# MKimiSH/video-filler

Measured on AMD Instinct MI355X. Metric: netG+netD fwd+bwd images/sec, 128x128 center-mask, higher is better.
Workload: dtype f32

## Files before the change

### include/vf_hip.h

```cpp
#ifndef VF_HIP_H
#define VF_HIP_H
#include <stddef.h>
#include <stdint.h>
#ifdef __cplusplus
extern "C" {
#endif

typedef struct vf_ctx vf_ctx;

enum { VF_ACT_NONE = 0, VF_ACT_LRELU = 1, VF_ACT_RELU = 2, VF_ACT_TANH = 3, VF_ACT_SIGMOID = 4 };

const char* vf_last_error(void);
int vf_version(void);
int vf_ctx_create(vf_ctx** out, int device, void* stream);
int vf_ctx_destroy(vf_ctx* ctx);
int vf_ctx_set_mfma_mode(vf_ctx* ctx, int mode);
int vf_ctx_set_stream(vf_ctx* ctx, void* stream);
int vf_ctx_set_workspace(vf_ctx* ctx, void* ptr, size_t bytes);
size_t vf_workspace_bytes_hint(void);
int vf_stream_synchronize(vf_ctx* ctx);
int vf_malloc(void** out, size_t bytes);
int vf_free(void* ptr);
int vf_memcpy_h2d(vf_ctx* ctx, void* dst, const void* src, size_t bytes);
int vf_memcpy_d2h(vf_ctx* ctx, void* dst, const void* src, size_t bytes);
// ... 6 lines not shown
int vf_conv2d_fwd(vf_ctx* ctx, const float* x, const float* w, const float* bias, float* y, int B, int H,
                  int W, int Cin, int Cout, int k, int stride, int pad, int act, float slope);
int vf_conv2d_bwd_data(vf_ctx* ctx, const float* gy, const float* w, float* gx, int B, int H, int W,
                       int Cin, int Cout, int k, int stride, int pad);
int vf_conv2d_bwd_data_act(vf_ctx* ctx, const float* gy, const float* w, float* gx, const float* x_act, int act,
                           float slope, int B, int H, int W, int Cin, int Cout, int k, int stride, int pad);
int vf_conv2d_bwd_weight(vf_ctx* ctx, const float* x, const float* gy, float* gw, float* gb, int B, int H,
                         int W, int Cin, int Cout, int k, int stride, int pad, float beta);

int vf_deconv2d_fwd(vf_ctx* ctx, const float* x, const float* w, const float* bias, float* y, int B, int H,
                    int W, int Cin, int Cout, int k, int stride, int pad, int act, float slope);
int vf_deconv2d_bwd_data(vf_ctx* ctx, const float* gy, const float* w, float* gx, int B, int H, int W,
                         int Cin, int Cout, int k, int stride, int pad);
int vf_deconv2d_bwd_weight(vf_ctx* ctx, const float* x, const float* gy, float* gw, float* gb, int B, int H,
                           int W, int Cin, int Cout, int k, int stride, int pad, float beta);

int vf_planes_split(vf_ctx* ctx, const float* x, void* planes, int64_t n);
int vf_conv2d_fwd_planes(vf_ctx* ctx, const float* x, const float* w, const float* bias, float* y, void* y_planes, int B,
                         int H, int W, int Cin, int Cout, int k, int stride, int pad, int act, float slope);
int vf_weight_planes(vf_ctx* ctx, const float* w, void* planes_native, void* planes_transposed, int d0, int d1);
int vf_weight_planes_multi(vf_ctx* ctx, const void* desc_dev, int n, int blocks);
int vf_pconv_supported(int B, int H, int W, int Cin, int Cout, int k, int stride, int pad, int transposed);
int vf_pconv_supported_in_mode(int mfma_mode, int B, int H, int W, int Cin, int Cout, int k, int stride, int pad, int transposed);
int vf_pconv_set_routing(int gather_patch, int scatter_patch);
int vf_pconv_gather(vf_ctx* ctx, const void* ap, const void* wp, const float* bias, float* y, int B, int H, int W, int Cin,
                    int Cout, int act, float slope);
int vf_pconv_scatter(vf_ctx* ctx, const void* ap, const void* wp, const float* bias, float* y, int B, int H, int W, int Cin,
                     int Cout, int act, float slope, const float* dmask, int dact, float dslope);
int vf_conv2d_bwd_weight_planes(vf_ctx* ctx, const float* x, const float* gy, const void* x_planes, const void* gy_planes, float* gw,
                                float* gb, int B, int H, int W, int Cin, int Cout, int k, int stride, int pad, float beta);
int vf_deconv2d_bwd_weight_planes(vf_ctx* ctx, const float* x, const float* gy, const void* x_planes, const void* gy_planes,
                                  float* gw, float* gb, int B, int H, int W, int Cin, int Cout, int k, int stride, int pad,
                                  float beta);

int vf_bn_stats(vf_ctx* ctx, const float* x, const float* shift, double* sums, int64_t npix, int C);
int vf_bn_finalize(vf_ctx* ctx, const double* sums, float* running_mean, float* running_var, float* save_mean,
                   float* save_invstd, int64_t n_total, int C, float momentum, float eps);
int vf_bn_apply(vf_ctx* ctx, const float* x, float* y, const float* gamma, const float* beta, const float* mean,
                const float* invstd, int64_t npix, int C, int act, float slope);
int vf_bn_train_fwd(vf_ctx* ctx, const float* x, float* y, const float* gamma, const float* beta,
                    float* running_mean, float* running_var, float* save_mean, float* save_invstd, double* sums,
                    int64_t npix, int C, float momentum, float eps, int act, float slope);
int vf_bn_eval_fwd(vf_ctx* ctx, const float* x, float* y, const float* gamma, const float* beta,
                   const float* running_mean, const float* running_var, int64_t npix, int C, float eps, int act,
                   float slope);
int vf_bn_bwd_stats(vf_ctx* ctx, const float* x, const float* y_act, const float* gy, const float* save_mean,
                    double* sums, int64_t npix, int C, int act, float slope);
int vf_bn_bwd_apply(vf_ctx* ctx, const float* x, const float* y_act, const float* gy, float* gx, float* ggamma,
                    float* gbeta, const float* gamma, const float* save_mean, const float* save_invstd,
                    const double* sums, int64_t npix, int64_t n_total, int C, int act, float slope, float pbeta);
int vf_bn_bwd(vf_ctx* ctx, const float* x, const float* y_act, const float* gy, float* gx, float* ggamma,
              float* gbeta, const float* gamma, const float* save_mean, const float* save_invstd, double* sums,
              int64_t npix, int C, int act, float slope, float pbeta);
int vf_bn_train_fwd_groups(vf_ctx* ctx, const float* x, float* y, const float* gamma, const float* beta,
                           float* running_mean, float* running_var, float* save_mean, float* save_invstd,
                           double* sums, int64_t npix_per_group, int C, int groups, float momentum, float eps,
                           int act, float slope);
int vf_bn_bwd_groups(vf_ctx* ctx, const float* x, const float* y_act, const float* gy, float* gx, float* ggamma,
                     float* gbeta, const float* gamma, const float* save_mean, const float* save_invstd,
                     double* sums, int64_t npix_per_group, int C, int groups, int act, float slope, float pbeta);

int vf_bn_train_fwd_planes(vf_ctx* ctx, const float* x, float* y, const float* gamma, const float* beta,
                           float* running_mean, float* running_var, float* save_mean, float* save_invstd, double* sums,
                           int64_t npix_per_group, int C, int groups, float momentum, float eps, int act, float slope,
                           void* y_planes);
int vf_bn_bwd_planes(vf_ctx* ctx, const float* x, const float* y_act, const float* gy, float* gx, float* ggamma,
// ... 158 lines not shown
                   int reason_cap);
int vf_gif_decode_workspace_bytes(const unsigned char* data, const int64_t* offs, int n, int alpha, size_t* ws_bytes,
                                  size_t* stage_bytes);
int vf_gif_decode(vf_ctx* ctx, const unsigned char* data, const int64_t* offs, int n, int alpha, const int64_t* out_offs,
                  unsigned char* out, void* stage, size_t stage_bytes, void* ws, size_t ws_bytes, int32_t* status);

int vf_display_workspace_bytes(int N, int C, int h, int w, int padding, int nrow, int scaleeach, int has_min, int has_max,
                               size_t* ws_bytes);
int vf_display_tensor(vf_ctx* ctx, const float* packed, int src_layout, float* grid, int N, int C, int h, int w, int padding,
                      int nrow, int scaleeach, int has_min, double min, int has_max, double max, int symmetric, int saturate);
int vf_center_finish(vf_ctx* ctx, const float* ctx_nhwc, const float* pred_nhwc, float* pretty, float* pasted,
                     float* pred_mapped, int B, int C, int fs, int overlapPred);

enum {
  VF_METRICS_N = 0, VF_METRICS_SSE = 1, VF_METRICS_SAE = 2, VF_METRICS_SSIM_Q = 3, VF_METRICS_SSIM_N = 4,
  VF_METRICS_FLICKER = 5, VF_METRICS_COLS = 6
};
int vf_frame_metrics(vf_ctx* ctx, const void* a, const void* b, int kind, int N, int C, int H, int W, int vh, int vw,
                     const unsigned char* mask, int clip, int64_t* table);

int vf_channel_copy(vf_ctx* ctx, const float* src, int Csrc, int c_src, float* dst, int Cdst, int c_dst, int Ccopy,
                    int64_t npix);
int vf_noise_fill(vf_ctx* ctx, float* out, int64_t n, uint64_t seed, const int32_t* counter_dev, uint64_t counter,
                  int normal);

int vf_wgrad_group_begin(vf_ctx* ctx);
int vf_wgrad_group_end(vf_ctx* ctx);
int vf_wgrad_group_abort(vf_ctx* ctx);
int vf_wgrad_group_count(vf_ctx* ctx, int* count);
int vf_wgrad_group_end_partial(vf_ctx* ctx, int count);

int vf_bias_grad_plan(int64_t P, int C, int* cq, int* rows_per_block, int* gx, int* gy);
int vf_bias_grad_multi(vf_ctx* ctx, const void* desc_dev, int n, int blocks1, int blocks2);

typedef struct vf_comm vf_comm;
#define VF_COMM_ID_BYTES 128
int vf_comm_available(void);
int vf_comm_unique_id(void* id128);
int vf_comm_init(vf_comm** out, const void* id128, int world, int rank);
int vf_comm_world(const vf_comm* c);
int vf_comm_rank(const vf_comm* c);
int vf_comm_allreduce_async(vf_comm* c, vf_ctx* ctx, void* buf, int64_t count, int dtype, int op, int* ticket);
int vf_comm_allreduce_avg_async(vf_comm* c, vf_ctx* ctx, float* buf, int64_t n, int* ticket);
int vf_comm_reduce_scatter_avg_async(vf_comm* c, vf_ctx* ctx, float* buf, int64_t shard_count, int* ticket);
int vf_comm_allgather_async(vf_comm* c, vf_ctx* ctx, float* buf, int64_t shard_count, int* ticket);
int vf_comm_broadcast_async(vf_comm* c, vf_ctx* ctx, float* buf, int64_t count, int root, int* ticket);
int vf_comm_wait(vf_comm* c, vf_ctx* ctx, int ticket);
int vf_comm_allreduce_inline(vf_comm* c, vf_ctx* ctx, void* buf, int64_t count, int dtype, int op);
int vf_comm_broadcast(vf_comm* c, vf_ctx* ctx, void* buf, int64_t count, int dtype, int root);
int vf_comm_barrier(vf_comm* c, vf_ctx* ctx);
int vf_comm_destroy(vf_comm* c);

int vf_prof_begin(vf_ctx* ctx);
int vf_prof_end(vf_ctx* ctx);
int vf_prof_count(void);
int vf_prof_get(int i, char* name, int name_cap, int64_t* launches, double* ms, double* flops, double* bytes);

enum { VF_L_CONV = 1, VF_L_FULLCONV = 2, VF_L_BN = 3, VF_L_ACT = 4, VF_L_VIEW = 5 };
typedef struct vf_layer_desc {
  int kind;
  int nin, nout;
  int k, stride, pad;
  int act;
  float slope;
  float eps, momentum;
} vf_layer_desc;
// ... 60 lines not shown
```

### video-filler_amd/_lib.py

```python
import ctypes as C
import os
import re

_HERE = os.path.dirname(os.path.abspath(__file__))
_HEADER = os.path.join(_HERE, "..", "include", "vf_hip.h")

vp, f32, i32, i64, f64, sz, u64 = C.c_void_p, C.c_float, C.c_int, C.c_int64, C.c_double, C.c_size_t, C.c_uint64

SIGNATURES = {
    "vf_last_error": (C.c_char_p, []),
    "vf_version": (i32, []),
    "vf_ctx_create": (i32, [C.POINTER(vp), i32, vp]),
    "vf_ctx_destroy": (i32, [vp]),
    "vf_ctx_set_mfma_mode": (i32, [vp, i32]),
    "vf_ctx_set_stream": (i32, [vp, vp]),
    "vf_ctx_set_workspace": (i32, [vp, vp, sz]),
    "vf_workspace_bytes_hint": (sz, []),
    "vf_stream_synchronize": (i32, [vp]),
    "vf_malloc": (i32, [C.POINTER(vp), sz]),
    "vf_free": (i32, [vp]),
    "vf_memcpy_h2d": (i32, [vp, vp, vp, sz]),
    "vf_memcpy_d2h": (i32, [vp, vp, vp, sz]),
    "vf_zero": (i32, [vp, vp, sz]),
    "vf_zero_segments": (i32, [vp, vp, vp, vp, i32]),
# ... 13 lines not shown
    "vf_pconv_supported_in_mode": (i32, [i32] * 10),
    "vf_pconv_set_routing": (i32, [i32, i32]),
    "vf_pconv_gather": (i32, [vp, vp, vp, vp, vp] + [i32] * 5 + [i32, f32]),
    "vf_pconv_scatter": (i32, [vp, vp, vp, vp, vp] + [i32] * 5 + [i32, f32, vp, i32, f32]),
    "vf_bn_stats": (i32, [vp, vp, vp, vp, i64, i32]),
    "vf_bn_finalize": (i32, [vp, vp, vp, vp, vp, vp, i64, i32, f32, f32]),
    "vf_bn_apply": (i32, [vp, vp, vp, vp, vp, vp, vp, i64, i32, i32, f32]),
    "vf_bn_train_fwd": (i32, [vp] * 10 + [i64, i32, f32, f32, i32, f32]),
    "vf_bn_eval_fwd": (i32, [vp] * 7 + [i64, i32, f32, i32, f32]),
    "vf_bn_bwd_stats": (i32, [vp] * 6 + [i64, i32, i32, f32]),
    "vf_bn_bwd_apply": (i32, [vp] * 11 + [i64, i64, i32, i32, f32, f32]),
    "vf_bn_bwd": (i32, [vp] * 11 + [i64, i32, i32, f32, f32]),
    "vf_bn_train_fwd_groups": (i32, [vp] * 10 + [i64, i32, i32, f32, f32, i32, f32]),
    "vf_bn_bwd_groups": (i32, [vp] * 11 + [i64, i32, i32, i32, f32, f32]),
    "vf_bn_train_fwd_planes": (i32, [vp] * 10 + [i64, i32, i32, f32, f32, i32, f32, vp]),
    "vf_bn_bwd_planes": (i32, [vp] * 11 + [i64, i32, i32, i32, f32, f32, vp]),
    "vf_bn_fuse_next_fwd": (i32, [vp, vp, vp, i32, i32]),
    "vf_bn_fuse_next_bwd": (i32, [vp, vp, vp, i32, f32, vp, vp, i32, i32]),
    "vf_bn_fuse_result": (i32, [vp, C.POINTER(i32)]),
    "vf_bn_train_fwd_pre": (i32, [vp, vp, i32] + [vp] * 9 + [i64, i32, i32, f32, f32, i32, f32, vp]),
    "vf_bn_bwd_pre": (i32, [vp, vp, i32] + [vp] * 9 + [i64, i32, i32, f32, vp]),
    "vf_act_fwd": (i32, [vp, vp, vp, i64, i32, f32]),
    "vf_act_bwd": (i32, [vp, vp, vp, vp, i64, i32, f32]),
    "vf_axpby": (i32, [vp, f32, vp, f32, vp, i64]),
    "vf_cmul": (i32, [vp, vp, vp, i64]),
    "vf_scale_shift": (i32, [vp, vp, f32, f32, i64]),
    "vf_masked_compose": (i32, [vp, vp, vp, vp, vp, i64]),
    "vf_conv2d_bwd_data_act": (i32, [vp, vp, vp, vp, vp, i32, f32, i32, i32, i32, i32, i32, i32, i32, i32]),
    "vf_wgrad_group_begin": (i32, [vp]),
    "vf_wgrad_group_end": (i32, [vp]),
    "vf_wgrad_group_abort": (i32, [vp]),
    "vf_bias_grad_plan": (i32, [i64, i32, vp, vp, vp, vp]),
    "vf_bias_grad_multi": (i32, [vp, vp, i32, i32, i32]),
    "vf_center_prepare": (i32, [vp, vp, vp, vp, vp, i32, i32, i32, i32]),
    "vf_clip_prepare": (i32, [vp, vp, vp, vp, vp, vp, i32, i32, i32, i32, i32, i32, i32, f32, i32, i32, vp, vp]),
    "vf_tiles_gather": (i32, [vp, vp, vp, i32, i32, i32, i32, i32, vp]),
    "vf_tiles_scatter": (i32, [vp, vp, vp, i32, i32, i32, i32, i32, vp]),
    "vf_image_scale": (i32, [vp, vp, i32, vp] + [i32] * 6),
    "vf_image_scale_u8": (i32, [vp, vp, vp] + [i32] * 6),
    "vf_image_hook2d": (i32, [vp, vp, i32, vp] + [i32] * 9),
    "vf_image_whole_frames": (i32, [vp, vp, i32, vp] + [i32] * 8 + [vp, f32]),
    "vf_crop_stats": (i32, [vp, vp, vp] + [i32] * 6 + [vp]),
    "vf_patch_array_prepare": (i32, [vp, vp, i32] + [vp] * 5 + [i32] * 10 + [f32]),
    "vf_jpeg_inspect": (i32, [vp, sz, i32, vp, C.c_char_p, i32]),
    "vf_jpeg_workspace_bytes": (i32, [vp, vp, i32, i32, C.POINTER(sz), C.POINTER(sz)]),
    "vf_jpeg_decode": (i32, [vp, vp, vp, i32, i32, i32, vp, vp, vp, sz, vp, sz, vp, vp]),
    "vf_jpeg_scans_inspect": (i32, [vp, sz, vp, vp, i32, C.c_char_p, i32]),
    "vf_jpeg_prog_workspace_bytes": (i32, [vp, vp, i32, i32, C.POINTER(sz), C.POINTER(sz)]),
    "vf_jpeg_prog_decode": (i32, [vp, vp, vp, i32, i32, i32, vp, vp, vp, sz, vp, sz, vp, vp, vp]),
    "vf_jpeg_prog_coefficients_host": (i32, [vp, sz, i32, vp, sz, vp]),
    "vf_jpeg_inspect_layouts": (i32, [vp, sz, vp, C.c_char_p, i32]),
    "vf_jpeg_layouts_workspace_bytes": (i32, [vp, vp, i32, i32, C.POINTER(sz), C.POINTER(sz)]),
    "vf_jpeg_decode_layouts": (i32, [vp, vp, vp, i32, i32, i32, vp, vp, vp, sz, vp, sz, vp, vp, vp]),
    "vf_jpeg_layouts_coefficients_host": (i32, [vp, sz, i32, vp, sz, vp]),
    "vf_png_inspect": (i32, [vp, sz, vp, C.c_char_p, i32]),
    "vf_png_decode_workspace_bytes": (i32, [vp, vp, i32, i32, C.POINTER(sz), C.POINTER(sz)]),
    "vf_png_decode": (i32, [vp, vp, vp, i32, i32, vp, vp, vp, sz, vp, sz, vp]),
    "vf_png_bytes_to_float": (i32, [vp, vp, vp, i64]),
    "vf_png_inspect_full": (i32, [vp, sz, vp, vp, C.c_char_p, i32]),
    "vf_png_decode_full_workspace_bytes": (i32, [vp, vp, i32, i32, i32, C.POINTER(sz), C.POINTER(sz)]),
    "vf_png_decode_full": (i32, [vp, vp, vp, i32, i32, i32, vp, vp, vp, sz, vp, sz, vp]),
    "vf_png_workspace_bytes": (i32, [i32, i32, i32, i32, C.POINTER(sz), C.POINTER(sz)]),
    "vf_png_encode": (i32, [vp, vp, i32, i32, i32, i32, i32, vp, sz, vp, sz, vp]),
    "vf_jpeg_encode_workspace_bytes": (i32, [i32, i32, i32, i32, i32, C.POINTER(sz), C.POINTER(sz)]),
    "vf_jpeg_encode": (i32, [vp, vp, i32, i32, i32, i32, i32, i32, i32, vp, sz, vp, sz, vp]),
    "vf_jpeg_encode_opts_workspace_bytes": (i32, [i32] * 8 + [C.POINTER(sz), C.POINTER(sz)]),
# ... 6 lines not shown
    "vf_apng_encode": (i32, [vp, vp, i32, i32, i32, i32, i32, i32, i32, i32, vp, sz, vp, sz, vp]),
    "vf_apng_inspect": (i32, [vp, sz, vp, vp, i32, C.c_char_p, i32]),
    "vf_apng_decode_workspace_bytes": (i32, [vp, vp, i32, i32, C.POINTER(sz), C.POINTER(sz)]),
    "vf_apng_decode": (i32, [vp, vp, vp, i32, i32, vp, vp, vp, sz, vp, sz, vp]),
    "vf_gif_inspect": (i32, [vp, sz, vp, vp, i32, C.c_char_p, i32]),
    "vf_gif_decode_workspace_bytes": (i32, [vp, vp, i32, i32, C.POINTER(sz), C.POINTER(sz)]),
    "vf_gif_decode": (i32, [vp, vp, vp, i32, i32, vp, vp, vp, sz, vp, sz, vp]),
    "vf_display_workspace_bytes": (i32, [i32] * 9 + [C.POINTER(sz)]),
    "vf_display_tensor": (i32, [vp, vp, i32, vp] + [i32] * 8 + [f64, i32, f64, i32, i32]),
    "vf_center_finish": (i32, [vp] * 6 + [i32] * 4),
    "vf_frame_metrics": (i32, [vp, vp, vp] + [i32] * 7 + [vp, i32, vp]),
    "vf_channel_copy": (i32, [vp, vp, i32, i32, vp, i32, i32, i32, i64]),
    "vf_noise_fill": (i32, [vp, vp, i64, u64, vp, u64, i32]),
    "vf_bce_fwd": (i32, [vp, vp, f32, i32, vp]),
    "vf_bce_bwd": (i32, [vp, vp, f32, vp, i32]),
    "vf_bce_fwd_bwd": (i32, [vp, vp, f32, f32, i32, i32, vp, vp, vp]),
    "vf_mse_fwd": (i32, [vp, vp, vp, i64, vp]),
    "vf_mse_bwd": (i32, [vp, vp, vp, vp, i64]),
    "vf_recon_grad_mix": (i32, [vp, vp, vp, vp, vp, f32, f32, f32, i32, i32, i32, i64, vp]),
    "vf_gdl_fwd": (i32, [vp, vp, vp, i32, i32, i32, i32, vp]),
    "vf_gdl_bwd": (i32, [vp, vp, vp, vp, i32, i32, i32, i32]),
    "vf_masked_mse_fwd": (i32, [vp, vp, vp, vp, f32, i64, vp]),
    "vf_masked_mse_bwd": (i32, [vp, vp, vp, vp, f32, vp, i64]),
    "vf_adam_step": (i32, [vp, vp, vp, vp, vp, i64, f64, f64, f64, f64, vp]),
    "vf_adam_prep": (i32, [vp, f64, f64, f64, vp]),
    "vf_adam_apply": (i32, [vp, vp, vp, vp, vp, i64, f64, f64, f64, vp]),
    "vf_adam_apply_ranges": (i32, [vp, vp, vp, vp, vp, C.POINTER(i64), C.POINTER(i64), i32, f64, f64, f64, vp]),
    "vf_wgrad_adam_outer_supported": (i32, [i32, i32, i32]),
    "vf_wgrad_adam_outer": (i32, [vp, vp, vp, i32, i32, i32, vp, vp, vp, vp, f64, f64, f64, vp]),
    "vf_wgrad_adam_outer_gathered": (i32, [vp, vp, vp, i32, i32, i64, i32, i32, vp, vp, vp, vp, C.c_float, f64, f64, f64, vp]),
    "vf_wgrad_adam_outer_rows": (i32, [vp, vp, vp, i32, i32, i64, i32, i32, i32, i32, vp, vp, vp, vp, C.c_float, f64, f64, f64, vp]),
    "vf_conv_is_fast": (i32, [i32, i32, i32, i32, i32]),
    "vf_conv2d_bwd_weight_planes": (i32, [vp, vp, vp, vp, vp, vp, vp, i32, i32, i32, i32, i32, i32, i32, i32, f32]),
    "vf_deconv2d_bwd_weight_planes": (i32, [vp, vp, vp, vp, vp, vp, vp, i32, i32, i32, i32, i32, i32, i32, i32, f32]),
    "vf_comm_available": (i32, []),
    "vf_comm_unique_id": (i32, [vp]),
    "vf_comm_init": (i32, [C.POINTER(vp), vp, i32, i32]),
    "vf_comm_world": (i32, [vp]),
    "vf_comm_rank": (i32, [vp]),
    "vf_comm_allreduce_async": (i32, [vp, vp, vp, i64, i32, i32, C.POINTER(i32)]),
    "vf_comm_allreduce_avg_async": (i32, [vp, vp, vp, i64, C.POINTER(i32)]),
    "vf_comm_reduce_scatter_avg_async": (i32, [vp, vp, vp, i64, C.POINTER(i32)]),
    "vf_comm_allgather_async": (i32, [vp, vp, vp, i64, C.POINTER(i32)]),
    "vf_comm_broadcast_async": (i32, [vp, vp, vp, i64, i32, C.POINTER(i32)]),
    "vf_comm_wait": (i32, [vp, vp, i32]),
    "vf_comm_allreduce_inline": (i32, [vp, vp, vp, i64, i32, i32]),
    "vf_comm_broadcast": (i32, [vp, vp, vp, i64, i32, i32]),
    "vf_comm_barrier": (i32, [vp, vp]),
    "vf_comm_destroy": (i32, [vp]),
    "vf_net_create": (i32, [vp, C.POINTER(vp), vp, i32, i32, i32, i32, i32]),
    "vf_net_destroy": (i32, [vp]),
    "vf_net_parameters": (i32, [vp, C.POINTER(vp), C.POINTER(vp), C.POINTER(i64)]),
    "vf_net_param_offset": (i64, [vp, i32, i32, C.POINTER(i64)]),
    "vf_net_bn_running": (i32, [vp, i32, C.POINTER(vp), C.POINTER(vp)]),
    "vf_net_training": (i32, [vp, i32]),
    "vf_net_zero_grad": (i32, [vp]),
    "vf_net_forward": (i32, [vp, vp, C.POINTER(vp)]),
    "vf_net_backward": (i32, [vp, vp, vp, C.POINTER(vp)]),
    "vf_net_update_grad_input": (i32, [vp, vp, vp, C.POINTER(vp)]),
    "vf_net_layer_output": (i32, [vp, i32, C.POINTER(vp)]),
    "vf_net_layer_grad_input": (i32, [vp, i32, C.POINTER(vp)]),
    "vf_net_layer_shape": (i32, [vp, i32] + [C.POINTER(i32)] * 7),
    "vf_net_reshape": (i32, [vp, i32, i32, i32, i32]),
    "vf_net_bind_parameters": (i32, [vp, vp, vp, i64]),
    "vf_net_bind_bn_running": (i32, [vp, i32, vp, vp]),
    "vf_net_bn_saved": (i32, [vp, i32, C.POINTER(vp), C.POINTER(vp)]),
# ... 79 lines not shown
```

### video-filler_amd/backend.py

```python
import ctypes as C
import os

import numpy as np
import torch

from . import _lib

ACT = {"none": 0, "lrelu": 1, "relu": 2, "tanh": 3, "sigmoid": 4}
COLSUM_DESC = [("g", "<u8"), ("gb", "<u8"), ("part", "<u8"), ("P", "<i8"), ("C", "<i4"), ("cq", "<i4"), ("rows_per_block", "<i4"),
               ("gx", "<i4"), ("gy", "<i4"), ("blk1_off", "<i4"), ("blk2_off", "<i4"), ("beta", "<f4")]
WPLANES_DESC = [("w", "<u8"), ("nat", "<u8"), ("tr", "<u8"), ("d0", "<i4"), ("d1", "<i4"), ("gx", "<i4"), ("gz", "<i4"),
                ("blk_off", "<i4"), ("pad", "<i4")]
MFMA_MODES = {"f32": 0, "bf16": 1, "f32_3xbf16": 3}
DEFAULT_MFMA_MODE = "f32_3xbf16"


_COMM_DTYPE = {torch.float32: 0, torch.float64: 1}
_COMM_OP = {"sum": 0, "avg": 1, "max": 2, "min": 3}


class _Range:
    def __init__(self, lib, name):
        self.lib, self.name = lib, name.encode()

    def __enter__(self):
        self.lib.vf_range_push(self.name)
        return self

    def __exit__(self, *exc):
        self.lib.vf_range_pop()
        return False


class _CommHandle:

    def __init__(self, backend, ticket):
        self.backend, self.ticket = backend, ticket

    def wait(self):
        b = self.backend
        _lib.check(b.lib.vf_comm_wait(b.comm, b.ctx, self.ticket))


def exchange_comm_id(backend, world, rank, addr=None, port=None, timeout_s=300):
    import datetime
# ... 640 lines not shown
        self._c("vf_conv2d_fwd_planes", _ptr(x), _ptr(w), _ptr(bias), _ptr(y), _ptr(y_planes), B, H, W, Cin, w.shape[0], k, stride,
                pad, ACT[act], slope)

    def conv2d_bwd_data(self, gy, w, gx, k, stride, pad):
        B, Cin, H, W = gx.shape
        self._c("vf_conv2d_bwd_data", _ptr(gy), _ptr(w), _ptr(gx), B, H, W, Cin, w.shape[0], k, stride, pad)

    def conv2d_bwd_data_act(self, gy, w, gx, x_act, act, slope, k, stride, pad):
        B, Cin, H, W = gx.shape
        self._c("vf_conv2d_bwd_data_act", _ptr(gy), _ptr(w), _ptr(gx), _ptr(x_act), ACT[act], slope, B, H, W, Cin,
                w.shape[0], k, stride, pad)

    def wgrad_group_begin(self):
        self._c("vf_wgrad_group_begin")

    def wgrad_group_end(self):
        self._c("vf_wgrad_group_end")

    def wgrad_group_abort(self):
        self._c("vf_wgrad_group_abort")

    def wgrad_group_count(self):
        n = C.c_int(0)
        self._c("vf_wgrad_group_count", C.byref(n))
        return n.value

    def wgrad_group_end_partial(self, count):
        self._c("vf_wgrad_group_end_partial", int(count))

    def bias_grad_multi(self, items):
        import numpy as np
        if not items:
            return
        key = (self.workspace.data_ptr(), self.workspace.numel()) + tuple(
            (g.data_ptr(), gb.data_ptr(), g.numel(), gb.numel(), float(beta)) for g, gb, beta in items)
        cache = self.__dict__.setdefault("_colsum_plans", {})
        plan = cache.get(key)
        if plan is None:
            desc = np.zeros(len(items), dtype=COLSUM_DESC)
            ws = self.workspace.data_ptr()
            off, b1, b2 = 0, 0, 0
            for i, (g, gb, beta) in enumerate(items):
                Cc = gb.numel()
                P = g.numel() // Cc
                assert Cc % 4 == 0 and g.data_ptr() % 16 == 0 and is_nhwc(g)
                geo = [C.c_int() for _ in range(4)]
                _lib.check(self.lib.vf_bias_grad_plan(P, Cc, *[C.byref(v) for v in geo]))
                cq, rpb, gx, gy = [v.value for v in geo]
                desc[i] = (g.data_ptr(), gb.data_ptr(), ws + off, P, Cc, cq, rpb, gx, gy, b1, b2, beta)
                off += (gx * Cc * 8 + 255) // 256 * 256
                b1 += gx * gy
                b2 += (Cc + 3) // 4
            assert off <= self.workspace.numel(), "workspace too small for the bias-gradient partials"
            dev = torch.from_numpy(desc.view(np.uint8).copy()).to(self.device)
            plan = (dev, len(items), b1, b2)
            cache[key] = plan
        dev, n, b1, b2 = plan
        self._c("vf_bias_grad_multi", _ptr(dev), n, b1, b2)

    def conv2d_bwd_weight(self, x, gy, gw, gb, k, stride, pad, beta, x_planes=None, gy_planes=None):
        B, Cin, H, W = x.shape
        if x_planes is not None and gy_planes is not None:
            self._c("vf_conv2d_bwd_weight_planes", _ptr(x), _ptr(gy), _ptr(x_planes), _ptr(gy_planes), _ptr(gw), _ptr(gb), B, H, W,
                    Cin, gw.shape[0], k, stride, pad, beta)
            return
        self._c("vf_conv2d_bwd_weight", _ptr(x), _ptr(gy), _ptr(gw), _ptr(gb), B, H, W, Cin, gw.shape[0], k, stride,
                pad, beta)

    def deconv2d_fwd(self, x, w, bias, y, k, stride, pad, act="none", slope=0.0):
        B, Cin, H, W = x.shape
        self._c("vf_deconv2d_fwd", _ptr(x), _ptr(w), _ptr(bias), _ptr(y), B, H, W, Cin, w.shape[1], k, stride, pad,
                ACT[act], slope)

    def deconv2d_bwd_data(self, gy, w, gx, k, stride, pad):
        B, Cin, H, W = gx.shape
        self._c("vf_deconv2d_bwd_data", _ptr(gy), _ptr(w), _ptr(gx), B, H, W, Cin, w.shape[1], k, stride, pad)

    def deconv2d_bwd_weight(self, x, gy, gw, gb, k, stride, pad, beta, x_planes=None, gy_planes=None):
        B, Cin, H, W = x.shape
        if x_planes is not None and gy_planes is not None:
            self._c("vf_deconv2d_bwd_weight_planes", _ptr(x), _ptr(gy), _ptr(x_planes), _ptr(gy_planes), _ptr(gw), _ptr(gb), B, H,
                    W, Cin, gw.shape[1], k, stride, pad, beta)
            return
        self._c("vf_deconv2d_bwd_weight", _ptr(x), _ptr(gy), _ptr(gw), _ptr(gb), B, H, W, Cin, gw.shape[1], k, stride,
                pad, beta)

    def planes_split(self, x, planes=None):
        n = x.numel()
        if planes is None:
            planes = torch.empty((3, n), dtype=torch.bfloat16, device=self.device)
        self._c("vf_planes_split", _ptr(x), _ptr(planes), n)
        return planes

    def weight_planes(self, w, native=None, transposed=None, want_transposed=True):
        d0, d1 = w.shape[0], w.shape[1]
        n = w.numel()
        if native is None:
            native = torch.empty((3, n), dtype=torch.bfloat16, device=self.device)
        if transposed is None and want_transposed:
            transposed = torch.empty((3, n), dtype=torch.bfloat16, device=self.device)
# ... 29 lines not shown
        self._c("vf_pconv_scatter", _ptr(ap), _ptr(wp), _ptr(bias), _ptr(y), B, H, W, Cin, Cout, ACT[act], slope, _ptr(dmask),
                ACT[dact], dslope)

    def bn_stats(self, x, shift, sums):
        B, Cc, H, W = x.shape
        self._c("vf_bn_stats", _ptr(x), _ptr(shift), _ptr(sums), B * H * W, Cc)

    def bn_finalize(self, sums, rm, rv, save_mean, save_invstd, n_total, momentum, eps):
        self._c("vf_bn_finalize", _ptr(sums), _ptr(rm), _ptr(rv), _ptr(save_mean), _ptr(save_invstd), n_total,
                rm.numel(), momentum, eps)

    def bn_apply(self, x, y, gamma, beta, mean, invstd, act="none", slope=0.0):
        B, Cc, H, W = x.shape
        self._c("vf_bn_apply", _ptr(x), _ptr(y), _ptr(gamma), _ptr(beta), _ptr(mean), _ptr(invstd), B * H * W, Cc,
                ACT[act], slope)

    def bn_train_fwd(self, x, y, gamma, beta, rm, rv, save_mean, save_invstd, sums, momentum, eps, act="none", slope=0.0):
        B, Cc, H, W = x.shape
        self._c("vf_bn_train_fwd", _ptr(x), _ptr(y), _ptr(gamma), _ptr(beta), _ptr(rm), _ptr(rv), _ptr(save_mean),
                _ptr(save_invstd), _ptr(sums), B * H * W, Cc, momentum, eps, ACT[act], slope)

    def bn_train_fwd_groups(self, x, y, gamma, beta, rm, rv, save_mean, save_invstd, sums, groups, momentum, eps,
                            act="none", slope=0.0, y_planes=None):
        B, Cc, H, W = x.shape
        assert B % groups == 0 and save_mean.numel() == groups * Cc and sums.numel() == groups * 2 * Cc
        if y_planes is not None:
            self._c("vf_bn_train_fwd_planes", _ptr(x), _ptr(y), _ptr(gamma), _ptr(beta), _ptr(rm), _ptr(rv), _ptr(save_mean),
                    _ptr(save_invstd), _ptr(sums), (B // groups) * H * W, Cc, groups, momentum, eps, ACT[act], slope, _ptr(y_planes))
            return
        self._c("vf_bn_train_fwd_groups", _ptr(x), _ptr(y), _ptr(gamma), _ptr(beta), _ptr(rm), _ptr(rv), _ptr(save_mean),
                _ptr(save_invstd), _ptr(sums), (B // groups) * H * W, Cc, groups, momentum, eps, ACT[act], slope)

    def bn_bwd_groups(self, x, y_act, gy, gx, ggamma, gbeta, gamma, save_mean, save_invstd, sums, groups, act="none",
                      slope=0.0, pbeta=1.0, gx_planes=None):
        B, Cc, H, W = x.shape
        assert B % groups == 0 and save_mean.numel() == groups * Cc and sums.numel() == groups * 2 * Cc
        if gx_planes is not None:
            self._c("vf_bn_bwd_planes", _ptr(x), _ptr(y_act), _ptr(gy), _ptr(gx), _ptr(ggamma), _ptr(gbeta), _ptr(gamma),
                    _ptr(save_mean), _ptr(save_invstd), _ptr(sums), (B // groups) * H * W, Cc, groups, ACT[act], slope, pbeta,
                    _ptr(gx_planes))
            return
        self._c("vf_bn_bwd_groups", _ptr(x), _ptr(y_act), _ptr(gy), _ptr(gx), _ptr(ggamma), _ptr(gbeta), _ptr(gamma),
                _ptr(save_mean), _ptr(save_invstd), _ptr(sums), (B // groups) * H * W, Cc, groups, ACT[act], slope, pbeta)

    def bn_fuse_next_fwd(self, shift, part, groups=1):
        self._c("vf_bn_fuse_next_fwd", _ptr(shift), _ptr(part), part.numel() // (2 * shift.numel()), groups)

    def bn_fuse_next_bwd(self, x, y_act, act, slope, save_mean, part, groups=1):
        Cc = x.shape[1]
        self._c("vf_bn_fuse_next_bwd", _ptr(x), _ptr(y_act), ACT[act], slope, _ptr(save_mean), _ptr(part),
                part.numel() // (2 * Cc), groups)

    def bn_fuse_result(self):
        rows = C.c_int(0)
        self._c("vf_bn_fuse_result", C.byref(rows))
        return rows.value

    def bn_train_fwd_pre(self, part, rows, x, y, gamma, beta, rm, rv, save_mean, save_invstd, sums, groups, momentum, eps,
                         act="none", slope=0.0, y_planes=None):
        B, Cc, H, W = x.shape
        self._c("vf_bn_train_fwd_pre", _ptr(part), rows, _ptr(x), _ptr(y), _ptr(gamma), _ptr(beta), _ptr(rm), _ptr(rv),
                _ptr(save_mean), _ptr(save_invstd), _ptr(sums), (B // groups) * H * W, Cc, groups, momentum, eps, ACT[act], slope,
                _ptr(y_planes))

    def bn_bwd_pre(self, part, rows, x, g_masked, gx, ggamma, gbeta, gamma, save_mean, save_invstd, sums, groups, pbeta=1.0,
                   gx_planes=None):
        B, Cc, H, W = x.shape
        self._c("vf_bn_bwd_pre", _ptr(part), rows, _ptr(x), _ptr(g_masked), _ptr(gx), _ptr(ggamma), _ptr(gbeta), _ptr(gamma),
                _ptr(save_mean), _ptr(save_invstd), _ptr(sums), (B // groups) * H * W, Cc, groups, pbeta, _ptr(gx_planes))

    def bn_eval_fwd(self, x, y, gamma, beta, rm, rv, eps, act="none", slope=0.0):
        B, Cc, H, W = x.shape
        self._c("vf_bn_eval_fwd", _ptr(x), _ptr(y), _ptr(gamma), _ptr(beta), _ptr(rm), _ptr(rv), B * H * W, Cc, eps,
                ACT[act], slope)

    def bn_bwd_stats(self, x, y_act, gy, save_mean, sums, act="none", slope=0.0):
        B, Cc, H, W = x.shape
        self._c("vf_bn_bwd_stats", _ptr(x), _ptr(y_act), _ptr(gy), _ptr(save_mean), _ptr(sums), B * H * W, Cc,
                ACT[act], slope)

    def bn_bwd_apply(self, x, y_act, gy, gx, ggamma, gbeta, gamma, save_mean, save_invstd, sums, n_total, act="none",
                     slope=0.0, pbeta=1.0):
        B, Cc, H, W = x.shape
        self._c("vf_bn_bwd_apply", _ptr(x), _ptr(y_act), _ptr(gy), _ptr(gx), _ptr(ggamma), _ptr(gbeta), _ptr(gamma),
                _ptr(save_mean), _ptr(save_invstd), _ptr(sums), B * H * W, n_total, Cc, ACT[act], slope, pbeta)

    def bn_bwd(self, x, y_act, gy, gx, ggamma, gbeta, gamma, save_mean, save_invstd, sums, act="none", slope=0.0, pbeta=1.0):
        B, Cc, H, W = x.shape
        self._c("vf_bn_bwd", _ptr(x), _ptr(y_act), _ptr(gy), _ptr(gx), _ptr(ggamma), _ptr(gbeta), _ptr(gamma),
                _ptr(save_mean), _ptr(save_invstd), _ptr(sums), B * H * W, Cc, ACT[act], slope, pbeta)

    def act_fwd(self, x, y, act, slope=0.0):
        self._c("vf_act_fwd", _ptr(x), _ptr(y), x.numel(), ACT[act], slope)

    def act_bwd(self, y, gy, gx, act, slope=0.0):
        self._c("vf_act_bwd", _ptr(y), _ptr(gy), _ptr(gx), y.numel(), ACT[act], slope)

    def axpby(self, a, x, b, y):
        self._c("vf_axpby", a, _ptr(x), b, _ptr(y), y.numel())

# ... 404 lines not shown
```

### video-filler_amd/csrc/vf_bn.hip

```cpp
#include <algorithm>

#include "vf_device.h"

__device__ __forceinline__ void bn_store_planes(unsigned short* __restrict__ planes, int64_t pstride, int64_t i, f32x4 v, int npl) {
  if (npl == 1) {
    *(u32x2*)(planes + i) = vf_round4(v);
    return;
  }
  u32x2 o[3];
  vf_split3(v, o);
#pragma unroll
  for (int q = 0; q < 3; ++q) *(u32x2*)(planes + q * pstride + i) = o[q];
}

struct BnGeom {
  int cq;
  int rp;
  int gy;
  int gx;
  int rows_per_block;
};

static BnGeom bn_geom(int64_t npix, int C, int target_blocks = 2048) {
  BnGeom g;
// ... 271 lines not shown
      const int64_t o = r * C + 4 * c4;
      f32x4 g = *(const f32x4*)(gy + o);
      if (act != VF_ACT_NONE) {
        const f32x4 ya = *(const f32x4*)(yact + o);
#pragma unroll
        for (int e = 0; e < 4; ++e) g[e] = vf_act_grad(ya[e], g[e], act, slope);
      }
      const f32x4 xv = *(const f32x4*)(x + o);
      s += g;
      dp += g * (xv - mu);
    }
  }
  __shared__ f32x4 red[2][256];
  red[0][threadIdx.x] = s;
  red[1][threadIdx.x] = dp;
  __syncthreads();
  if (ty == 0 && c4 < C4) {
    double a[4] = {0, 0, 0, 0}, b[4] = {0, 0, 0, 0};
    for (int j = 0; j < rp; ++j) {
      const f32x4 u = red[0][j * cq + tx], w = red[1][j * cq + tx];
      for (int e = 0; e < 4; ++e) {
        a[e] += (double)u[e];
        b[e] += (double)w[e];
      }
    }
    double* o = part + (int64_t)blockIdx.x * 2 * C;
    for (int e = 0; e < 4; ++e) {
      o[4 * c4 + e] = a[e];
      o[C + 4 * c4 + e] = b[e];
    }
  }
}

__global__ __launch_bounds__(256) void k_bn_bwd_apply(const float* __restrict__ x, const float* __restrict__ yact,
                                                      const float* __restrict__ gy, float* __restrict__ gx,
                                                      float* __restrict__ ggamma, float* __restrict__ gbeta,
                                                      const float* __restrict__ gamma, const float* __restrict__ mean,
                                                      const float* __restrict__ invstd, const double* __restrict__ sums,
                                                      int64_t npix, double n, int C, int cq, int rows_per_block, int act,
                                                      float slope, float pbeta, unsigned short* __restrict__ planes, int64_t pstride, int npl) {
  const int rp = 256 / cq;
  const int tx = threadIdx.x % cq, ty = threadIdx.x / cq;
  const int c4 = blockIdx.y * cq + tx;
  if (c4 >= (C >> 2)) return;
  if (blockIdx.x == 0 && blockIdx.z == 0 && ty == 0) {
#pragma unroll
    for (int e = 0; e < 4; ++e) {
      float gg = (ggamma && pbeta != 0.f) ? pbeta * ggamma[4 * c4 + e] : 0.f;
      float gb = (gbeta && pbeta != 0.f) ? pbeta * gbeta[4 * c4 + e] : 0.f;
      for (int g = 0; g < (int)gridDim.z; ++g) {
        const double sm = sums[(int64_t)g * 2 * C + 4 * c4 + e], dp = sums[(int64_t)g * 2 * C + C + 4 * c4 + e];
        gg = gg + (float)(dp * invstd[(int64_t)g * C + 4 * c4 + e]);
        gb = gb + (float)sm;
      }
      if (ggamma) ggamma[4 * c4 + e] = gg;
      if (gbeta) gbeta[4 * c4 + e] = gb;
    }
  }
  if (!gx) return;
  {
    const int64_t go = (int64_t)blockIdx.z * npix * C;
    x += go;
    gy += go;
    gx += go;
    if (yact) yact += go;
    if (planes) planes += go;
    mean += (int64_t)blockIdx.z * C;
    invstd += (int64_t)blockIdx.z * C;
    sums += (int64_t)blockIdx.z * 2 * C;
  }
  const int64_t r0 = (int64_t)blockIdx.x * rows_per_block, r1 = min(npix, r0 + rows_per_block);
  const f32x4 mu = *(const f32x4*)(mean + 4 * c4), is = *(const f32x4*)(invstd + 4 * c4);
  const f32x4 ga = gamma ? *(const f32x4*)(gamma + 4 * c4) : f32x4{1, 1, 1, 1};
  f32x4 kk, gm;
#pragma unroll
  for (int e = 0; e < 4; ++e) {
    const double sum = sums[4 * c4 + e], dotp = sums[C + 4 * c4 + e];
    kk[e] = (float)(dotp * is[e] * is[e] / n);
    gm[e] = (float)(sum / n);
  }
  for (int64_t r = r0 + ty; r < r1; r += rp) {
    const int64_t o = r * C + 4 * c4;
    f32x4 g = *(const f32x4*)(gy + o);
    if (act != VF_ACT_NONE) {
      const f32x4 ya = *(const f32x4*)(yact + o);
#pragma unroll
      for (int e = 0; e < 4; ++e) g[e] = vf_act_grad(ya[e], g[e], act, slope);
    }
    const f32x4 xv = *(const f32x4*)(x + o);
    const f32x4 out = (g - gm - (xv - mu) * kk) * is * ga;
    *(f32x4*)(gx + o) = out;
    if (planes) bn_store_planes(planes, pstride, o, out, npl);
  }
}

__device__ __forceinline__ int vf_find_layer(const VfColsumDesc* __restrict__ d, int n, int blk, bool stage2) {
  int l = 0;
  while (l + 1 < n && blk >= (stage2 ? d[l + 1].blk2_off : d[l + 1].blk1_off)) ++l;
  return l;
}
__global__ __launch_bounds__(256) void k_colsum4_multi(const VfColsumDesc* __restrict__ d, int n) {
  const int l = vf_find_layer(d, n, blockIdx.x, false);
  const VfColsumDesc L = d[l];
  const int local = blockIdx.x - L.blk1_off;
  const int bx = local % L.gx, by = local / L.gx;
  const int rp = 256 / L.cq;
  const int tx = threadIdx.x % L.cq, ty = threadIdx.x / L.cq;
  const int c4 = by * L.cq + tx;
  const int C4 = L.C >> 2;
  const int64_t r0 = (int64_t)bx * L.rows_per_block, r1 = min(L.P, r0 + L.rows_per_block);
  f32x4 s = {0, 0, 0, 0};
  if (c4 < C4)
    for (int64_t r = r0 + ty; r < r1; r += rp) s += *(const f32x4*)(L.g + r * L.C + 4 * c4);
  __shared__ f32x4 red[256];
  red[threadIdx.x] = s;
  __syncthreads();
  if (ty == 0 && c4 < C4) {
    double a[4] = {0, 0, 0, 0};
    for (int j = 0; j < rp; ++j) {
      const f32x4 u = red[j * L.cq + tx];
      for (int e = 0; e < 4; ++e) a[e] += (double)u[e];
    }
    double* o = L.part + (int64_t)bx * L.C;
    for (int e = 0; e < 4; ++e) o[4 * c4 + e] = a[e];
  }
}
__global__ __launch_bounds__(256) void k_reduce_bias_multi(const VfColsumDesc* __restrict__ d, int n) {
  const int l = vf_find_layer(d, n, blockIdx.x, true);
  const VfColsumDesc L = d[l];
  const int lane = threadIdx.x & 63, slot = threadIdx.x >> 6;
  const int col = (blockIdx.x - L.blk2_off) * 4 + slot;
  double s0 = 0, s1 = 0;
  if (col < L.C) {
    const double* p = L.part + col;
    int k = lane;
    for (; k + 64 < L.gx; k += 128) {
      s0 += p[(int64_t)k * L.C];
      s1 += p[(int64_t)(k + 64) * L.C];
    }
    for (; k < L.gx; k += 64) s0 += p[(int64_t)k * L.C];
  }
  double t = s0 + s1;
#pragma unroll
  for (int off = 32; off > 0; off >>= 1) t += __shfl_down(t, off, 64);
  if (lane == 0 && col < L.C) L.gb[col] = (L.beta != 0.f ? L.beta * L.gb[col] : 0.f) + (float)t;
}

static int run_stats(vf_ctx* ctx, const BnGeom& g, double* sums, int C, int groups = 1) {
  hipLaunchKernelGGL((k_reduce_partials<0>), dim3((int)vf_cdiv(2 * C, 16), groups), dim3(256), 0, ctx->stream,
                     (const double*)vf_ws_ptr(ctx), g.gx, 2 * C, sums, (float*)nullptr, (float*)nullptr, (float*)nullptr,
                     (float*)nullptr, 0.0, 0.f, 0.f, (float*)nullptr, 0.f, 1);
  VF_LAUNCH_CHECK();
  return 0;
}

int vf_internal_colsum(vf_ctx* ctx, const float* g, float* gb, int64_t P, int C, float beta) {
  VfProf prof(ctx, "bias_grad", 0.0, 4.0 * (double)P * C);
  double* part = (double*)vf_ws_ptr(ctx);
  int nslab;
  if (C % 4 == 0 && (((uintptr_t)g) & 15) == 0) {
    const BnGeom ge = bn_geom(P, C, bn_stat_blocks(P, C, 32768));
    nslab = ge.gx;
    VF_REQUIRE((size_t)(nslab + 1) * C * sizeof(double) <= vf_ws_avail(ctx), "workspace too small for bias-grad partials");
    hipLaunchKernelGGL(k_colsum4, dim3(ge.gx, ge.gy), dim3(256), 0, ctx->stream, g, part, P, C, ge.cq, ge.rows_per_block);
  } else {
    const int64_t rpb = std::max<int64_t>(256, vf_cdiv(P, std::max(1, 1024 / C)));
    nslab = (int)vf_cdiv(P, rpb);
    VF_REQUIRE((size_t)(nslab + 1) * C * sizeof(double) <= vf_ws_avail(ctx), "workspace too small for bias-grad partials");
    hipLaunchKernelGGL(k_colsum1, dim3(nslab, C), dim3(256), 0, ctx->stream, g, part, P, C, (int)rpb);
  }
  VF_LAUNCH_CHECK();
  hipLaunchKernelGGL((k_reduce_partials<2>), dim3((int)vf_cdiv(C, 16)), dim3(256), 0, ctx->stream, (const double*)part, nslab,
                     C, (double*)nullptr, (float*)nullptr, (float*)nullptr, (float*)nullptr, (float*)nullptr, 0.0, 0.f, 0.f,
                     gb, beta, 1);
  VF_LAUNCH_CHECK();
  return 0;
}

VF_API int vf_bn_stats(vf_ctx* ctx, const float* x, const float* shift, double* sums, int64_t npix, int C) {
// ... 71 lines not shown
  return bn_train_fwd_groups(ctx, x, y, gamma, beta, running_mean, running_var, save_mean, save_invstd, sums, npix_per_group, C,
                             groups, momentum, eps, act, slope);
}

VF_API int vf_bn_eval_fwd(vf_ctx* ctx, const float* x, float* y, const float* gamma, const float* beta,
                          const float* running_mean, const float* running_var, int64_t npix, int C, float eps, int act,
                          float slope) {
  VF_REQUIRE((size_t)2 * C * sizeof(float) <= vf_ws_avail(ctx), "workspace too small");
  float* mean = (float*)vf_ws_ptr(ctx);
  float* invstd = mean + C;
  hipLaunchKernelGGL(k_bn_eval_coeff, dim3((int)vf_cdiv(C, 256)), dim3(256), 0, ctx->stream, running_mean, running_var, mean,
                     invstd, C, eps);
  VF_LAUNCH_CHECK();
  return vf_bn_apply(ctx, x, y, gamma, beta, mean, invstd, npix, C, act, slope);
}

static int bn_bwd_stats_groups(vf_ctx* ctx, const float* x, const float* y_act, const float* gy, const float* save_mean,
                               double* sums, int64_t npix, int C, int groups, int act, float slope) {
  VF_REQUIRE(C % 4 == 0, "BatchNorm channel count must be a multiple of 4 (got %d)", C);
  VF_REQUIRE(act == VF_ACT_NONE || y_act != nullptr, "fused activation backward needs the activated output");
  VF_REQUIRE(groups >= 1 && groups <= 64, "BatchNorm batch groups: %d", groups);
  const BnGeom g = bn_geom(npix, C, bn_stat_blocks(npix, C, 16384));
  VF_REQUIRE((size_t)groups * g.gx * 2 * C * sizeof(double) <= vf_ws_avail(ctx), "workspace too small for BN partials");
  VfProf prof(ctx, "bn_bwd_stats", 0.0, 4.0 * (double)npix * C * groups * (act != VF_ACT_NONE ? 3 : 2));
  hipLaunchKernelGGL(k_bn_bwd_stats, dim3(g.gx, g.gy, groups), dim3(256), 0, ctx->stream, x, y_act, gy, save_mean,
                     (double*)vf_ws_ptr(ctx), npix, C, g.cq, g.rows_per_block, act, slope);
  VF_LAUNCH_CHECK();
  return run_stats(ctx, g, sums, C, groups);
}

static int bn_bwd_apply_groups(vf_ctx* ctx, const float* x, const float* y_act, const float* gy, float* gx, float* ggamma,
                               float* gbeta, const float* gamma, const float* save_mean, const float* save_invstd,
                               const double* sums, int64_t npix, int64_t n_total, int C, int groups, int act, float slope,
                               float pbeta, void* planes = nullptr) {
  VF_REQUIRE(C % 4 == 0, "BatchNorm channel count must be a multiple of 4 (got %d)", C);
  VF_REQUIRE(!planes || gx, "gradient planes go with the gradient itself");
  const BnGeom g = bn_geom(npix, C);
  VfProf prof(ctx, planes ? "bn_bwd_apply_planes" : "bn_bwd_apply", 0.0,
              gx ? (double)npix * C * groups * (4.0 * (act != VF_ACT_NONE ? 4 : 3) + (planes ? 6.0 : 0.0)) : 0.0);
  hipLaunchKernelGGL(k_bn_bwd_apply, dim3(g.gx, g.gy, groups), dim3(256), 0, ctx->stream, x, y_act, gy, gx, ggamma, gbeta, gamma,
                     save_mean, save_invstd, sums, npix, (double)n_total, C, g.cq, g.rows_per_block, act, slope, pbeta,
                     (unsigned short*)planes, npix * C * groups, ctx->mfma_bf16 == 1 ? 1 : 3);
  VF_LAUNCH_CHECK();
  return 0;
}

VF_API int vf_bn_bwd_stats(vf_ctx* ctx, const float* x, const float* y_act, const float* gy, const float* save_mean,
                           double* sums, int64_t npix, int C, int act, float slope) {
  return bn_bwd_stats_groups(ctx, x, y_act, gy, save_mean, sums, npix, C, 1, act, slope);
}

VF_API int vf_bn_bwd_apply(vf_ctx* ctx, const float* x, const float* y_act, const float* gy, float* gx, float* ggamma,
                           float* gbeta, const float* gamma, const float* save_mean, const float* save_invstd,
                           const double* sums, int64_t npix, int64_t n_total, int C, int act, float slope, float pbeta) {
  return bn_bwd_apply_groups(ctx, x, y_act, gy, gx, ggamma, gbeta, gamma, save_mean, save_invstd, sums, npix, n_total, C, 1, act,
                             slope, pbeta);
}

VF_API int vf_bn_bwd(vf_ctx* ctx, const float* x, const float* y_act, const float* gy, float* gx, float* ggamma,
                     float* gbeta, const float* gamma, const float* save_mean, const float* save_invstd, double* sums,
                     int64_t npix, int C, int act, float slope, float pbeta) {
  if (int rc = bn_bwd_stats_groups(ctx, x, y_act, gy, save_mean, sums, npix, C, 1, act, slope)) return rc;
  return bn_bwd_apply_groups(ctx, x, y_act, gy, gx, ggamma, gbeta, gamma, save_mean, save_invstd, sums, npix, npix, C, 1, act,
                             slope, pbeta);
}

VF_API int vf_bn_bwd_groups(vf_ctx* ctx, const float* x, const float* y_act, const float* gy, float* gx, float* ggamma,
                            float* gbeta, const float* gamma, const float* save_mean, const float* save_invstd, double* sums,
                            int64_t npix_per_group, int C, int groups, int act, float slope, float pbeta) {
  if (int rc = bn_bwd_stats_groups(ctx, x, y_act, gy, save_mean, sums, npix_per_group, C, groups, act, slope)) return rc;
  return bn_bwd_apply_groups(ctx, x, y_act, gy, gx, ggamma, gbeta, gamma, save_mean, save_invstd, sums, npix_per_group,
                             npix_per_group, C, groups, act, slope, pbeta);
}

VF_API int vf_bn_train_fwd_planes(vf_ctx* ctx, const float* x, float* y, const float* gamma, const float* beta,
                                  float* running_mean, float* running_var, float* save_mean, float* save_invstd, double* sums,
                                  int64_t npix_per_group, int C, int groups, float momentum, float eps, int act, float slope,
                                  void* y_planes) {
  return bn_train_fwd_groups(ctx, x, y, gamma, beta, running_mean, running_var, save_mean, save_invstd, sums, npix_per_group, C,
                             groups, momentum, eps, act, slope, y_planes);
}
VF_API int vf_bn_bwd_planes(vf_ctx* ctx, const float* x, const float* y_act, const float* gy, float* gx, float* ggamma,
                            float* gbeta, const float* gamma, const float* save_mean, const float* save_invstd, double* sums,
                            int64_t npix_per_group, int C, int groups, int act, float slope, float pbeta, void* gx_planes) {
  if (int rc = bn_bwd_stats_groups(ctx, x, y_act, gy, save_mean, sums, npix_per_group, C, groups, act, slope)) return rc;
  return bn_bwd_apply_groups(ctx, x, y_act, gy, gx, ggamma, gbeta, gamma, save_mean, save_invstd, sums, npix_per_group,
                             npix_per_group, C, groups, act, slope, pbeta, gx_planes);
}

VF_API int vf_bn_train_fwd_pre(vf_ctx* ctx, const double* part, int rows_per_group, const float* x, float* y, const float* gamma,
                               const float* beta, float* running_mean, float* running_var, float* save_mean, float* save_invstd,
                               double* sums, int64_t npix_per_group, int C, int groups, float momentum, float eps, int act,
                               float slope, void* y_planes) {
  VF_REQUIRE(C % 4 == 0, "BatchNorm channel count must be a multiple of 4 (got %d)", C);
  VF_REQUIRE(part && rows_per_group > 0 && groups >= 1 && groups <= 64, "vf_bn_train_fwd_pre: bad partials");
  {
    VfProf prof(ctx, "bn_finalize", 0.0, 8.0 * (double)rows_per_group * 2 * C * groups);
    hipLaunchKernelGGL((k_reduce_partials<1>), dim3((int)vf_cdiv(C, 8)), dim3(256), 0, ctx->stream, part, rows_per_group, 2 * C, sums,
                       running_mean, running_var, save_mean, save_invstd, (double)npix_per_group, momentum, eps, (float*)nullptr, 0.f,
                       groups);
    VF_LAUNCH_CHECK();
  }
  return bn_apply_groups(ctx, x, y, gamma, beta, save_mean, save_invstd, npix_per_group, C, groups, act, slope, y_planes);
}
VF_API int vf_bn_bwd_pre(vf_ctx* ctx, const double* part, int rows_per_group, const float* x, const float* g_masked, float* gx,
                         float* ggamma, float* gbeta, const float* gamma, const float* save_mean, const float* save_invstd,
                         double* sums, int64_t npix_per_group, int C, int groups, float pbeta, void* gx_planes) {
  VF_REQUIRE(C % 4 == 0, "BatchNorm channel count must be a multiple of 4 (got %d)", C);
  VF_REQUIRE(part && rows_per_group > 0 && groups >= 1 && groups <= 64, "vf_bn_bwd_pre: bad partials");
  {
    VfProf prof(ctx, "bn_bwd_finalize", 0.0, 8.0 * (double)rows_per_group * 2 * C * groups);
    hipLaunchKernelGGL((k_reduce_partials<0>), dim3((int)vf_cdiv(2 * C, 16), groups), dim3(256), 0, ctx->stream, part, rows_per_group,
                       2 * C, sums, (float*)nullptr, (float*)nullptr, (float*)nullptr, (float*)nullptr, 0.0, 0.f, 0.f, (float*)nullptr,
                       0.f, 1);
    VF_LAUNCH_CHECK();
  }
  return bn_bwd_apply_groups(ctx, x, nullptr, g_masked, gx, ggamma, gbeta, gamma, save_mean, save_invstd, sums, npix_per_group,
                             npix_per_group, C, groups, VF_ACT_NONE, 0.f, pbeta, gx_planes);
}

VF_API int vf_bias_grad_plan(int64_t P, int C, int* cq, int* rows_per_block, int* gx, int* gy) {
  VF_REQUIRE(P > 0 && C > 0 && C % 4 == 0, "vf_bias_grad_plan: C must be a positive multiple of 4 (got %d)", C);
  const BnGeom g = bn_geom(P, C, bn_stat_blocks(P, C, 32768));
  *cq = g.cq; *rows_per_block = g.rows_per_block; *gx = g.gx; *gy = g.gy;
  return 0;
}
VF_API int vf_bias_grad_multi(vf_ctx* ctx, const void* desc_dev, int n, int blocks1, int blocks2) {
  VF_REQUIRE(desc_dev != nullptr && n > 0 && blocks1 > 0 && blocks2 > 0, "vf_bias_grad_multi: empty plan");
  VfProf prof(ctx, "bias_grad_multi", 0.0, 0.0);
  hipLaunchKernelGGL(k_colsum4_multi, dim3(blocks1), dim3(256), 0, ctx->stream, (const VfColsumDesc*)desc_dev, n);
  VF_LAUNCH_CHECK();
  hipLaunchKernelGGL(k_reduce_bias_multi, dim3(blocks2), dim3(256), 0, ctx->stream, (const VfColsumDesc*)desc_dev, n);
  VF_LAUNCH_CHECK();
  return 0;
}
```

### video-filler_amd/csrc/vf_conv.hip

```cpp
#include <algorithm>
#include <vector>
#include <cstdlib>

#include "vf_device.h"

template <int LD>
__device__ __forceinline__ bf16x8 vf_tr_frag(const __bf16* tile, int col0, int k0, int lane) {
  const int grp = lane >> 4, i = lane & 15;
  const __bf16* a = tile + (k0 + 8 * (grp >> 1) + (i >> 2)) * LD + col0 + 16 * (grp & 1) + 4 * (i & 3);
  typedef __attribute__((address_space(3))) bf16x4 lds_bf16x4;
  const bf16x4 lo = __builtin_amdgcn_ds_read_tr16_b64_v4bf16((lds_bf16x4*)a);
  const bf16x4 hi = __builtin_amdgcn_ds_read_tr16_b64_v4bf16((lds_bf16x4*)(a + 4 * LD));
  return __builtin_shufflevector(lo, hi, 0, 1, 2, 3, 4, 5, 6, 7);
}

struct IGemm {
  const float* A;
  const float* Wt;
  const float* bias;
  float* Y;
  float* slab;
  int64_t out_elems;
  unsigned a_bytes, w_bytes;
  int M, lgMh, lgMw;
// ... 678 lines not shown
static int launch_slab_reduce(vf_ctx* ctx, const float* slab, float* dst, const float* bias, int64_t total, int N, int ksplit,
                              int act, float slope, float beta, const float* dmask = nullptr, int dact = 0,
                              float dslope = 0.f) {
  if (total % 4 == 0 && ((((uintptr_t)slab) | ((uintptr_t)dst) | ((uintptr_t)dmask)) & 15) == 0 && ksplit > 0) {
    const int64_t total4 = total / 4;
    if (total4 <= 8192 && ksplit >= 64)
      hipLaunchKernelGGL(k_slab_reduce4<16>, dim3((int)vf_cdiv(total4, 16)), dim3(256), 0, ctx->stream, slab, dst, bias, total4, N,
                         ksplit, act, slope, beta, dmask, dact, dslope);
    else
      hipLaunchKernelGGL(k_slab_reduce4<64>, dim3((int)vf_cdiv(total4, 64)), dim3(256), 0, ctx->stream, slab, dst, bias, total4, N,
                         ksplit, act, slope, beta, dmask, dact, dslope);
  } else {
    const int nb = (int)std::min<int64_t>(vf_cdiv(total, 256), 4096);
    hipLaunchKernelGGL(k_slab_reduce, dim3(nb), dim3(256), 0, ctx->stream, slab, dst, bias, total, N, ksplit, act, slope, beta,
                       dmask, dact, dslope);
  }
  VF_LAUNCH_CHECK();
  return 0;
}

struct WGrad {
  const float* U;
  const float* V;
  float* dW;
  float* slab;
  unsigned u_bytes, v_bytes;
  int P, lgMh, lgMw;
  int Nu, Cv, Hv, Wv;
  int stride, pad;
  int ntaps;
  int gx, gy, gz;
  int ksplit, nk;
  float beta;
};

enum WgV {
  WGV_SCALAR,
  WGV_VEC16,
  WGV_PIX3
};
template <int BM, bool VU, WgV VV, int BF = 0, int BN = 128>
__device__ __forceinline__ void wgrad_body(const WGrad& p, const int block_id) {
  static_assert(VV == WGV_PIX3 ? (BN == 64 && BF != 0) : BN == 128, "the whole-pixel form is a 64-column tile of the bf16 modes");
  constexpr int BK = BF ? 32 : 16;
  constexpr int LDU = BM + 4, LDV = BN + 4;
  constexpr int WN = (BM == 128 && BN == 128) ? 64 : 32;
  constexpr int NT = WN / 32;
  constexpr int WAVES_N = BN / WN;
  constexpr int WM = BM / (4 / WAVES_N);
  constexpr int MT = WM / 32;
  constexpr int CQ = BN / 4;
  constexpr int U_CH = (BK * BM / 4) / 256;
  constexpr int V_CH = (BK * BN / 4) / 256;
  constexpr int U_SZ = BK * LDU, V_SZ = BK * LDV;
  constexpr int LDMU = BM + 32, LDMV = BN + 32;
  constexpr int UH_SZ = BK * LDMU, VH_SZ = BK * LDMV;
  constexpr int NP = BF > 0 ? BF : 1;
  constexpr int NBUF = BF == 3 ? 1 : 2;
  constexpr int PL_SZ = UH_SZ + VH_SZ;
  constexpr int SMEM_F = BF ? (NBUF * NP * PL_SZ + 1) / 2 : 2 * (U_SZ + V_SZ);
  __shared__ __attribute__((aligned(16))) float smem[SMEM_F];

  const int tid = threadIdx.x, lane = tid & 63, wave = tid >> 6;
  const int wm = (wave / WAVES_N) * WM, wn = (wave % WAVES_N) * WN;
  const int lid = vf_xcd_remap(block_id, p.gx * p.gy * p.gz);
  const int n0 = ((lid / p.gx) % p.gy) * BM, j0 = (lid % p.gx) * BN;
  const int ks = lid / (p.gx * p.gy);
  const int steps = (p.nk + p.ksplit - 1) / p.ksplit;
  const int kt0 = ks * steps, kt1 = min(p.nk, kt0 + steps);
  const int Ncols = p.ntaps * p.Cv;
  const int Mw = 1 << p.lgMw, Mh = 1 << p.lgMh;

  const int cq = tid % CQ, vrow = tid / CQ;
  int v_dy[4], v_dx[4], v_c[4];
  bool v_okc[4];
#pragma unroll
  for (int j = 0; j < 4; ++j) {
    const int col = j0 + 4 * cq + j;
    v_okc[j] = col < Ncols;
    const int tap = v_okc[j] ? col / p.Cv : 0;
    v_c[j] = v_okc[j] ? col - tap * p.Cv : 0;
    v_dy[j] = (tap >> 2) - p.pad;
    v_dx[j] = (tap & 3) - p.pad;
  }
  const int uq = tid % (BM / 4), ukk = tid / (BM / 4);
  const int un = n0 + 4 * uq;

  f32x4 ru[U_CH], rv[V_CH];
  const __amdgpu_buffer_rsrc_t rsU = vf_rsrc(p.U, p.u_bytes), rsV = vf_rsrc(p.V, p.v_bytes);

  auto load_piece = [&](int kt, int pc, bool live) {
    if (pc < U_CH) {
      const int i = pc;
      const int pp = kt * BK + ukk + i * (1024 / BM);
      const bool okp = live && pp < p.P;
      if constexpr (VU) {
        ru[i] = vf_bload4(rsU, (okp && un < p.Nu) ? 4u * (unsigned)(pp * p.Nu + un) : VF_OOB);
      } else {
        f32x4 v;
#pragma unroll
        for (int j = 0; j < 4; ++j) {
          v[j] = vf_bload1(rsU, (okp && un + j < p.Nu) ? 4u * (unsigned)(pp * p.Nu + un + j) : VF_OOB);
        }
        ru[i] = v;
      }
    } else {
      const int i = pc - U_CH;
      const int pp = kt * BK + vrow + (256 / CQ) * i;
      const bool okp = live && pp < p.P;
      const int mx = pp & (Mw - 1), my = (pp >> p.lgMw) & (Mh - 1), b = pp >> (p.lgMw + p.lgMh);
      const int boff = b * p.Hv * p.Wv * p.Cv;
      if constexpr (VV == WGV_PIX3) {
        const int iy = my * p.stride + (cq >> 2) - p.pad, ix = mx * p.stride + (cq & 3) - p.pad;
        const bool ok = okp && (unsigned)iy < (unsigned)p.Hv && (unsigned)ix < (unsigned)p.Wv;
        rv[i] = vf_bload3(rsV, ok ? 4u * (unsigned)(boff + (iy * p.Wv + ix) * 3) : VF_OOB);
      } else if constexpr (VV == WGV_VEC16) {
        const int iy = my * p.stride + v_dy[0], ix = mx * p.stride + v_dx[0];
        const bool ok = okp && v_okc[0] && (unsigned)iy < (unsigned)p.Hv && (unsigned)ix < (unsigned)p.Wv;
        rv[i] = vf_bload4(rsV, ok ? 4u * (unsigned)(boff + (iy * p.Wv + ix) * p.Cv + v_c[0]) : VF_OOB);
      } else {
        f32x4 v;
#pragma unroll
        for (int j = 0; j < 4; ++j) {
          const int iy = my * p.stride + v_dy[j], ix = mx * p.stride + v_dx[j];
          const bool ok = okp && v_okc[j] && (unsigned)iy < (unsigned)p.Hv && (unsigned)ix < (unsigned)p.Wv;
          v[j] = vf_bload1(rsV, ok ? 4u * (unsigned)(boff + (iy * p.Wv + ix) * p.Cv + v_c[j]) : VF_OOB);
        }
        rv[i] = v;
      }
    }
  };
  auto store_piece = [&](int buf, int pc) {
    if constexpr (BF) {
      __bf16* base = (__bf16*)smem + buf * (NP * PL_SZ);
      f32x4 v;
      int off;
      if (pc < U_CH) {
        v = ru[pc];
        off = (ukk + pc * (1024 / BM)) * LDMU + 4 * uq;
      } else {
        const int i = pc - U_CH;
        v = rv[i];
        off = UH_SZ + (vrow + (256 / CQ) * i) * LDMV + 4 * cq;
      }
      if constexpr (NP == 3) {
        u32x2 s3[3];
        vf_split3(v, s3);
#pragma unroll
        for (int q = 0; q < 3; ++q) *(u32x2*)(base + q * PL_SZ + off) = s3[q];
      } else {
        *(bf16x4*)(base + off) = __builtin_convertvector(v, bf16x4);
      }
      return;
    }
    float* Us = smem + buf * (U_SZ + V_SZ);
    float* Vs = Us + U_SZ;
    if (pc < U_CH) {
      *(f32x4*)(Us + (ukk + pc * (1024 / BM)) * LDU + 4 * uq) = ru[pc];
    } else {
      const int i = pc - U_CH;
      *(f32x4*)(Vs + (vrow + (256 / CQ) * i) * LDV + 4 * cq) = rv[i];
    }
  };
  constexpr int NPC = U_CH + V_CH;
  auto load_tile = [&](int kt) {
#pragma unroll
    for (int pc = 0; pc < NPC; ++pc) load_piece(kt, pc, true);
  };
  auto store_tile = [&](int buf) {
#pragma unroll
    for (int pc = 0; pc < NPC; ++pc) store_piece(buf, pc);
// ... 62 lines not shown
    const float* Vs = Us + U_SZ;
    auto read_frag = [&](int ss, float (&a)[2][4], float (&b)[NT][4]) {
#pragma unroll
      for (int j = 0; j < 4; ++j) {
        const int k = 8 * ss + 4 * lh + j;
#pragma unroll
        for (int mt = 0; mt < 2; ++mt) a[mt][j] = Us[k * LDU + wm + mt * 32 + lr];
#pragma unroll
        for (int nt = 0; nt < NT; ++nt) b[nt][j] = Vs[k * LDV + wn + nt * 32 + lr];
      }
    };
    float fa[2][2][4], fb[2][NT][4];
    read_frag(0, fa[0], fb[0]);
#pragma unroll
    for (int ss = 0; ss < 2; ++ss) {
      if (ss == 0) read_frag(1, fa[1], fb[1]);
      __builtin_amdgcn_sched_barrier(0);
#pragma unroll
      for (int j = 0; j < 4; ++j)
#pragma unroll
        for (int mt = 0; mt < 2; ++mt)
#pragma unroll
          for (int nt = 0; nt < NT; ++nt) {
            acc[mt][nt] = __builtin_amdgcn_mfma_f32_32x32x2f32(fa[ss][mt][j], fb[ss][nt][j], acc[mt][nt], 0, 0, 0);
            const int slot = ss * NMF + (j * 2 + mt) * NT + nt;
            if (slot < NPC) load_piece(kt + 1, slot, more);
            if (slot >= SLOTS - NPC) store_piece(buf ^ 1, slot - (SLOTS - NPC));
            __builtin_amdgcn_sched_barrier(0);
          }
    }
    __syncthreads();
  }

  }
  const int64_t total = (int64_t)p.Nu * Ncols;
  float* out = p.ksplit > 1 ? p.slab + (int64_t)ks * total : p.dW;
#pragma unroll
  for (int mt = 0; mt < MT; ++mt)
#pragma unroll
    for (int r = 0; r < 16; ++r) {
      const int n = n0 + wm + mt * 32 + (r & 3) + 8 * (r >> 2) + 4 * lh;
      if (n >= p.Nu) continue;
#pragma unroll
      for (int nt = 0; nt < NT; ++nt) {
        int col = j0 + wn + nt * 32 + lr;
        bool okc = col < Ncols;
        if constexpr (VV == WGV_PIX3) {
          okc = (col & 3) != 3;
          col = 3 * (col >> 2) + (col & 3);
        }
        if (okc) {
          const int64_t idx = (int64_t)n * Ncols + col;
          float v = acc[mt][nt][r];
          if (p.ksplit == 1 && p.beta != 0.f) v += p.beta * out[idx];
          out[idx] = v;
        }
      }
    }
}

template <int BM, bool VU, WgV VV, int BF = 0>
__global__ __launch_bounds__(256) void k_wgrad(const WGrad p) {
  wgrad_body<BM, VU, VV, BF, VV == WGV_PIX3 ? 64 : 128>(p, blockIdx.x);
}

#define VF_WG_GROUP_MAX 16
struct WGradGroup {
  int n;
  int blk_off[VF_WG_GROUP_MAX + 1];
  WGrad d[VF_WG_GROUP_MAX];
};
static_assert(sizeof(WGradGroup) <= 3584, "kernel arguments are limited to 4 KB");
template <int BM, bool VU, WgV VV, int BF>
__global__ __launch_bounds__(256) void k_wgrad_group(const WGradGroup G) {
  int l = 0;
  while (l + 1 < G.n && (int)blockIdx.x >= G.blk_off[l + 1]) ++l;
  const int local = (int)blockIdx.x - G.blk_off[l];
  if (local >= G.d[l].gx * G.d[l].gy * G.d[l].gz) return;
  wgrad_body<BM, VU, VV, BF>(G.d[l], local);
}
struct SlabGroup {
  int n;
  int blk_off[VF_WG_GROUP_MAX + 1];
  struct { const float* slab; float* dst; int64_t total4; int ksplit; float beta; } d[VF_WG_GROUP_MAX];
};
__global__ __launch_bounds__(256) void k_slab_reduce4_group(const SlabGroup G) {
  int l = 0;
  while (l + 1 < G.n && (int)blockIdx.x >= G.blk_off[l + 1]) ++l;
  const int tx = threadIdx.x & 63, sl = threadIdx.x >> 6;
  const int64_t i4 = (int64_t)((int)blockIdx.x - G.blk_off[l]) * 64 + tx;
  const int64_t total4 = G.d[l].total4;
  const int ksplit = G.d[l].ksplit;
  const float* slab = G.d[l].slab;
  f32x4 s = {0.f, 0.f, 0.f, 0.f};
  if (i4 < total4) {
#pragma unroll 4
// ... 661 lines not shown
  R.clear();
  R.open = false;
  return 0;
}
VF_API int vf_wgrad_group_end(vf_ctx* ctx) {
  WgRecorder& R = wg_recorder(ctx);
  VF_REQUIRE(R.open, "vf_wgrad_group_end: no group is open");
  R.open = false;
  return wg_flush(ctx);
}

VF_API int vf_wgrad_group_count(vf_ctx* ctx, int* count) {
  VF_REQUIRE(count != nullptr, "vf_wgrad_group_count: NULL");
  WgRecorder& R = wg_recorder(ctx);
  *count = R.open ? (int)R.recs.size() : 0;
  return 0;
}
VF_API int vf_wgrad_group_end_partial(vf_ctx* ctx, int count) {
  WgRecorder& R = wg_recorder(ctx);
  VF_REQUIRE(R.open, "vf_wgrad_group_end_partial: no group is open");
  if (R.recs.empty() || count <= 0) return 0;
  std::vector<WgRec> rest;
  if (count < (int)R.recs.size()) {
    rest.assign(R.recs.begin() + count, R.recs.end());
    R.recs.resize((size_t)count);
  }
  const size_t used = R.ws_used;
  const int rc = wg_flush(ctx);
  R.recs = rest;
  R.ws_used = used;
  return rc;
}

static int wgrad(vf_ctx* ctx, const float* U, const float* V, float* dW, const VfConvShape& s, bool full, float beta, const void* Up,
                 const void* Vp) {
  WgPlan p = wg_plan(ctx, s, full, U, V, Up, Vp);
  if (p.route == WG_SMALLK) {
    const int rc = vf_internal_wgrad_smallk(ctx, U, V, dW, p.B, p.Nu, 16 * p.Cv, beta);
    if (rc >= 0) return rc;
    p.route = p.fp32_route();
  }
  VF_REQUIRE(p.in_range(4), "operand exceeds the 2 GiB buffer-descriptor range");
  WgRecorder& R = wg_recorder(ctx);
  auto slab_at = [&](size_t off) { return p.ksplit > 1 ? (float*)(vf_ws_ptr(ctx) + off) : nullptr; };
  size_t off = 0;
  if (p.planes() || (R.open && p.route == WG_FP32_GROUP)) {
    if (!R.reserve(p.slab_bytes(), vf_ws_avail(ctx), &off)) {
      if (int rc = wg_flush(ctx)) return rc;
      R.clear();
      VF_REQUIRE(R.reserve(p.slab_bytes(), vf_ws_avail(ctx), &off), "workspace too small for this layer's split-K slabs");
    }
    WgRec r;
    r.p = p;
    r.g = wg_desc(p, U, V, dW, slab_at(off), beta);
    r.bf = p.planes() ? 4 : ctx->mfma_bf16;
    if (p.planes()) r.pw = wg_desc_planes(p, Up, Vp, dW, r.g.slab, beta);
    else if (p.rider) r.pw = wg_desc_rider(p, U, V, dW, beta);
    R.recs.push_back(r);
    return R.open ? 0 : wg_flush(ctx);
  }
  float* slab = slab_at(0);
  if (R.open) {
    if (R.reserve(p.slab_bytes(), vf_ws_avail(ctx), &off)) slab = slab_at(off);
    else if (int rc = wg_flush(ctx)) return rc;
  }
  const WGrad g = wg_desc(p, U, V, dW, slab, beta);
  const int bf = ctx->mfma_bf16;
  const char* wname = p.pix3 ? (p.bm == 128 ? (bf == 3 ? "wgrad_128x64_pix3_bf16x3" : "wgrad_128x64_pix3_bf16")
                                            : (bf == 3 ? "wgrad_64x64_pix3_bf16x3" : "wgrad_64x64_pix3_bf16"))
                      : p.bm == 128 ? (bf == 3 ? "wgrad_128x128_bf16x3" : bf ? "wgrad_128x128_bf16" : "wgrad_128x128")
                                    : (bf == 3 ? "wgrad_64x128_bf16x3" : bf ? "wgrad_64x128_bf16" : "wgrad_64x128");
  const double wfl = p.flops();
  const dim3 grid((unsigned)p.blocks()), block(256);
  wg_dispatch(p.bm, bf, [&](auto BM, auto BF) {
    constexpr int bm_ = decltype(BM)::value, bf_ = decltype(BF)::value;
    if constexpr (bf_ != 0) {
      if (p.pix3) {
        VF_LAUNCH_TIMED(ctx, wname, wfl, 0.0, (k_wgrad<bm_, true, WGV_PIX3, bf_>), grid, block, g);
        return;
      }
    }
    if (p.vecU && p.vecV) VF_LAUNCH_TIMED(ctx, wname, wfl, 0.0, (k_wgrad<bm_, true, WGV_VEC16, bf_>), grid, block, g);
    else if (p.vecU) VF_LAUNCH_TIMED(ctx, wname, wfl, 0.0, (k_wgrad<bm_, true, WGV_SCALAR, bf_>), grid, block, g);
    else if (p.vecV) VF_LAUNCH_TIMED(ctx, wname, wfl, 0.0, (k_wgrad<bm_, false, WGV_VEC16, bf_>), grid, block, g);
    else VF_LAUNCH_TIMED(ctx, wname, wfl, 0.0, (k_wgrad<bm_, false, WGV_SCALAR, bf_>), grid, block, g);
  });
  VF_LAUNCH_CHECK();
  if (p.ksplit > 1) {
    VfProf prof(ctx, "slab_reduce_wgrad", 0.0, 4.0 * (double)p.total * (p.ksplit + 1));
    return launch_slab_reduce(ctx, g.slab, dW, nullptr, p.total, 1, p.ksplit, VF_ACT_NONE, 0.f, beta);
  }
  return 0;
}

VF_API int vf_conv_is_fast(int H, int W, int k, int stride, int pad) { return VfConvShape{0, H, W, 0, 0, k, stride, pad}.matrix_core_conv(); }

int vf_internal_conv2d_fwd(vf_ctx* ctx, const float* x, const float* w, const float* bias, float* y, const VfConvShape& s, int act,
                           float slope, VfConvExtras* ex) {
  if (!s.matrix_core_conv()) return vf_internal_gconv_fwd(ctx, x, w, bias, y, s, act, slope);
  if (int rc = check_conv_args(s)) return rc;
  if (s.stride == 2 && s.Cin == 3 && !ex->bn.st.mode) {
    const int rc = vf_internal_conv_thin_fwd(ctx, x, w, bias, y, nullptr, s, act, slope, ex);
    if (rc >= 0) return rc;
  }
  return conv_like_fwd(ctx, x, w, bias, y, s, act, slope, ex);
}
VF_API int vf_conv2d_fwd(vf_ctx* ctx, const float* x, const float* w, const float* bias, float* y, int B, int H, int W,
                         int Cin, int Cout, int k, int stride, int pad, int act, float slope) {
  const VfConvShape s{B, H, W, Cin, Cout, k, stride, pad};
  return vf_take_pending(ctx, [&](VfConvExtras* ex) { return vf_internal_conv2d_fwd(ctx, x, w, bias, y, s, act, slope, ex); });
}
// ... 19 lines not shown
  return vf_take_pending(ctx, [&](VfConvExtras* ex) { return vf_internal_conv2d_bwd_data(ctx, gy, w, gx, s, ex); });
}

int vf_internal_conv2d_bwd_data_act(vf_ctx* ctx, const float* gy, const float* w, float* gx, const float* x_act, int act, float slope,
                                    const VfConvShape& s, VfConvExtras* ex) {
  if (int rc = check_conv_args(s)) return rc;
  VF_REQUIRE(x_act != nullptr && (act == VF_ACT_LRELU || act == VF_ACT_RELU),
             "vf_conv2d_bwd_data_act: needs the activated input and a (leaky) ReLU");
  VF_REQUIRE(s.stride == 2, "vf_conv2d_bwd_data_act: only the stride-2 layers follow a bare conv + activation pair");
  return conv_like_bwd(ctx, gy, w, nullptr, gx, s.gradient_of_conv(), VF_ACT_NONE, 0.f, ex, x_act, act, slope);
}
VF_API int vf_conv2d_bwd_data_act(vf_ctx* ctx, const float* gy, const float* w, float* gx, const float* x_act, int act,
                                  float slope, int B, int H, int W, int Cin, int Cout, int k, int stride, int pad) {
  const VfConvShape s{B, H, W, Cin, Cout, k, stride, pad};
  return vf_take_pending(ctx, [&](VfConvExtras* ex) { return vf_internal_conv2d_bwd_data_act(ctx, gy, w, gx, x_act, act, slope, s, ex); });
}

int vf_internal_conv2d_bwd_weight(vf_ctx* ctx, const float* x, const float* gy, const void* x_planes, const void* gy_planes, float* gw,
                                  float* gb, const VfConvShape& s, float beta, const VfConvExtras* ex) {
  if (!s.matrix_core_conv()) return vf_internal_gconv_bwd_weight(ctx, x, gy, gw, gb, s, beta);
  if (int rc = check_conv_args(s)) return rc;
  if (s.Cout == 1 && s.stride == 1 && s.H == 4 && s.W == 4) {
    const VfConvExtras plain;
    if (!ex) ex = &plain;
    hipLaunchKernelGGL(k_dot_bwd_weight, dim3((int)vf_cdiv(16 * s.Cin, 64)), dim3(512), 0, ctx->stream, x, gy, gw, gb, s.B,
                       16 * s.Cin, beta, ex->dot_act_y, ex->dot_act, ex->dot_act_slope);
    VF_LAUNCH_CHECK();
    return 0;
  }
  if (int rc = wgrad(ctx, gy, x, gw, s, false, beta, gy_planes, x_planes)) return rc;
  if (gb) return vf_internal_colsum(ctx, gy, gb, (int64_t)s.B * s.out_h() * s.out_w(), s.Cout, beta);
  return 0;
}
VF_API int vf_conv2d_bwd_weight(vf_ctx* ctx, const float* x, const float* gy, float* gw, float* gb, int B, int H, int W,
                                int Cin, int Cout, int k, int stride, int pad, float beta) {
  return vf_conv2d_bwd_weight_planes(ctx, x, gy, nullptr, nullptr, gw, gb, B, H, W, Cin, Cout, k, stride, pad, beta);
}
VF_API int vf_conv2d_bwd_weight_planes(vf_ctx* ctx, const float* x, const float* gy, const void* x_planes, const void* gy_planes,
                                       float* gw, float* gb, int B, int H, int W, int Cin, int Cout, int k, int stride, int pad,
                                       float beta) {
  return vf_internal_conv2d_bwd_weight(ctx, x, gy, x_planes, gy_planes, gw, gb, VfConvShape{B, H, W, Cin, Cout, k, stride, pad}, beta, nullptr);
}

int vf_internal_deconv2d_fwd(vf_ctx* ctx, const float* x, const float* w, const float* bias, float* y, const VfConvShape& s, int act,
                             float slope, VfConvExtras* ex) {
  if (int rc = check_full_conv_args(s)) return rc;
  return conv_like_bwd(ctx, x, w, bias, y, s, act, slope, ex);
}
VF_API int vf_deconv2d_fwd(vf_ctx* ctx, const float* x, const float* w, const float* bias, float* y, int B, int H, int W,
                           int Cin, int Cout, int k, int stride, int pad, int act, float slope) {
  const VfConvShape s{B, H, W, Cin, Cout, k, stride, pad};
  return vf_take_pending(ctx, [&](VfConvExtras* ex) { return vf_internal_deconv2d_fwd(ctx, x, w, bias, y, s, act, slope, ex); });
}

int vf_internal_deconv2d_bwd_data(vf_ctx* ctx, const float* gy, const float* w, float* gx, const VfConvShape& s, VfConvExtras* ex) {
  if (int rc = check_full_conv_args(s)) return rc;
  return conv_like_fwd(ctx, gy, w, nullptr, gx, s.gradient_of_full(), VF_ACT_NONE, 0.f, ex);
}
VF_API int vf_deconv2d_bwd_data(vf_ctx* ctx, const float* gy, const float* w, float* gx, int B, int H, int W, int Cin,
                                int Cout, int k, int stride, int pad) {
  const VfConvShape s{B, H, W, Cin, Cout, k, stride, pad};
  return vf_take_pending(ctx, [&](VfConvExtras* ex) { return vf_internal_deconv2d_bwd_data(ctx, gy, w, gx, s, ex); });
}

int vf_internal_deconv2d_bwd_weight(vf_ctx* ctx, const float* x, const float* gy, const void* x_planes, const void* gy_planes, float* gw,
                                    float* gb, const VfConvShape& s, float beta) {
// ... 15 lines not shown
```

### video-filler_amd/csrc/vf_internal.h

```cpp
#pragma once
struct vf_ctx; struct VfBnSt; struct VfBnRequest; struct VfConvExtras; struct VfPWGradGroup; struct VfFusedLayer; struct WgRecorder;

struct VfConvShape {
  int B, H, W, Cin, Cout, k, stride, pad;
  int out_h() const { return (H + 2 * pad - k) / stride + 1; }
  int out_w() const { return (W + 2 * pad - k) / stride + 1; }
  int full_out_h() const { return (H - 1) * stride - 2 * pad + k; }
  int full_out_w() const { return (W - 1) * stride - 2 * pad + k; }
  bool pow2_map() const { return H > 0 && (H & (H - 1)) == 0 && W > 0 && (W & (W - 1)) == 0; }
  bool main_net_taps() const { return k == 4 && ((stride == 2 && pad == 1) || (stride == 1 && pad == 0)); }
  bool matrix_core_conv() const { return main_net_taps() && (stride == 2 || (H == 4 && W == 4)) && pow2_map(); }
  VfConvShape gradient_of_conv() const { return {B, out_h(), out_w(), Cout, Cin, k, stride, pad}; }
  VfConvShape gradient_of_full() const { return {B, full_out_h(), full_out_w(), Cout, Cin, k, stride, pad}; }
};

void vf_internal_wg_free(vf_ctx* ctx);
int vf_internal_slab_reduce(vf_ctx* ctx, const float* slab, float* dst, const float* bias, int64_t total, int N, int ksplit, int act,
                            float slope, const float* dmask, int dact, float dslope, const VfBnSt* st, int st_groups);
bool vf_internal_slab_st_ok(int64_t total, int N, int groups, int rows_cap, int* blocks_per_group);
int vf_internal_conv2d_fwd(vf_ctx* ctx, const float* x, const float* w, const float* bias, float* y, const VfConvShape& s, int act,
                           float slope, VfConvExtras* ex);
int vf_internal_conv2d_bwd_data(vf_ctx* ctx, const float* gy, const float* w, float* gx, const VfConvShape& s, VfConvExtras* ex);
int vf_internal_conv2d_bwd_data_act(vf_ctx* ctx, const float* gy, const float* w, float* gx, const float* x_act, int act, float slope,
                                    const VfConvShape& s, VfConvExtras* ex);
int vf_internal_conv2d_bwd_weight(vf_ctx* ctx, const float* x, const float* gy, const void* x_planes, const void* gy_planes, float* gw,
                                  float* gb, const VfConvShape& s, float beta, const VfConvExtras* ex);
int vf_internal_deconv2d_fwd(vf_ctx* ctx, const float* x, const float* w, const float* bias, float* y, const VfConvShape& s, int act,
                             float slope, VfConvExtras* ex);
int vf_internal_deconv2d_bwd_data(vf_ctx* ctx, const float* gy, const float* w, float* gx, const VfConvShape& s, VfConvExtras* ex);
int vf_internal_deconv2d_bwd_weight(vf_ctx* ctx, const float* x, const float* gy, const void* x_planes, const void* gy_planes, float* gw,
                                    float* gb, const VfConvShape& s, float beta);
int vf_internal_bn_request_fwd(VfBnRequest* r, const float* shift, double* part, int part_rows_cap, int groups);
int vf_internal_bn_request_bwd(VfBnRequest* r, const float* x, const float* y_act, int act, float slope, const float* save_mean,
                               double* part, int part_rows_cap, int groups);

int vf_internal_conv2d_fwd_planes(vf_ctx* ctx, const float* x, const float* w, const float* bias, float* y, void* y_planes,
                                  const VfConvShape& s, int act, float slope, VfConvExtras* ex);
int vf_internal_conv_thin_fwd(vf_ctx* ctx, const float* x, const float* w, const float* bias, float* y, void* y_planes,
                              const VfConvShape& s, int act, float slope, VfConvExtras* ex);
int vf_internal_deconv_thin_out(vf_ctx* ctx, const float* x, const float* w, const float* bias, float* y, const VfConvShape& s, int act,
                                float slope);

int vf_internal_gconv_fwd(vf_ctx* ctx, const float* x, const float* w, const float* bias, float* y, const VfConvShape& s, int act,
                          float slope);
int vf_internal_gconv_bwd_data(vf_ctx* ctx, const float* gy, const float* w, float* gx, const VfConvShape& s);
int vf_internal_gconv_bwd_weight(vf_ctx* ctx, const float* x, const float* gy, float* gw, float* gb, const VfConvShape& s, float beta);

bool vf_internal_pconv_supported(int mfma_mode, const VfConvShape& s, bool transposed);
int vf_internal_pconv_gather(vf_ctx* ctx, const void* ap, const void* wp, const float* bias, float* y, const VfConvShape& s, int act,
                             float slope, VfConvExtras* ex);
int vf_internal_pconv_scatter(vf_ctx* ctx, const void* ap, const void* wp, const float* bias, float* y, const VfConvShape& s, int act,
                              float slope, const float* dmask, int dact, float dslope, VfConvExtras* ex);
int vf_internal_pwgrad_group(vf_ctx* ctx, const VfPWGradGroup& G, int blocks, const char* name, double flops);

int vf_internal_smallm_plan(int form, int M, int N, int K, size_t ws_bytes);
int vf_internal_smallm_launch(vf_ctx* ctx, int form, const float* A, const float* W, float* slab, int M, int N, int K, int ksplit);

int vf_internal_wgrad_smallk(vf_ctx* ctx, const float* U, const float* V, float* dW, int K, int Nu, int Ncols, float beta);
int vf_internal_adam_fused_multi(vf_ctx* ctx, const VfFusedLayer* layers, int nl, double beta1, double beta2, double eps,
// ... 4 lines not shown
```

### video-filler_amd/csrc/vf_net.hip

```cpp
#include <algorithm>
#include <cstdlib>
#include <cstring>
#include <map>
#include <string>
#include <vector>

#include "vf_common.h"

namespace {

double g_gate_gflop = getenv("VF_PCONV_MIN_GFLOP") ? atof(getenv("VF_PCONV_MIN_GFLOP")) : 3.0;
int g_gate_rows = getenv("VF_PCONV_MIN_ROWS") ? atoi(getenv("VF_PCONV_MIN_ROWS")) : 1024;
const bool g_no_pconv = getenv("VF_NO_PCONV") != nullptr;
const bool g_no_bn_fuse = getenv("VF_NO_BN_FUSE") != nullptr;
const bool g_pwgrad = !(getenv("VF_PWGRAD") && strcmp(getenv("VF_PWGRAD"), "1") != 0);

struct Layer {
  vf_layer_desc d;
  int C = 0, H = 0, W = 0;
  int Co = 0, Ho = 0, Wo = 0;
  int64_t w_off = -1, b_off = -1, w_n = 0, b_n = 0;
  float* y = nullptr;
  float* y_own = nullptr;
  float* gx = nullptr;
  float* gtmp = nullptr;
  float *rm = nullptr, *rv = nullptr, *sm = nullptr, *si = nullptr;
  double* sums = nullptr;
  double* part = nullptr;
  int part_rows_cap = 0;
  void* xp = nullptr;
  void* gp = nullptr;
  void* yp = nullptr;
  void* bgp = nullptr;
  unsigned* ybits = nullptr;
  bool bits_live = false;
  const void* out_planes = nullptr;
  const void* grad_planes = nullptr;
  void *wp_nat = nullptr, *wp_tr = nullptr;
  bool wp_live = false;
  int wp_mode = 0;
  const float* x_seen = nullptr;
  const void* xp_seen = nullptr;
  const float* g_seen = nullptr;
  const void* gp_seen = nullptr;
  int fused_act = VF_ACT_NONE;
  float fused_slope = 0.f;
  bool absorbed = false;
  bool fresh = true;
  bool fa = false;
  const float *fa_u = nullptr, *fa_v = nullptr;
  int fa_k = 0;
  VfConvShape shape(int Bn) const { return {Bn, H, W, C, Co, d.k, d.stride, d.pad}; }
  VfConvShape grad_shape(int Bn) const { return d.kind == VF_L_FULLCONV ? shape(Bn).gradient_of_full() : shape(Bn).gradient_of_conv(); }
};

struct Entry {
  int main;
  int act;
};

inline bool is_conv(const Layer& l) { return l.d.kind == VF_L_CONV || l.d.kind == VF_L_FULLCONV; }
inline bool is_full(const Layer& l) { return l.d.kind == VF_L_FULLCONV; }
// ... 224 lines not shown
int conv_bwd_data(vf_net* n, Layer& l, const float* x, const float* go, int Bn, int in_act, float in_slope, const void* g_planes,
                  VfConvExtras* ex) {
  vf_ctx* ctx = n->ctx;
  const float* w = n->params + l.w_off;
  const bool full = is_full(l);
  const VfConvShape s = l.shape(Bn), gs = l.grad_shape(Bn);
  if (pconv_ok(n, l, gs, !full) && (in_act == VF_ACT_NONE || !full)) {
    const void* gp = g_planes;
    if (!gp) {
      if (int rc = ensure_planes(n, &l.gp, (int64_t)n->B * l.Ho * l.Wo * l.Co)) return rc;
      if (int rc = vf_planes_split(ctx, go, l.gp, (int64_t)Bn * l.Ho * l.Wo * l.Co)) return rc;
      gp = l.gp;
    }
    l.g_seen = go;
    l.gp_seen = gp;
    const void* wp = nullptr;
    if (int rc = weight_planes(n, l, !full, &wp)) return rc;
    if (full) return vf_internal_pconv_gather(ctx, gp, wp, nullptr, l.gx, gs, VF_ACT_NONE, 0.f, ex);
    return vf_internal_pconv_scatter(ctx, gp, wp, nullptr, l.gx, gs, VF_ACT_NONE, 0.f, in_act != VF_ACT_NONE ? x : nullptr, in_act, in_slope,
                                     ex);
  }
  l.g_seen = nullptr;
  if (in_act != VF_ACT_NONE)
    return vf_internal_conv2d_bwd_data_act(ctx, go, w, l.gx, x, in_act, in_slope, s, ex);
  return full ? vf_internal_deconv2d_bwd_data(ctx, go, w, l.gx, s, ex) : vf_internal_conv2d_bwd_data(ctx, go, w, l.gx, s, ex);
}

struct Deferred {
  const float* g;
  float* gb;
  int64_t P;
  int C;
  float beta;
};

int conv_acc(vf_net* n, Layer& l, const float* x, const float* go, int Bn, std::vector<Deferred>* deferred, const VfConvExtras* ex) {
  vf_ctx* ctx = n->ctx;
  const bool full = is_full(l);
  float* gw = n->grads + l.w_off;
  float* gb = n->grads + l.b_off;
  const float beta = l.fresh ? 0.f : 1.f;
  l.fresh = false;
  if (deferred && l.Co % 4 == 0 && ((uintptr_t)go & 15) == 0) {
    deferred->push_back(Deferred{go, gb, (int64_t)Bn * l.Ho * l.Wo, l.Co, beta});
    gb = nullptr;
  }
  VF_REQUIRE(!(n->fused_adam && l.fa && l.fa_k > 0 && beta != 0.f),
             "fused Adam: a second backward pass accumulates onto a weight gradient that was never written (one backward per zeroGradParameters)");
  if (n->fused_adam && l.fa && beta == 0.f) {
    l.fa_u = full ? x : go;
    l.fa_v = full ? go : x;
    l.fa_k = Bn;
    l.g_seen = nullptr;
    l.gp_seen = nullptr;
    if (!gb) return 0;
    return vf_internal_colsum(ctx, go, gb, (int64_t)Bn * l.Ho * l.Wo, l.Co, beta);
  }
  l.fa_k = 0;
  const bool planes = g_pwgrad && !g_no_pconv && l.x_seen == x && l.xp_seen && l.g_seen == go && l.gp_seen;
  const void *xp = l.xp_seen, *gp = l.gp_seen;
  l.g_seen = nullptr;
  l.gp_seen = nullptr;
  if (!planes) xp = gp = nullptr;
  return full ? vf_internal_deconv2d_bwd_weight(ctx, x, go, xp, gp, gw, gb, l.shape(Bn), beta)
              : vf_internal_conv2d_bwd_weight(ctx, x, go, xp, gp, gw, gb, l.shape(Bn), beta, ex);
}

int bn_backward(vf_net* n, Layer& l, const float* x, const float* gy, int Bn, bool want_gx, bool want_gp, int act, float slope,
                const float* y_act, int gsel, int pre_rows, bool want_planes) {
  vf_ctx* ctx = n->ctx;
  VF_REQUIRE(n->train, "vf_net_backward: BatchNorm backward in evaluate mode is not part of the path");
  const float* gamma = n->params + l.w_off;
  float* gg = want_gp ? n->grads + l.w_off : nullptr;
  float* gbt = want_gp ? n->grads + l.b_off : nullptr;
  float* gx = want_gx ? l.gx : nullptr;
  float pbeta = 1.f;
  if (want_gp) {
    pbeta = l.fresh ? 0.f : 1.f;
    l.fresh = false;
  }
  l.grad_planes = nullptr;
  const int G = gsel >= 0 ? 1 : n->groups;
  const int row = gsel >= 0 ? gsel : 0;
  float *sm = l.sm + (int64_t)row * l.C, *si = l.si + (int64_t)row * l.C;
  double* su = l.sums + (int64_t)row * 2 * l.C;
  const int64_t npix_g = (int64_t)Bn * l.H * l.W / G;
  void* gp = nullptr;
  if (want_planes && gx && !sync_on(n)) {
    if (int rc = ensure_planes(n, &l.bgp, (int64_t)n->B * l.H * l.W * l.C)) return rc;
    gp = l.bgp;
  }
  if (pre_rows > 0) {
    int rc = vf_bn_bwd_pre(ctx, l.part, pre_rows, x, gy, gx, gg, gbt, gamma, sm, si, su, npix_g, l.C, G, pbeta, gp);
    l.grad_planes = gp;
    return rc;
  }
  if (!sync_on(n)) {
    int rc = gp ? vf_bn_bwd_planes(ctx, x, y_act, gy, gx, gg, gbt, gamma, sm, si, su, npix_g, l.C, G, act, slope, pbeta, gp)
                : vf_bn_bwd_groups(ctx, x, y_act, gy, gx, gg, gbt, gamma, sm, si, su, npix_g, l.C, G, act, slope, pbeta);
    l.grad_planes = gp;
    return rc;
  }
  VF_REQUIRE(G == 1 && gsel < 0, "SyncBN with batch groups is not part of the path");
  const int64_t npix = (int64_t)Bn * l.H * l.W, n_total = npix * n->sync_world;
  if (int rc = vf_bn_bwd_stats(ctx, x, y_act, gy, sm, su, npix, l.C, act, slope)) return rc;
  if (want_gp)
    if (int rc = vf_bn_bwd_apply(ctx, x, y_act, gy, nullptr, gg, gbt, gamma, sm, si, su, npix, n_total, l.C, act, slope, pbeta)) return rc;
  if (n->comm)
    if (int rc = vf_comm_allreduce_inline(n->comm, ctx, su, 2 * l.C, 1, 0)) return rc;
  if (want_gx) return vf_bn_bwd_apply(ctx, x, y_act, gy, gx, nullptr, nullptr, gamma, sm, si, su, npix, n_total, l.C, act, slope, 1.f);
  return 0;
}

int bias_grad_flush(vf_net* n, const std::vector<Deferred>& items) {
  if (items.empty()) return 0;
  std::string key((const char*)items.data(), items.size() * sizeof(Deferred));
  char* ws = vf_ws_ptr(n->ctx);
  const size_t ws_avail = vf_ws_avail(n->ctx);
  auto it = n->colsum_plans.find(key);
  if (it == n->colsum_plans.end() || it->second.ws != ws || it->second.ws_avail != ws_avail) {
    std::vector<VfColsumDesc> desc(items.size());
    size_t off = 0;
    int b1 = 0, b2 = 0;
    for (size_t i = 0; i < items.size(); ++i) {
      const Deferred& d = items[i];
      int cq, rpb, gx, gy;
      if (int rc = vf_bias_grad_plan(d.P, d.C, &cq, &rpb, &gx, &gy)) return rc;
      desc[i] = VfColsumDesc{d.g, d.gb, (double*)(ws + off), d.P, d.C, cq, rpb, gx, gy, b1, b2, d.beta};
      off += ((size_t)gx * d.C * 8 + 255) / 256 * 256;
      b1 += gx * gy;
      b2 += (d.C + 3) / 4;
    }
    VF_REQUIRE(off <= ws_avail, "vf_net: workspace too small for the bias-gradient partials");
    void* dev = nullptr;
    if (int rc = net_alloc(n->owned, &dev, desc.size() * sizeof(VfColsumDesc))) return rc;
    VF_CHECK_HIP(hipMemcpy(dev, desc.data(), desc.size() * sizeof(VfColsumDesc), hipMemcpyHostToDevice));
    vf_net::ColsumPlan plan;
    plan.dev = dev;
    plan.n = (int)items.size(); plan.b1 = b1; plan.b2 = b2;
    plan.ws = ws; plan.ws_avail = ws_avail;
    n->colsum_plans[key] = plan;
    it = n->colsum_plans.find(key);
  }
  const vf_net::ColsumPlan& p = it->second;
  return vf_bias_grad_multi(n->ctx, p.dev, p.n, p.b1, p.b2);
}

int net_walk_back(vf_net* n, const float* x_in, const float* gy, const float** gx_out, bool want_gp, bool need_input_grad, int hi,
                  int lo, int gi, int G, int defer_cut = -1) {
  vf_ctx* ctx = n->ctx;
  const int np = (int)n->plan.size();
  if (hi < 0 || hi > np) hi = np;
  VF_REQUIRE(lo >= 0 && lo <= hi, "vf_net backward: bad plan range [%d, %d)", lo, hi);
  VF_REQUIRE(gi < 0 || (!want_gp && G >= 1 && gi < G && n->B % G == 0), "vf_net: bad batch group %d of %d", gi, G);
  VF_REQUIRE(!(want_gp && n->split_pending), "vf_net: a split backward is pending — call vf_net_backward_finish first");
  const int Bn = gi >= 0 ? n->B / G : n->B;
  int cut_wg = -1;
  size_t cut_bias = 0;
  const float* g = gy;
  const void* g_pl = nullptr;
  std::vector<Deferred> deferred;
  bool act_done = hi < np ? (n->act_done_at == hi) : false;
  int bn_pre = 0, pre = 0;
  if (!n->wp_managed)
    if (int rc = refresh_weight_planes(n)) return rc;
  if (hi < np && n->bn_pre_at == hi) bn_pre = n->bn_pre_rows;
  n->bn_pre_at = -1;
  int rc = 0;
  if (want_gp && (rc = vf_wgrad_group_begin(ctx))) return rc;
  auto slice = [&](const float* p, int64_t per_sample) { return (gi >= 0 && p) ? p + (int64_t)gi * Bn * per_sample : p; };
  for (int idx = hi - 1; idx >= lo && !rc; --idx) {
    if (want_gp && defer_cut >= 0 && idx == defer_cut - 1) {
      if ((rc = vf_wgrad_group_count(ctx, &cut_wg))) break;
      cut_bias = deferred.size();
    }
    const Entry& e = n->plan[idx];
    Layer& l = n->L[e.main];
    const float* x = idx == 0 ? x_in : slice(entry_out(n, idx - 1, nullptr), (int64_t)l.H * l.W * l.C);
    const float* mout = slice(entry_out(n, idx, nullptr), (int64_t)l.Ho * l.Wo * l.Co);
    const bool want_gx = need_input_grad || idx > 0;
    const int64_t out_e = (int64_t)Bn * l.Ho * l.Wo * l.Co;
    if (l.d.kind == VF_L_BN) {
      const int rows = bn_pre;
      bn_pre = 0;
      bool want_pl = false;
      if (want_gx && idx > 0) {
        const Layer& below = n->L[n->plan[idx - 1].main];
        want_pl = is_conv(below) && pconv_layer(below) && (idx - 1 > 0 || need_input_grad) &&
                  pconv_ok(n, below, below.grad_shape(Bn), !is_full(below));
      }
      rc = bn_backward(n, l, x, g, Bn, want_gx, want_gp, l.fused_act, l.fused_slope, l.fused_act != VF_ACT_NONE ? mout : nullptr,
                       gi, rows, want_pl);
      g = l.gx;
      g_pl = l.grad_planes;
      act_done = false;
      continue;
    }
    if (is_conv(l)) {
      const float* go = g;
      VfConvExtras ex;
      const bool dot_head = l.d.kind == VF_L_CONV && l.Co == 1 && l.d.k == 4 && l.d.stride == 1 && l.d.pad == 0 && l.H == 4 && l.W == 4 &&
                            l.fused_act != VF_ACT_NONE && !relu_like(l.fused_act) && !act_done;
      if (l.fused_act != VF_ACT_NONE && !act_done && !dot_head) {
        const bool ours = g != gy;
        if (relu_like(l.fused_act) && ours) {
          rc = vf_act_bwd(ctx, mout, g, const_cast<float*>(g), out_e, l.fused_act, l.fused_slope);
          g_pl = nullptr;
        } else {
          if (!l.gtmp && (rc = net_alloc(n->act_owned, (void**)&l.gtmp, sizeof(float) * (size_t)n->B * l.Ho * l.Wo * l.Co))) break;
          rc = vf_act_bwd(ctx, mout, g, l.gtmp, out_e, l.fused_act, l.fused_slope);
          go = l.gtmp;
          g_pl = nullptr;
        }
        if (rc) break;
      }
      int in_act = VF_ACT_NONE;
      float in_slope = 0.f;
      const unsigned* in_bits = nullptr;
      if (want_gx && idx > 0 && l.d.kind == VF_L_CONV && is_s2(l)) {
        const Layer& pm = n->L[n->plan[idx - 1].main];
        if (is_conv(pm) && relu_like(pm.fused_act)) {
          in_act = pm.fused_act;
          in_slope = pm.fused_slope;
          if (pm.bits_live && pm.ybits && !n->observer)
            in_bits = pm.ybits + (gi >= 0 ? (int64_t)gi * Bn * pm.Ho * pm.Wo * (pm.Co / 32) : 0);
        }
      }
      bool fuse_below = false;
      if (want_gx && idx > 1) {
        Layer& pm = n->L[n->plan[idx - 1].main];
        if (pm.d.kind == VF_L_BN && bn_fusable(n, pm) && (pm.fused_act == VF_ACT_NONE || relu_like(pm.fused_act)) && pm.C == l.C &&
            (gi < 0 || n->groups == G)) {
          const float* xbn = slice(entry_out(n, idx - 2, nullptr), (int64_t)pm.H * pm.W * pm.C);
          const float* yact = pm.fused_act != VF_ACT_NONE ? x : nullptr;
          const float* smv = gi >= 0 ? pm.sm + (int64_t)gi * pm.C : pm.sm;
          if ((rc = vf_internal_bn_request_bwd(&ex.bn, xbn, yact, pm.fused_act, pm.fused_slope, smv, pm.part, pm.part_rows_cap,
                                               gi >= 0 ? 1 : n->groups)))
            break;
          fuse_below = true;
        }
      }
      ex.dot_act_y = dot_head ? mout : nullptr;
      ex.dot_act = l.fused_act;
      ex.dot_act_slope = l.fused_slope;
      if (want_gx) {
        if (!fuse_below && in_act != VF_ACT_NONE) ex.dmask_bits = in_bits;
        rc = conv_bwd_data(n, l, x, go, Bn, fuse_below ? VF_ACT_NONE : in_act, in_slope, g_pl, &ex);
        pre = ex.bn_result_rows;
        if (rc) break;
      }
      if (want_gp) {
        rc = conv_acc(n, l, x, go, Bn, &deferred, &ex);
        if (rc) break;
      }
      g = want_gx ? l.gx : nullptr;
      g_pl = nullptr;
      act_done = !fuse_below && in_act != VF_ACT_NONE && want_gx;
      bn_pre = pre;
      pre = 0;
      continue;
    }
    if (l.d.kind == VF_L_ACT && !l.absorbed) {
      rc = vf_act_bwd(ctx, mout, g, l.gx, out_e, l.d.act, l.d.slope);
      g = l.gx;
      g_pl = nullptr;
    }
    act_done = false;
  }
  if (want_gp) {
    if (rc) {
      (void)vf_wgrad_group_abort(ctx);
      return rc;
    }
    if (defer_cut >= 0 && cut_wg >= 0) {
      if ((rc = vf_wgrad_group_end_partial(ctx, cut_wg))) return rc;
      std::vector<Deferred> first(deferred.begin(), deferred.begin() + cut_bias);
      if ((rc = bias_grad_flush(n, first))) return rc;
      n->pending_bias.assign((const char*)(deferred.data() + cut_bias), (deferred.size() - cut_bias) * sizeof(Deferred));
      n->split_pending = true;
    } else {
      if ((rc = vf_wgrad_group_end(ctx))) return rc;
      if ((rc = bias_grad_flush(n, deferred))) return rc;
    }
  }
  if (rc) return rc;
// ... 15 lines not shown
  free_pool(n->act_owned);
  n->colsum_plans.clear();
  n->B = B; n->C0 = C; n->H0 = H; n->W0 = W;
  n->act_done_at = n->bn_pre_at = -1;
  int c = C, h = H, w = W;
  for (size_t i = 0; i < n->L.size(); ++i) {
    Layer& l = n->L[i];
    l.C = c; l.H = h; l.W = w;
    l.Co = c; l.Ho = h; l.Wo = w;
    switch (l.d.kind) {
      case VF_L_CONV:
      case VF_L_FULLCONV:
        VF_REQUIRE(l.d.nin == c, "vf_net: layer %d expects %d input planes, gets %d", (int)i, l.d.nin, c);
        l.Co = l.d.nout;
        l.Ho = is_full(l) ? l.shape(B).full_out_h() : l.shape(B).out_h();
        l.Wo = is_full(l) ? l.shape(B).full_out_w() : l.shape(B).out_w();
        break;
      case VF_L_BN:
        VF_REQUIRE(l.d.nout == c, "vf_net: BatchNorm layer %d has %d channels, gets %d", (int)i, l.d.nout, c);
        break;
      default:
        break;
    }
    VF_REQUIRE(l.Ho > 0 && l.Wo > 0, "vf_net: layer %d has an empty output", (int)i);
    c = l.Co; h = l.Ho; w = l.Wo;
    l.y = l.y_own = l.gx = l.gtmp = nullptr;
    l.xp = l.gp = l.yp = l.bgp = nullptr;
    l.ybits = nullptr;
    l.bits_live = false;
    l.out_planes = l.grad_planes = nullptr;
    l.x_seen = l.g_seen = nullptr;
    l.xp_seen = l.gp_seen = nullptr;
    l.part = nullptr;
    l.sm = l.si = nullptr;
    l.sums = nullptr;
  }
  n->gcap = std::max(n->groups, 2);
  for (size_t i = 0; i < n->L.size(); ++i) {
    Layer& l = n->L[i];
    const size_t in_e = (size_t)B * l.H * l.W * l.C, out_e = (size_t)B * l.Ho * l.Wo * l.Co;
    const bool own_out = is_conv(l) || l.d.kind == VF_L_BN || (l.d.kind == VF_L_ACT && !l.absorbed);
    if (own_out) {
      if (int rc = net_alloc(n->act_owned, (void**)&l.y_own, sizeof(float) * out_e)) return rc;
      l.y = l.y_own;
    }
    if (is_conv(l) || l.d.kind == VF_L_BN || (l.d.kind == VF_L_ACT && !l.absorbed))
      if (int rc = net_alloc(n->act_owned, (void**)&l.gx, sizeof(float) * in_e)) return rc;
    if (l.d.kind == VF_L_BN) {
      const size_t gc = (size_t)n->gcap * l.C;
      if (int rc = net_alloc(n->act_owned, (void**)&l.sm, 4 * gc)) return rc;
      if (int rc = net_alloc(n->act_owned, (void**)&l.si, 4 * gc)) return rc;
      if (int rc = net_alloc(n->act_owned, (void**)&l.sums, 16 * gc)) return rc;
      const int64_t npix = (int64_t)B * l.H * l.W;
      l.part_rows_cap = (int)std::max<int64_t>(npix / 64, 512) + 8 * n->gcap;
      if (int rc = net_alloc(n->act_owned, (void**)&l.part, sizeof(double) * (size_t)l.part_rows_cap * 2 * l.C)) return rc;
      (void)hipMemsetAsync(l.sm, 0, 4 * gc, n->ctx->stream);
      (void)hipMemsetAsync(l.si, 0, 4 * gc, n->ctx->stream);
      (void)hipMemsetAsync(l.sums, 0, 16 * gc, n->ctx->stream);
    }
  }
  return 0;
}

}

VF_API int vf_net_destroy(vf_net* n) {
  if (!n) return 0;
  if (n->ctx) (void)hipStreamSynchronize(n->ctx->stream);
  free_pool(n->act_owned);
  free_pool(n->owned);
  delete n;
  return 0;
}

VF_API int vf_net_create(vf_ctx* ctx, vf_net** out, const vf_layer_desc* layers, int nlayers, int B, int C, int H, int W) {
  VF_REQUIRE(ctx && out && layers && nlayers > 0 && B > 0 && C > 0 && H > 0 && W > 0, "vf_net_create: bad arguments");
  *out = nullptr;
  vf_net* n = new vf_net();
  n->ctx = ctx;
  int64_t off = 0;
// ... 553 lines not shown
```

### video-filler_amd/nn.py

```python
import torch

from .backend import bump_param_version, get_backend, is_nhwc, param_version, to_nhwc


class DeviceScalar:

    def __init__(self, fn):
        self._fn = fn

    @staticmethod
    def of(t):
        return DeviceScalar(lambda: float(t.item()))

    def __float__(self):
        return float(self._fn())

    def _bin(self, other, op):
        a, b = self, other
        return DeviceScalar(lambda: op(float(a), float(b)))

    def __add__(self, o):
        return self._bin(o, lambda x, y: x + y)

    __radd__ = __add__
# ... 136 lines not shown
            wp = self.weight_planes(self._is_full, refresh=not managed)
            fn = B.pconv_scatter if self._is_full else B.pconv_gather
            fn(xp, wp, self.bias, y, Bn, H, W, Cin, self.nOutputPlane, act, slope)
            return y
        self._x_planes = None
        fn = B.deconv2d_fwd if self._is_full else B.conv2d_fwd
        fn(input, self.weight, self.bias, y, self.kH, self.dH, self.padH, act, slope)
        return y

    def updateGradInput(self, input, gradOutput, in_act=None, buf="gradInput", g_planes=None, managed=False):
        gx = self._buf(buf, *input.shape)
        B = get_backend()
        go = to_nhwc(gradOutput)
        Bn, Co, Ho, Wo = go.shape
        if self._pconv_ok(Bn, Ho, Wo, Co, self.nInputPlane, not self._is_full) and (in_act is None or not self._is_full):
            gp = g_planes if g_planes is not None else B.planes_split(go, self._planes_buf("_gp" + buf, go.numel()))
            self._g_planes = (go.data_ptr(), tuple(go.shape), gp)
            wp = self.weight_planes(not self._is_full, refresh=not managed)
            if self._is_full:
                B.pconv_gather(gp, wp, None, gx, Bn, Ho, Wo, Co, self.nInputPlane)
            elif in_act is not None:
                B.pconv_scatter(gp, wp, None, gx, Bn, Ho, Wo, Co, self.nInputPlane, dmask=input, dact=in_act[0], dslope=in_act[1])
            else:
                B.pconv_scatter(gp, wp, None, gx, Bn, Ho, Wo, Co, self.nInputPlane)
            return gx
        self._g_planes = None
        if in_act is not None:
            B.conv2d_bwd_data_act(to_nhwc(gradOutput), self.weight, gx, input, in_act[0], in_act[1], self.kH, self.dH, self.padH)
            return gx
        fn = B.deconv2d_bwd_data if self._is_full else B.conv2d_bwd_data
        fn(to_nhwc(gradOutput), self.weight, gx, self.kH, self.dH, self.padH)
        return gx

    def accGradParameters(self, input, gradOutput, scale=1, defer_bias=None, use_planes=True):
        assert scale == 1, "the reference always uses scale = 1"
        beta = 0.0 if self._fresh else 1.0
        self._fresh = False
        fn = get_backend().deconv2d_bwd_weight if self._is_full else get_backend().conv2d_bwd_weight
        go = to_nhwc(gradOutput)
        gb = self.gradBias
        if defer_bias is not None and self.nOutputPlane % 4 == 0 and go.data_ptr() % 16 == 0:
            defer_bias.append((go, self.gradBias, beta))
            gb = None
        x = to_nhwc(input)
        xs, gs = getattr(self, "_x_planes", None), getattr(self, "_g_planes", None)
        self._g_planes = None
        if (use_planes and _PWGRAD and not _NO_PCONV and xs is not None and gs is not None and xs[0] == x.data_ptr()
                and xs[1] == tuple(x.shape) and gs[0] == go.data_ptr() and gs[1] == tuple(go.shape)):
            fn(x, go, self.gradWeight, gb, self.kH, self.dH, self.padH, beta, xs[2], gs[2])
        else:
            fn(x, go, self.gradWeight, gb, self.kH, self.dH, self.padH, beta)

    def parameters(self):
        return [self.weight, self.bias], [self.gradWeight, self.gradBias]


class SpatialFullConvolution(SpatialConvolution):
    _type = "nn.SpatialFullConvolution"
    _is_full = True


class SpatialBatchNormalization(Module):
    _type = "nn.SpatialBatchNormalization"

    def __init__(self, nOutput, eps=1e-5, momentum=0.1, affine=True):
        super().__init__()
        assert affine, "the reference builds affine BN only"
        B = get_backend()
        self.nOutputPlane = nOutput
        self.eps, self.momentum = eps, momentum
        self.weight = B.zeros(nOutput) + 1.0
        self.bias = B.zeros(nOutput)
        self.gradWeight = B.zeros(nOutput)
        self.gradBias = B.zeros(nOutput)
        self.running_mean = B.zeros(nOutput)
        self.running_var = B.zeros(nOutput) + 1.0
        self.save_mean = B.zeros(nOutput)
        self.save_std = B.zeros(nOutput)
        self._sums = B.zeros(2 * nOutput, dtype=torch.float64)
        self._fresh = False
        self.sync_world = 1
        self.sync_group = None
        self.sync_force = False
        self.groups = 1
# ... 59 lines not shown
                if hasattr(B, "bn_train_fwd"):
                    B.bn_train_fwd(xg, yg, self.weight, self.bias, self.running_mean, self.running_var, sm, ss, su,
                                   self.momentum, self.eps, act, slope)
                else:
                    B.bn_stats(xg, self.running_mean, su)
                    B.bn_finalize(su, self.running_mean, self.running_var, sm, ss, h * H * W, self.momentum, self.eps)
                    B.bn_apply(xg, yg, self.weight, self.bias, sm, ss, act, slope)
            return y
        if self.train and not self._sync() and hasattr(B, "bn_train_fwd"):
            B.bn_train_fwd(input, y, self.weight, self.bias, self.running_mean, self.running_var, self.save_mean,
                           self.save_std, self._sums, self.momentum, self.eps, act, slope)
        elif self.train:
            B.bn_stats(input, self.running_mean, self._sums)
            if self._sync():
                B.all_reduce(self._sums, self.sync_group)
            B.bn_finalize(self._sums, self.running_mean, self.running_var, self.save_mean, self.save_std,
                          Bn * H * W * self.sync_world, self.momentum, self.eps)
            B.bn_apply(input, y, self.weight, self.bias, self.save_mean, self.save_std, act, slope)
        else:
            B.bn_eval_fwd(input, y, self.weight, self.bias, self.running_mean, self.running_var, self.eps, act, slope)
        return y

    def _group_state(self):
        if self._gsave is None or len(self._gsave) != self.groups:
            B = get_backend()
            n, G = self.nOutputPlane, self.groups
            self._gmean, self._gstd = B.zeros(G * n), B.zeros(G * n)
            self._gsums = B.zeros(G * 2 * n, dtype=torch.float64)
            self._gsave = [(self._gmean[g * n:(g + 1) * n], self._gstd[g * n:(g + 1) * n],
                            self._gsums[g * 2 * n:(g + 1) * 2 * n]) for g in range(G)]
        return self._gsave

    def _bwd(self, input, gradOutput, want_gx, want_gp, act="none", slope=0.0, y_act=None, group=None, buf="gradInput",
             pre_rows=0, want_planes=False):
        assert self.train, "the reference never back-propagates through BN in evaluate mode"
        B = get_backend()
        input, gradOutput = to_nhwc(input), to_nhwc(gradOutput)
        Bn, Cc, H, W = input.shape
        gx = self._buf(buf, Bn, Cc, H, W) if want_gx else None
        pbeta = 1.0
        if want_gp:
            pbeta = 0.0 if self._fresh else 1.0
            self._fresh = False
        self.grad_planes = None
        if pre_rows > 0:
            assert self.fusable()
            if group is not None:
                (sm, ss, su), G = self._group_state()[group], 1
            else:
                (sm, ss, su), G = self._stat_bufs(), self.groups
            gp = None
            if want_planes and gx is not None:
                gp = getattr(self, "_gp_" + buf, None)
                if gp is None or gp.shape[1] != gx.numel():
                    gp = torch.empty((3, gx.numel()), dtype=torch.bfloat16, device=gx.device)
                    setattr(self, "_gp_" + buf, gp)
            B.bn_bwd_pre(self._part, pre_rows, input, gradOutput, gx, self.gradWeight if want_gp else None,
                         self.gradBias if want_gp else None, self.weight, sm, ss, su, G, pbeta, gp)
            self.grad_planes = gp
            return gx
        if want_planes and gx is not None and not self._sync() and hasattr(B, "bn_bwd_groups"):
            if group is not None:
                (sm, ss, su), G = self._group_state()[group], 1
            else:
                (sm, ss, su), G = self._stat_bufs(), self.groups
            gp = getattr(self, "_gp_" + buf, None)
            if gp is None or gp.shape[1] != gx.numel():
                gp = torch.empty((3, gx.numel()), dtype=torch.bfloat16, device=gx.device)
                setattr(self, "_gp_" + buf, gp)
            B.bn_bwd_groups(input, y_act, gradOutput, gx, self.gradWeight if want_gp else None, self.gradBias if want_gp else None,
                            self.weight, sm, ss, su, G, act, slope, pbeta, gx_planes=gp)
            self.grad_planes = gp
            return gx
        if self.groups > 1:
            assert not self._sync()
            state = self._group_state()
            gw, gb = (self.gradWeight, self.gradBias) if want_gp else (None, None)

            def one(x, ya, gy, gxx, st, pb):
                sm, ss, su = st
                if hasattr(B, "bn_bwd"):
                    B.bn_bwd(x, ya, gy, gxx, gw, gb, self.weight, sm, ss, su, act, slope, pb)
                else:
                    B.bn_bwd_stats(x, ya, gy, sm, su, act, slope)
                    B.bn_bwd_apply(x, ya, gy, gxx, gw, gb, self.weight, sm, ss, su, x.shape[0] * H * W, act, slope, pb)

            if group is not None:
                one(input, y_act, gradOutput, gx, state[group], pbeta)
                return gx
            h = Bn // self.groups
            if hasattr(B, "bn_bwd_groups") and not _NO_BN_GROUPS:
# ... 346 lines not shown
                if Sequential.act_hook is not None and isinstance(m, _Act) and m.act in ("lrelu", "relu"):
                    Sequential.act_hook(m, cur)
            else:
                cur = m.updateOutput(cur, a.act, a.slope)
                a.output = cur
                if Sequential.act_hook is not None and a.act in ("lrelu", "relu"):
                    Sequential.act_hook(a, cur)
        self.output = cur
        return cur

    @staticmethod
    def _run_act_hook(a, cur, cur_pl):
        if Sequential.act_hook is None or a.act not in ("lrelu", "relu"):
            return
        edited = Sequential.act_hook(a, cur)
        if cur_pl is not None and edited is not False:
            get_backend().planes_split(cur, cur_pl)

    def _walk(self, input, gradOutput, want_gp, need_input_grad=True, hi=None, lo=0, group=None, defer_cut=None):
        plan = self._plan or self._build_plan()
        B = get_backend()
        g = gradOutput
        used_side = False
        deferred = [] if (want_gp and self.fuse and hasattr(B, "bias_grad_multi") and not _NO_DEFER_BIAS) else None
        grouped = (want_gp and self.fuse and self.side is None and hasattr(B, "wgrad_group_begin") and not _NO_WG_GROUP
                   and not Sequential._group_open)
        if grouped:
            B.wgrad_group_begin()
            Sequential._group_open = True
        hi = len(plan) if hi is None else hi
        act_done = self._act_done_at == hi if hi < len(plan) else False
        bn_pre, pre = 0, [0]
        g_pl = None
        managed = self._wp_managed
        if not managed or self._wp_stale():
            self.refresh_weight_planes()
            managed = True
        if hi < len(plan) and self._bn_pre_at is not None and self._bn_pre_at[0] == hi:
            bn_pre = self._bn_pre_at[1]
        self._bn_pre_at = None
        cut_wg, cut_bias = None, 0
        assert not getattr(self, "_split_pending", None) or not want_gp, "a split backward is pending: call backward_finish() first"
        try:
            for idx in range(hi - 1, lo - 1, -1):
                if defer_cut is not None and want_gp and idx == defer_cut - 1:
                    cut_wg = B.wgrad_group_count() if grouped else 0
                    cut_bias = len(deferred) if deferred is not None else 0
                m, a = plan[idx]
                x = input if idx == 0 else plan[idx - 1][0].output
                mout = m.output
                gbuf = "gradInput"
                if group is not None:
                    gi, G = group
                    gbuf = "gradInput_g"
                    h = mout.shape[0] // G
                    mout = mout[gi * h:(gi + 1) * h]
                    if idx > 0:
                        x = x[gi * h:(gi + 1) * h]
                want_gx = need_input_grad or idx > 0
                if isinstance(m, ParallelTable):
                    assert group is None, "group passes are built for plain chains"
                    g = m.walk(x, g, want_gx, want_gp)
                    g_pl = None
                    act_done = False
                    continue
                if isinstance(m, SpatialBatchNormalization):
                    gsel = None if group is None else group[0]
                    rows, bn_pre = bn_pre, 0
                    below = plan[idx - 1][0] if idx > 0 else None
                    want_pl = (self.fuse and want_gx and isinstance(below, SpatialConvolution) and below.pconv_layer()
                               and (idx - 1 > 0 or need_input_grad) and not _NO_PCONV
                               and below._pconv_ok(x.shape[0], x.shape[2], x.shape[3], below.nOutputPlane, below.nInputPlane,
                                                   not below._is_full))
                    if a is None:
                        g = m._bwd(x, g, want_gx, want_gp, group=gsel, buf=gbuf, pre_rows=rows, want_planes=want_pl)
                    else:
                        a.gradInput = g
                        g = m._bwd(x, g, want_gx, want_gp, a.act, a.slope, mout, group=gsel, buf=gbuf, pre_rows=rows,
                                   want_planes=want_pl)
                    g_pl = m.grad_planes
                else:
                    if a is not None:
                        if not act_done:
                            if a.inplace:
                                B.act_bwd(mout, g, g, a.act, a.slope)
                            else:
                                bufs = a.__dict__.setdefault("_gfused", {})
                                gb_ = bufs.get(tuple(g.shape))
                                if gb_ is None:
                                    gb_ = bufs[tuple(g.shape)] = torch.empty_like(g)
                                B.act_bwd(mout, g, gb_, a.act, a.slope)
                                g = gb_
                            g_pl = None
                        a.gradInput = g
                    in_act = None
                    if (self.fuse and want_gx and idx > 0 and type(m) is SpatialConvolution and m.dH == 2 and m.kH == 4 and m.padH == 1 and hasattr(B, "conv2d_bwd_data_act")):
                        pm, pa = plan[idx - 1]
                        if pa is not None and pa.act in ("lrelu", "relu") and not isinstance(pm, SpatialBatchNormalization):
                            in_act = (pa.act, pa.slope)
                    fuse_below = None
                    if (self.fuse and want_gx and idx > 1 and isinstance(m, SpatialConvolution) and hasattr(B, "bn_fuse_next_bwd")):
                        pm, pa = plan[idx - 1]
                        if (isinstance(pm, SpatialBatchNormalization) and pm.fusable() and (pa is None or pa.act in ("lrelu", "relu"))
                                and pm.nOutputPlane == m.nInputPlane and (group is None or pm.groups == group[1])):
                            fuse_below = (pm, pa)
                    if fuse_below is not None:
                        def upd(m=m, x=x, g=g, fb=fuse_below, idx=idx, gpl=g_pl):
                            pm, pa = fb
                            xbn = plan[idx - 2][0].output
                            yact = pm.output if pa is not None else None
                            if group is not None:
                                gi, G = group
                                hb = xbn.shape[0] // G
                                xbn = xbn[gi * hb:(gi + 1) * hb]
                                yact = None if yact is None else yact[gi * hb:(gi + 1) * hb]
                                sm, ng = pm._group_state()[gi][0], 1
                            else:
                                sm, ng = pm._stat_bufs()[0], pm.groups
                            B.bn_fuse_next_bwd(xbn, yact, pa.act if pa is not None else "none", pa.slope if pa is not None else 0.0,
                                               sm, pm.part_buffer(xbn.shape[0] * xbn.shape[2] * xbn.shape[3]), ng)
                            out = m.updateGradInput(x, g, None, gbuf, g_planes=gpl, managed=managed)
                            pre[0] = B.bn_fuse_result()
                            return out
                    elif isinstance(m, SpatialConvolution):
                        upd = lambda: m.updateGradInput(x, g, in_act, gbuf, g_planes=g_pl, managed=managed)
                    elif group is not None and isinstance(m, _Act):
                        upd = lambda: m.updateGradInput(x, g, mout)
                    else:
                        upd = lambda: m.updateGradInput(x, g)
                    if want_gp and self.side is not None and m.parameters():
                        with self.side.on():
                            self._acc(m, x, g, deferred, use_planes=False)
                        used_side = True
                        gin = upd() if want_gx else None
                    else:
                        gin = upd() if want_gx else None
                        if want_gp:
                            self._acc(m, x, g, deferred)
                    g = gin
                    g_pl = None
                    act_done = in_act is not None
                    bn_pre, pre[0] = pre[0], 0
                    continue
                act_done = False
        except BaseException:
            if grouped:
                Sequential._group_open = False
                B.wgrad_group_abort()
            raise
        if cut_wg is not None:
            if grouped:
                B.wgrad_group_end_partial(cut_wg)
            if deferred:
                if deferred[:cut_bias]:
                    B.bias_grad_multi(deferred[:cut_bias])
            self._split_pending = (grouped, deferred[cut_bias:] if deferred else [])
        else:
            if grouped:
                Sequential._group_open = False
                B.wgrad_group_end()
            if deferred:
                B.bias_grad_multi(deferred)
        if used_side:
            self.side.join()
        self._act_done_at = lo if act_done else -1
        self._bn_pre_at = (lo, bn_pre) if (bn_pre and lo > 0) else None
        if lo == 0:
            self.gradInput = g
        return g

    @staticmethod
    def _acc(m, x, g, deferred, use_planes=True):
        if isinstance(m, SpatialConvolution):
            m.accGradParameters(x, g, 1, deferred, use_planes)
        else:
            m.accGradParameters(x, g, 1)

    def refresh_weight_planes(self):
        B = get_backend()
        if self._flat is not None:
            self._wp_version = param_version(self._flat[0])
        if _NO_PCONV or getattr(B, "mfma_mode", None) not in _PLANES_MODES or not hasattr(B, "weight_planes_multi"):
            return
        mods = [m for m in self.leaves() if isinstance(m, SpatialConvolution) and getattr(m, "_wp_live", False)
                and m._wp_src == m.weight.data_ptr() and getattr(m, "_wp_mode", None) == B.mfma_mode]
        if not mods:
            return
        key = tuple(m.weight.data_ptr() for m in mods)
        if self._wp_plan is None or self._wp_plan[3] != key:
            self._wp_plan = B.weight_planes_multi([(m.weight, m._wp[0], m._wp[1]) for m in mods])
        B.weight_planes_run(self._wp_plan)

    def _wp_stale(self):
        return self._flat is not None and param_version(self._flat[0]) != getattr(self, "_wp_version", -1)

    def set_weight_planes_managed(self, on=True):
        self._wp_managed = bool(on)
        return self

    def redirect_last_output(self, cur, buf):
        last = [m for m in self.leaves() if isinstance(m, SpatialConvolution)][-1]
        lo = getattr(last, "output", None)
        if lo is not None and lo.data_ptr() == cur.data_ptr() and tuple(lo.shape) == tuple(buf.shape):
            last.output = buf
            return True
        return False

# ... 254 lines not shown
```

Baseline: 23390.

## Fuse conv bias-gradient partial sums into BN backward and first-layer wgrad kernels

```diff
diff --git a/include/vf_hip.h b/include/vf_hip.h
--- a/include/vf_hip.h
+++ b/include/vf_hip.h
@@ -62,6 +62,10 @@
 int vf_deconv2d_bwd_weight_planes(vf_ctx* ctx, const float* x, const float* gy, const void* x_planes, const void* gy_planes,
                                   float* gw, float* gb, int B, int H, int W, int Cin, int Cout, int k, int stride, int pad,
                                   float beta);
+int vf_conv2d_bwd_weight_bias_rows(vf_ctx* ctx, const float* x, const float* gy, int B, int H, int W, int Cin, int Cout, int k,
+                                   int stride, int pad, int* rows, int* terms_per_thread);
+int vf_conv2d_bwd_weight_bias(vf_ctx* ctx, const float* x, const float* gy, float* gw, int B, int H, int W, int Cin, int Cout,
+                              int k, int stride, int pad, float beta, double* bias_part, int rows_cap);
 
 int vf_bn_stats(vf_ctx* ctx, const float* x, const float* shift, double* sums, int64_t npix, int C);
 int vf_bn_finalize(vf_ctx* ctx, const double* sums, float* running_mean, float* running_var, float* save_mean,
@@ -286,6 +290,15 @@
 
 int vf_bias_grad_plan(int64_t P, int C, int* cq, int* rows_per_block, int* gx, int* gy);
 int vf_bias_grad_multi(vf_ctx* ctx, const void* desc_dev, int n, int blocks1, int blocks2);
+int vf_bn_bwd_bias_rows(int64_t npix_per_group, int C, int groups, int* rows, int* terms_per_thread);
+int vf_bn_bwd_bias(vf_ctx* ctx, const float* x, const float* y_act, const float* gy, float* gx, float* ggamma, float* gbeta,
+                   const float* gamma, const float* save_mean, const float* save_invstd, double* sums, int64_t npix_per_group,
+                   int C, int groups, int act, float slope, float pbeta, void* gx_planes, double* bias_part);
+int vf_bn_bwd_pre_bias(vf_ctx* ctx, const double* part, int rows_per_group, const float* x, const float* g_masked, float* gx,
+                       float* ggamma, float* gbeta, const float* gamma, const float* save_mean, const float* save_invstd,
+                       double* sums, int64_t npix_per_group, int C, int groups, float pbeta, void* gx_planes,
+                       double* bias_part);
+int vf_bias_grad_finish(vf_ctx* ctx, const void* desc_dev, int n, int blocks2);
 
 typedef struct vf_comm vf_comm;
 #define VF_COMM_ID_BYTES 128
diff --git a/video-filler_amd/_lib.py b/video-filler_amd/_lib.py
--- a/video-filler_amd/_lib.py
+++ b/video-filler_amd/_lib.py
@@ -69,6 +69,10 @@
     "vf_wgrad_group_abort": (i32, [vp]),
     "vf_bias_grad_plan": (i32, [i64, i32, vp, vp, vp, vp]),
     "vf_bias_grad_multi": (i32, [vp, vp, i32, i32, i32]),
+    "vf_bn_bwd_bias_rows": (i32, [i64, i32, i32, vp, vp]),
+    "vf_bn_bwd_bias": (i32, [vp] * 11 + [i64, i32, i32, i32, f32, f32, vp, vp]),
+    "vf_bn_bwd_pre_bias": (i32, [vp, vp, i32] + [vp] * 9 + [i64, i32, i32, f32, vp, vp]),
+    "vf_bias_grad_finish": (i32, [vp, vp, i32, i32]),
     "vf_center_prepare": (i32, [vp, vp, vp, vp, vp, i32, i32, i32, i32]),
     "vf_clip_prepare": (i32, [vp, vp, vp, vp, vp, vp, i32, i32, i32, i32, i32, i32, i32, f32, i32, i32, vp, vp]),
     "vf_tiles_gather": (i32, [vp, vp, vp, i32, i32, i32, i32, i32, vp]),
@@ -141,6 +145,8 @@
     "vf_wgrad_adam_outer_rows": (i32, [vp, vp, vp, i32, i32, i64, i32, i32, i32, i32, vp, vp, vp, vp, C.c_float, f64, f64, f64, vp]),
     "vf_conv_is_fast": (i32, [i32, i32, i32, i32, i32]),
     "vf_conv2d_bwd_weight_planes": (i32, [vp, vp, vp, vp, vp, vp, vp, i32, i32, i32, i32, i32, i32, i32, i32, f32]),
+    "vf_conv2d_bwd_weight_bias_rows": (i32, [vp, vp, vp] + [i32] * 8 + [vp, vp]),
+    "vf_conv2d_bwd_weight_bias": (i32, [vp, vp, vp, vp] + [i32] * 8 + [f32, vp, i32]),
     "vf_deconv2d_bwd_weight_planes": (i32, [vp, vp, vp, vp, vp, vp, vp, i32, i32, i32, i32, i32, i32, i32, i32, f32]),
     "vf_comm_available": (i32, []),
     "vf_comm_unique_id": (i32, [vp]),
diff --git a/video-filler_amd/backend.py b/video-filler_amd/backend.py
--- a/video-filler_amd/backend.py
+++ b/video-filler_amd/backend.py
@@ -11,6 +11,27 @@
                ("gx", "<i4"), ("gy", "<i4"), ("blk1_off", "<i4"), ("blk2_off", "<i4"), ("beta", "<f4")]
 WPLANES_DESC = [("w", "<u8"), ("nat", "<u8"), ("tr", "<u8"), ("d0", "<i4"), ("d1", "<i4"), ("gx", "<i4"), ("gz", "<i4"),
                 ("blk_off", "<i4"), ("pad", "<i4")]
+
+
+def colsum_table(lib, entries, ws):
+    desc = np.zeros(len(entries), dtype=COLSUM_DESC)
+    off, b1, b2 = 0, 0, 0
+    for i, (g, gb, P, Cc, beta, part, rows) in enumerate(entries):
+        assert Cc % 4 == 0 and g % 16 == 0
+        geo = [C.c_int() for _ in range(4)]
+        _lib.check(lib.vf_bias_grad_plan(P, Cc, *[C.byref(v) for v in geo]))
+        cq, rpb, gx, gy = [v.value for v in geo]
+        if part:
+            assert rows > 0
+            desc[i] = (g, gb, part, P, Cc, cq, rpb, rows, gy, b1, b2, beta)
+        else:
+            desc[i] = (g, gb, ws + off, P, Cc, cq, rpb, gx, gy, b1, b2, beta)
+            off += (gx * Cc * 8 + 255) // 256 * 256
+            b1 += gx * gy
+        b2 += (Cc + 3) // 4
+    return desc, off, b1, b2
+
+
 MFMA_MODES = {"f32": 0, "bf16": 1, "f32_3xbf16": 3}
 DEFAULT_MFMA_MODE = "f32_3xbf16"
 
@@ -717,31 +738,33 @@
         import numpy as np
         if not items:
             return
+        items = [tuple(it) + (None, 0) if len(it) == 3 else tuple(it) for it in items]
         key = (self.workspace.data_ptr(), self.workspace.numel()) + tuple(
-            (g.data_ptr(), gb.data_ptr(), g.numel(), gb.numel(), float(beta)) for g, gb, beta in items)
+            (g.data_ptr(), gb.data_ptr(), g.numel(), gb.numel(), float(beta), 0 if part is None else part.data_ptr(), int(rows))
+            for g, gb, beta, part, rows in items)
         cache = self.__dict__.setdefault("_colsum_plans", {})
         plan = cache.get(key)
         if plan is None:
-            desc = np.zeros(len(items), dtype=COLSUM_DESC)
-            ws = self.workspace.data_ptr()
-            off, b1, b2 = 0, 0, 0
-            for i, (g, gb, beta) in enumerate(items):
+            entries = []
+            for g, gb, beta, part, rows in items:
                 Cc = gb.numel()
-                P = g.numel() // Cc
-                assert Cc % 4 == 0 and g.data_ptr() % 16 == 0 and is_nhwc(g)
-                geo = [C.c_int() for _ in range(4)]
-                _lib.check(self.lib.vf_bias_grad_plan(P, Cc, *[C.byref(v) for v in geo]))
-                cq, rpb, gx, gy = [v.value for v in geo]
-                desc[i] = (g.data_ptr(), gb.data_ptr(), ws + off, P, Cc, cq, rpb, gx, gy, b1, b2, beta)
-                off += (gx * Cc * 8 + 255) // 256 * 256
-                b1 += gx * gy
-                b2 += (Cc + 3) // 4
+                assert is_nhwc(g) and (part is None or (part.dtype == torch.float64 and part.numel() >= rows * Cc))
+                entries.append((g.data_ptr(), gb.data_ptr(), g.numel() // Cc, Cc, beta, 0 if part is None else part.data_ptr(), int(rows)))
+            desc, off, b1, b2 = colsum_table(self.lib, entries, self.workspace.data_ptr())
             assert off <= self.workspace.numel(), "workspace too small for the bias-gradient partials"
             dev = torch.from_numpy(desc.view(np.uint8).copy()).to(self.device)
             plan = (dev, len(items), b1, b2)
             cache[key] = plan
         dev, n, b1, b2 = plan
-        self._c("vf_bias_grad_multi", _ptr(dev), n, b1, b2)
+        if b1:
+            self._c("vf_bias_grad_multi", _ptr(dev), n, b1, b2)
+        else:
+            self._c("vf_bias_grad_finish", _ptr(dev), n, b2)
+
+    def bn_bwd_bias_rows(self, npix_per_group, Cc, groups):
+        rows, terms = C.c_int(0), C.c_int(0)
+        _lib.check(self.lib.vf_bn_bwd_bias_rows(npix_per_group, Cc, groups, C.byref(rows), C.byref(terms)))
+        return rows.value, terms.value
 
     def conv2d_bwd_weight(self, x, gy, gw, gb, k, stride, pad, beta, x_planes=None, gy_planes=None):
         B, Cin, H, W = x.shape
@@ -751,6 +774,19 @@
             return
         self._c("vf_conv2d_bwd_weight", _ptr(x), _ptr(gy), _ptr(gw), _ptr(gb), B, H, W, Cin, gw.shape[0], k, stride,
                 pad, beta)
+
+    def conv2d_bwd_weight_bias_rows(self, x, gy, k, stride, pad):
+        B, Cin, H, W = x.shape
+        rows, terms = C.c_int(0), C.c_int(0)
+        self._c("vf_conv2d_bwd_weight_bias_rows", _ptr(x), _ptr(gy), B, H, W, Cin, gy.shape[1], k, stride, pad, C.byref(rows),
+                C.byref(terms))
+        return rows.value, terms.value
+
+    def conv2d_bwd_weight_bias(self, x, gy, gw, k, stride, pad, beta, bias_part, rows_cap):
+        B, Cin, H, W = x.shape
+        assert bias_part.dtype == torch.float64 and bias_part.numel() >= rows_cap * gw.shape[0]
+        self._c("vf_conv2d_bwd_weight_bias", _ptr(x), _ptr(gy), _ptr(gw), B, H, W, Cin, gw.shape[0], k, stride, pad, beta,
+                _ptr(bias_part), rows_cap)
 
     def deconv2d_fwd(self, x, w, bias, y, k, stride, pad, act="none", slope=0.0):
         B, Cin, H, W = x.shape
@@ -846,9 +882,15 @@
                 _ptr(save_invstd), _ptr(sums), (B // groups) * H * W, Cc, groups, momentum, eps, ACT[act], slope)
 
     def bn_bwd_groups(self, x, y_act, gy, gx, ggamma, gbeta, gamma, save_mean, save_invstd, sums, groups, act="none",
-                      slope=0.0, pbeta=1.0, gx_planes=None):
+                      slope=0.0, pbeta=1.0, gx_planes=None, bias_part=None):
         B, Cc, H, W = x.shape
         assert B % groups == 0 and save_mean.numel() == groups * Cc and sums.numel() == groups * 2 * Cc
+        if bias_part is not None:
+            assert gx is not None and bias_part.numel() >= self.bn_bwd_bias_rows((B // groups) * H * W, Cc, groups)[0] * Cc
+            self._c("vf_bn_bwd_bias", _ptr(x), _ptr(y_act), _ptr(gy), _ptr(gx), _ptr(ggamma), _ptr(gbeta), _ptr(gamma),
+                    _ptr(save_mean), _ptr(save_invstd), _ptr(sums), (B // groups) * H * W, Cc, groups, ACT[act], slope, pbeta,
+                    _ptr(gx_planes), _ptr(bias_part))
+            return
         if gx_planes is not None:
             self._c("vf_bn_bwd_planes", _ptr(x), _ptr(y_act), _ptr(gy), _ptr(gx), _ptr(ggamma), _ptr(gbeta), _ptr(gamma),
                     _ptr(save_mean), _ptr(save_invstd), _ptr(sums), (B // groups) * H * W, Cc, groups, ACT[act], slope, pbeta,
@@ -878,8 +920,14 @@
                 _ptr(y_planes))
 
     def bn_bwd_pre(self, part, rows, x, g_masked, gx, ggamma, gbeta, gamma, save_mean, save_invstd, sums, groups, pbeta=1.0,
-                   gx_planes=None):
+                   gx_planes=None, bias_part=None):
         B, Cc, H, W = x.shape
+        if bias_part is not None:
+            assert gx is not None and bias_part.numel() >= self.bn_bwd_bias_rows((B // groups) * H * W, Cc, groups)[0] * Cc
+            self._c("vf_bn_bwd_pre_bias", _ptr(part), rows, _ptr(x), _ptr(g_masked), _ptr(gx), _ptr(ggamma), _ptr(gbeta), _ptr(gamma),
+                    _ptr(save_mean), _ptr(save_invstd), _ptr(sums), (B // groups) * H * W, Cc, groups, pbeta, _ptr(gx_planes),
+                    _ptr(bias_part))
+            return
         self._c("vf_bn_bwd_pre", _ptr(part), rows, _ptr(x), _ptr(g_masked), _ptr(gx), _ptr(ggamma), _ptr(gbeta), _ptr(gamma),
                 _ptr(save_mean), _ptr(save_invstd), _ptr(sums), (B // groups) * H * W, Cc, groups, pbeta, _ptr(gx_planes))
 
diff --git a/video-filler_amd/csrc/vf_bn.hip b/video-filler_amd/csrc/vf_bn.hip
--- a/video-filler_amd/csrc/vf_bn.hip
+++ b/video-filler_amd/csrc/vf_bn.hip
@@ -327,18 +327,21 @@
   }
 }
 
-__global__ __launch_bounds__(256) void k_bn_bwd_apply(const float* __restrict__ x, const float* __restrict__ yact,
-                                                      const float* __restrict__ gy, float* __restrict__ gx,
-                                                      float* __restrict__ ggamma, float* __restrict__ gbeta,
-                                                      const float* __restrict__ gamma, const float* __restrict__ mean,
-                                                      const float* __restrict__ invstd, const double* __restrict__ sums,
-                                                      int64_t npix, double n, int C, int cq, int rows_per_block, int act,
-                                                      float slope, float pbeta, unsigned short* __restrict__ planes, int64_t pstride, int npl) {
+template <bool BP>
+__device__ __forceinline__ void bn_bwd_apply_body(const float* __restrict__ x, const float* __restrict__ yact,
+                                                  const float* __restrict__ gy, float* __restrict__ gx,
+                                                  float* __restrict__ ggamma, float* __restrict__ gbeta,
+                                                  const float* __restrict__ gamma, const float* __restrict__ mean,
+                                                  const float* __restrict__ invstd, const double* __restrict__ sums,
+                                                  int64_t npix, double n, int C, int cq, int rows_per_block, int act,
+                                                  float slope, float pbeta, unsigned short* __restrict__ planes, int64_t pstride, int npl,
+                                                  double* __restrict__ bias_part) {
   const int rp = 256 / cq;
   const int tx = threadIdx.x % cq, ty = threadIdx.x / cq;
   const int c4 = blockIdx.y * cq + tx;
-  if (c4 >= (C >> 2)) return;
-  if (blockIdx.x == 0 && blockIdx.z == 0 && ty == 0) {
+  const bool live = c4 < (C >> 2);
+  if (!BP && !live) return;
+  if (live && blockIdx.x == 0 && blockIdx.z == 0 && ty == 0) {
 #pragma unroll
     for (int e = 0; e < 4; ++e) {
       float gg = (ggamma && pbeta != 0.f) ? pbeta * ggamma[4 * c4 + e] : 0.f;
@@ -352,7 +355,7 @@
       if (gbeta) gbeta[4 * c4 + e] = gb;
     }
   }
-  if (!gx) return;
+  if (!BP && !gx) return;
   {
     const int64_t go = (int64_t)blockIdx.z * npix * C;
     x += go;
@@ -364,30 +367,62 @@
     invstd += (int64_t)blockIdx.z * C;
     sums += (int64_t)blockIdx.z * 2 * C;
   }
-  const int64_t r0 = (int64_t)blockIdx.x * rows_per_block, r1 = min(npix, r0 + rows_per_block);
-  const f32x4 mu = *(const f32x4*)(mean + 4 * c4), is = *(const f32x4*)(invstd + 4 * c4);
-  const f32x4 ga = gamma ? *(const f32x4*)(gamma + 4 * c4) : f32x4{1, 1, 1, 1};
-  f32x4 kk, gm;
-#pragma unroll
-  for (int e = 0; e < 4; ++e) {
-    const double sum = sums[4 * c4 + e], dotp = sums[C + 4 * c4 + e];
-    kk[e] = (float)(dotp * is[e] * is[e] / n);
-    gm[e] = (float)(sum / n);
-  }
-  for (int64_t r = r0 + ty; r < r1; r += rp) {
-    const int64_t o = r * C + 4 * c4;
-    f32x4 g = *(const f32x4*)(gy + o);
-    if (act != VF_ACT_NONE) {
-      const f32x4 ya = *(const f32x4*)(yact + o);
-#pragma unroll
-      for (int e = 0; e < 4; ++e) g[e] = vf_act_grad(ya[e], g[e], act, slope);
-    }
-    const f32x4 xv = *(const f32x4*)(x + o);
-    const f32x4 out = (g - gm - (xv - mu) * kk) * is * ga;
-    *(f32x4*)(gx + o) = out;
-    if (planes) bn_store_planes(planes, pstride, o, out, npl);
-  }
-}
+  f32x4 bs = {0, 0, 0, 0};
+  if (live) {
+    const int64_t r0 = (int64_t)blockIdx.x * rows_per_block, r1 = min(npix, r0 + rows_per_block);
+    const f32x4 mu = *(const f32x4*)(mean + 4 * c4), is = *(const f32x4*)(invstd + 4 * c4);
+    const f32x4 ga = gamma ? *(const f32x4*)(gamma + 4 * c4) : f32x4{1, 1, 1, 1};
+    f32x4 kk, gm;
+#pragma unroll
+    for (int e = 0; e < 4; ++e) {
+      const double sum = sums[4 * c4 + e], dotp = sums[C + 4 * c4 + e];
+      kk[e] = (float)(dotp * is[e] * is[e] / n);
+      gm[e] = (float)(sum / n);
+    }
+    for (int64_t r = r0 + ty; r < r1; r += rp) {
+      const int64_t o = r * C + 4 * c4;
+      f32x4 g = *(const f32x4*)(gy + o);
+      if (act != VF_ACT_NONE) {
+        const f32x4 ya = *(const f32x4*)(yact + o);
+#pragma unroll
+        for (int e = 0; e < 4; ++e) g[e] = vf_act_grad(ya[e], g[e], act, slope);
+      }
+      const f32x4 xv = *(const f32x4*)(x + o);
+      const f32x4 out = (g - gm - (xv - mu) * kk) * is * ga;
+      *(f32x4*)(gx + o) = out;
+      if (planes) bn_store_planes(planes, pstride, o, out, npl);
+      if (BP) bs += out;
+    }
+  }
+  if constexpr (BP) {
+    __shared__ f32x4 red[256];
+    red[threadIdx.x] = bs;
+    __syncthreads();
+    if (ty == 0 && live) {
+      double a[4] = {0, 0, 0, 0};
+      for (int j = 0; j < rp; ++j) {
+        const f32x4 u = red[j * cq + tx];
+        for (int e = 0; e < 4; ++e) a[e] += (double)u[e];
+      }
+      double* o = bias_part + ((int64_t)blockIdx.z * gridDim.x + blockIdx.x) * C;
+      for (int e = 0; e < 4; ++e) o[4 * c4 + e] = a[e];
+    }
+  }
+}
+#define VF_BN_BWD_APPLY_PARAMS                                                                                                    \
+  const float *__restrict__ x, const float *__restrict__ yact, const float *__restrict__ gy, float *__restrict__ gx,              \
+      float *__restrict__ ggamma, float *__restrict__ gbeta, const float *__restrict__ gamma, const float *__restrict__ mean,     \
+      const float *__restrict__ invstd, const double *__restrict__ sums, int64_t npix, double n, int C, int cq,                   \
+      int rows_per_block, int act, float slope, float pbeta, unsigned short *__restrict__ planes, int64_t pstride, int npl
+__global__ __launch_bounds__(256) void k_bn_bwd_apply(VF_BN_BWD_APPLY_PARAMS) {
+  bn_bwd_apply_body<false>(x, yact, gy, gx, ggamma, gbeta, gamma, mean, invstd, sums, npix, n, C, cq, rows_per_block, act, slope, pbeta,
+                           planes, pstride, npl, nullptr);
+}
+__global__ __launch_bounds__(256) void k_bn_bwd_apply_bias(VF_BN_BWD_APPLY_PARAMS, double* __restrict__ bias_part) {
+  bn_bwd_apply_body<true>(x, yact, gy, gx, ggamma, gbeta, gamma, mean, invstd, sums, npix, n, C, cq, rows_per_block, act, slope, pbeta,
+                          planes, pstride, npl, bias_part);
+}
+#undef VF_BN_BWD_APPLY_PARAMS
 
 __device__ __forceinline__ int vf_find_layer(const VfColsumDesc* __restrict__ d, int n, int blk, bool stage2) {
   int l = 0;
@@ -440,6 +475,33 @@
   for (int off = 32; off > 0; off >>= 1) t += __shfl_down(t, off, 64);
   if (lane == 0 && col < L.C) L.gb[col] = (L.beta != 0.f ? L.beta * L.gb[col] : 0.f) + (float)t;
 }
+__global__ __launch_bounds__(256) void k_reduce_bias_rows(const VfColsumDesc* __restrict__ d, int n) {
+  const int l = vf_find_layer(d, n, blockIdx.x, true);
+  const VfColsumDesc L = d[l];
+  const int cx = threadIdx.x & 3, ry = threadIdx.x >> 2;
+  const int col = (blockIdx.x - L.blk2_off) * 4 + cx;
+  double s[4] = {0, 0, 0, 0};
+  if (col < L.C) {
+    const double* p = L.part + col;
+    int k = ry;
+    for (; k + 448 < L.gx; k += 512) {
+      double v[8];
+#pragma unroll
+      for (int u = 0; u < 8; ++u) v[u] = p[(int64_t)(k + 64 * u) * L.C];
+#pragma unroll
+      for (int u = 0; u < 8; ++u) s[u & 3] += v[u];
+    }
+    for (; k < L.gx; k += 64) s[0] += p[(int64_t)k * L.C];
+  }
+  __shared__ double red[64][4];
+  red[ry][cx] = (s[0] + s[1]) + (s[2] + s[3]);
+  __syncthreads();
+  if (ry == 0 && col < L.C) {
+    double t = 0;
+    for (int j = 0; j < 64; ++j) t += red[j][cx];
+    L.gb[col] = (L.beta != 0.f ? L.beta * L.gb[col] : 0.f) + (float)t;
+  }
+}
 
 static int run_stats(vf_ctx* ctx, const BnGeom& g, double* sums, int C, int groups = 1) {
   hipLaunchKernelGGL((k_reduce_partials<0>), dim3((int)vf_cdiv(2 * C, 16), groups), dim3(256), 0, ctx->stream,
@@ -577,15 +639,21 @@
 static int bn_bwd_apply_groups(vf_ctx* ctx, const float* x, const float* y_act, const float* gy, float* gx, float* ggamma,
                                float* gbeta, const float* gamma, const float* save_mean, const float* save_invstd,
                                const double* sums, int64_t npix, int64_t n_total, int C, int groups, int act, float slope,
-                               float pbeta, void* planes = nullptr) {
+                               float pbeta, void* planes = nullptr, double* bias_part = nullptr) {
   VF_REQUIRE(C % 4 == 0, "BatchNorm channel count must be a multiple of 4 (got %d)", C);
   VF_REQUIRE(!planes || gx, "gradient planes go with the gradient itself");
+  VF_REQUIRE(!bias_part || gx, "bias partials are the column sums of the gradient: they go with the gradient itself");
   const BnGeom g = bn_geom(npix, C);
   VfProf prof(ctx, planes ? "bn_bwd_apply_planes" : "bn_bwd_apply", 0.0,
               gx ? (double)npix * C * groups * (4.0 * (act != VF_ACT_NONE ? 4 : 3) + (planes ? 6.0 : 0.0)) : 0.0);
-  hipLaunchKernelGGL(k_bn_bwd_apply, dim3(g.gx, g.gy, groups), dim3(256), 0, ctx->stream, x, y_act, gy, gx, ggamma, gbeta, gamma,
-                     save_mean, save_invstd, sums, npix, (double)n_total, C, g.cq, g.rows_per_block, act, slope, pbeta,
-                     (unsigned short*)planes, npix * C * groups, ctx->mfma_bf16 == 1 ? 1 : 3);
+  if (bias_part)
+    hipLaunchKernelGGL(k_bn_bwd_apply_bias, dim3(g.gx, g.gy, groups), dim3(256), 0, ctx->stream, x, y_act, gy, gx, ggamma, gbeta, gamma,
+                       save_mean, save_invstd, sums, npix, (double)n_total, C, g.cq, g.rows_per_block, act, slope, pbeta,
+                       (unsigned short*)planes, npix * C * groups, ctx->mfma_bf16 == 1 ? 1 : 3, bias_part);
+  else
+    hipLaunchKernelGGL(k_bn_bwd_apply, dim3(g.gx, g.gy, groups), dim3(256), 0, ctx->stream, x, y_act, gy, gx, ggamma, gbeta, gamma,
+                       save_mean, save_invstd, sums, npix, (double)n_total, C, g.cq, g.rows_per_block, act, slope, pbeta,
+                       (unsigned short*)planes, npix * C * groups, ctx->mfma_bf16 == 1 ? 1 : 3);
   VF_LAUNCH_CHECK();
   return 0;
 }
@@ -631,6 +699,21 @@
   if (int rc = bn_bwd_stats_groups(ctx, x, y_act, gy, save_mean, sums, npix_per_group, C, groups, act, slope)) return rc;
   return bn_bwd_apply_groups(ctx, x, y_act, gy, gx, ggamma, gbeta, gamma, save_mean, save_invstd, sums, npix_per_group,
                              npix_per_group, C, groups, act, slope, pbeta, gx_planes);
+}
+VF_API int vf_bn_bwd_bias_rows(int64_t npix_per_group, int C, int groups, int* rows, int* terms_per_thread) {
+  VF_REQUIRE(npix_per_group > 0 && C > 0 && C % 4 == 0 && groups >= 1 && groups <= 64 && rows, "vf_bn_bwd_bias_rows: bad shape");
+  const BnGeom g = bn_geom(npix_per_group, C);
+  *rows = groups * g.gx;
+  if (terms_per_thread) *terms_per_thread = g.rows_per_block / g.rp;
+  return 0;
+}
+VF_API int vf_bn_bwd_bias(vf_ctx* ctx, const float* x, const float* y_act, const float* gy, float* gx, float* ggamma, float* gbeta,
+                          const float* gamma, const float* save_mean, const float* save_invstd, double* sums, int64_t npix_per_group,
+                          int C, int groups, int act, float slope, float pbeta, void* gx_planes, double* bias_part) {
+  VF_REQUIRE(gx && bias_part, "vf_bn_bwd_bias: the gradient and its partial rows are not optional");
+  if (int rc = bn_bwd_stats_groups(ctx, x, y_act, gy, save_mean, sums, npix_per_group, C, groups, act, slope)) return rc;
+  return bn_bwd_apply_groups(ctx, x, y_act, gy, gx, ggamma, gbeta, gamma, save_mean, save_invstd, sums, npix_per_group,
+                             npix_per_group, C, groups, act, slope, pbeta, gx_planes, bias_part);
 }
 
 VF_API int vf_bn_train_fwd_pre(vf_ctx* ctx, const double* part, int rows_per_group, const float* x, float* y, const float* gamma,
@@ -648,9 +731,9 @@
   }
   return bn_apply_groups(ctx, x, y, gamma, beta, save_mean, save_invstd, npix_per_group, C, groups, act, slope, y_planes);
 }
-VF_API int vf_bn_bwd_pre(vf_ctx* ctx, const double* part, int rows_per_group, const float* x, const float* g_masked, float* gx,
-                         float* ggamma, float* gbeta, const float* gamma, const float* save_mean, const float* save_invstd,
-                         double* sums, int64_t npix_per_group, int C, int groups, float pbeta, void* gx_planes) {
+static int bn_bwd_pre(vf_ctx* ctx, const double* part, int rows_per_group, const float* x, const float* g_masked, float* gx,
+                      float* ggamma, float* gbeta, const float* gamma, const float* save_mean, const float* save_invstd, double* sums,
+                      int64_t npix_per_group, int C, int groups, float pbeta, void* gx_planes, double* bias_part) {
   VF_REQUIRE(C % 4 == 0, "BatchNorm channel count must be a multiple of 4 (got %d)", C);
   VF_REQUIRE(part && rows_per_group > 0 && groups >= 1 && groups <= 64, "vf_bn_bwd_pre: bad partials");
   {
@@ -661,7 +744,21 @@
     VF_LAUNCH_CHECK();
   }
   return bn_bwd_apply_groups(ctx, x, nullptr, g_masked, gx, ggamma, gbeta, gamma, save_mean, save_invstd, sums, npix_per_group,
-                             npix_per_group, C, groups, VF_ACT_NONE, 0.f, pbeta, gx_planes);
+                             npix_per_group, C, groups, VF_ACT_NONE, 0.f, pbeta, gx_planes, bias_part);
+}
+VF_API int vf_bn_bwd_pre(vf_ctx* ctx, const double* part, int rows_per_group, const float* x, const float* g_masked, float* gx,
+                         float* ggamma, float* gbeta, const float* gamma, const float* save_mean, const float* save_invstd,
+                         double* sums, int64_t npix_per_group, int C, int groups, float pbeta, void* gx_planes) {
+  return bn_bwd_pre(ctx, part, rows_per_group, x, g_masked, gx, ggamma, gbeta, gamma, save_mean, save_invstd, sums, npix_per_group, C,
+                    groups, pbeta, gx_planes, nullptr);
+}
+VF_API int vf_bn_bwd_pre_bias(vf_ctx* ctx, const double* part, int rows_per_group, const float* x, const float* g_masked, float* gx,
+                              float* ggamma, float* gbeta, const float* gamma, const float* save_mean, const float* save_invstd,
+                              double* sums, int64_t npix_per_group, int C, int groups, float pbeta, void* gx_planes,
+                              double* bias_part) {
+  VF_REQUIRE(gx && bias_part, "vf_bn_bwd_pre_bias: the gradient and its partial rows are not optional");
+  return bn_bwd_pre(ctx, part, rows_per_group, x, g_masked, gx, ggamma, gbeta, gamma, save_mean, save_invstd, sums, npix_per_group, C,
+                    groups, pbeta, gx_planes, bias_part);
 }
 
 VF_API int vf_bias_grad_plan(int64_t P, int C, int* cq, int* rows_per_block, int* gx, int* gy) {
@@ -679,3 +776,10 @@
   VF_LAUNCH_CHECK();
   return 0;
 }
+VF_API int vf_bias_grad_finish(vf_ctx* ctx, const void* desc_dev, int n, int blocks2) {
+  VF_REQUIRE(desc_dev != nullptr && n > 0 && blocks2 > 0, "vf_bias_grad_finish: empty plan");
+  VfProf prof(ctx, "bias_grad_finish", 0.0, 0.0);
+  hipLaunchKernelGGL(k_reduce_bias_rows, dim3(blocks2), dim3(256), 0, ctx->stream, (const VfColsumDesc*)desc_dev, n);
+  VF_LAUNCH_CHECK();
+  return 0;
+}
diff --git a/video-filler_amd/csrc/vf_conv.hip b/video-filler_amd/csrc/vf_conv.hip
--- a/video-filler_amd/csrc/vf_conv.hip
+++ b/video-filler_amd/csrc/vf_conv.hip
@@ -734,6 +734,7 @@
   int gx, gy, gz;
   int ksplit, nk;
   float beta;
+  double* bias_part;
 };
 
 enum WgV {
@@ -741,9 +742,10 @@
   WGV_VEC16,
   WGV_PIX3
 };
-template <int BM, bool VU, WgV VV, int BF = 0, int BN = 128>
+template <int BM, bool VU, WgV VV, int BF = 0, int BN = 128, bool UB = false>
 __device__ __forceinline__ void wgrad_body(const WGrad& p, const int block_id) {
   static_assert(VV == WGV_PIX3 ? (BN == 64 && BF != 0) : BN == 128, "the whole-pixel form is a 64-column tile of the bf16 modes");
+  static_assert(!UB || (VV == WGV_PIX3 && VU), "the bias partials ride in the whole-pixel form only");
   constexpr int BK = BF ? 32 : 16;
   constexpr int LDU = BM + 4, LDV = BN + 4;
   constexpr int WN = (BM == 128 && BN == 128) ? 64 : 32;
@@ -789,6 +791,7 @@
   const int un = n0 + 4 * uq;
 
   f32x4 ru[U_CH], rv[V_CH];
+  f32x4 ub = {0, 0, 0, 0};
   const __amdgpu_buffer_rsrc_t rsU = vf_rsrc(p.U, p.u_bytes), rsV = vf_rsrc(p.V, p.v_bytes);
 
   auto load_piece = [&](int kt, int pc, bool live) {
@@ -839,6 +842,7 @@
       int off;
       if (pc < U_CH) {
         v = ru[pc];
+        if constexpr (UB) ub += v;
         off = (ukk + pc * (1024 / BM)) * LDMU + 4 * uq;
       } else {
         const int i = pc - U_CH;
@@ -967,6 +971,22 @@
     __syncthreads();
   }
 
+  }
+  if constexpr (UB) {
+    constexpr int UQ = BM / 4, UR = 256 / UQ;
+    static_assert(SMEM_F >= 4 * 256, "the operand tiles hold 256 float4");
+    f32x4* red = (f32x4*)smem;
+    red[tid] = ub;
+    __syncthreads();
+    if (ukk == 0 && un < p.Nu) {
+      double a[4] = {0, 0, 0, 0};
+      for (int j = 0; j < UR; ++j) {
+        const f32x4 u = red[j * UQ + uq];
+        for (int e = 0; e < 4; ++e) a[e] += (double)u[e];
+      }
+      double* o = p.bias_part + (int64_t)ks * p.Nu + un;
+      for (int e = 0; e < 4; ++e) o[e] = a[e];
+    }
   }
   const int64_t total = (int64_t)p.Nu * Ncols;
   float* out = p.ksplit > 1 ? p.slab + (int64_t)ks * total : p.dW;
@@ -997,6 +1017,10 @@
 template <int BM, bool VU, WgV VV, int BF = 0>
 __global__ __launch_bounds__(256) void k_wgrad(const WGrad p) {
   wgrad_body<BM, VU, VV, BF, VV == WGV_PIX3 ? 64 : 128>(p, blockIdx.x);
+}
+template <int BM, int BF>
+__global__ __launch_bounds__(256) void k_wgrad_bias(const WGrad p) {
+  wgrad_body<BM, true, WGV_PIX3, BF, 64, true>(p, blockIdx.x);
 }
 
 #define VF_WG_GROUP_MAX 16
@@ -1724,9 +1748,13 @@
   return rc;
 }
 
+static bool wg_bias_served(const WgPlan& p) { return p.pix3 && p.route == WG_FP32_SINGLE && p.gx == 1 && p.gy == 1; }
+
 static int wgrad(vf_ctx* ctx, const float* U, const float* V, float* dW, const VfConvShape& s, bool full, float beta, const void* Up,
-                 const void* Vp) {
+                 const void* Vp, double* bias_part = nullptr, int bias_rows_cap = 0) {
   WgPlan p = wg_plan(ctx, s, full, U, V, Up, Vp);
+  VF_REQUIRE(!bias_part || (wg_bias_served(p) && p.ksplit <= bias_rows_cap),
+             "weight gradient with bias partials: this layer's launch does not make them (ask vf_conv2d_bwd_weight_bias_rows first)");
   if (p.route == WG_SMALLK) {
     const int rc = vf_internal_wgrad_smallk(ctx, U, V, dW, p.B, p.Nu, 16 * p.Cv, beta);
     if (rc >= 0) return rc;
@@ -1756,7 +1784,8 @@
     if (R.reserve(p.slab_bytes(), vf_ws_avail(ctx), &off)) slab = slab_at(off);
     else if (int rc = wg_flush(ctx)) return rc;
   }
-  const WGrad g = wg_desc(p, U, V, dW, slab, beta);
+  WGrad g = wg_desc(p, U, V, dW, slab, beta);
+  g.bias_part = bias_part;
   const int bf = ctx->mfma_bf16;
   const char* wname = p.pix3 ? (p.bm == 128 ? (bf == 3 ? "wgrad_128x64_pix3_bf16x3" : "wgrad_128x64_pix3_bf16")
                                             : (bf == 3 ? "wgrad_64x64_pix3_bf16x3" : "wgrad_64x64_pix3_bf16"))
@@ -1768,7 +1797,8 @@
     constexpr int bm_ = decltype(BM)::value, bf_ = decltype(BF)::value;
     if constexpr (bf_ != 0) {
       if (p.pix3) {
-        VF_LAUNCH_TIMED(ctx, wname, wfl, 0.0, (k_wgrad<bm_, true, WGV_PIX3, bf_>), grid, block, g);
+        if (bias_part) VF_LAUNCH_TIMED(ctx, wname, wfl, 0.0, (k_wgrad_bias<bm_, bf_>), grid, block, g);
+        else VF_LAUNCH_TIMED(ctx, wname, wfl, 0.0, (k_wgrad<bm_, true, WGV_PIX3, bf_>), grid, block, g);
         return;
       }
     }
@@ -1854,6 +1884,32 @@
   if (gb) return vf_internal_colsum(ctx, gy, gb, (int64_t)s.B * s.out_h() * s.out_w(), s.Cout, beta);
   return 0;
 }
+int vf_internal_conv2d_bwd_weight_bias_rows(vf_ctx* ctx, const float* x, const float* gy, const VfConvShape& s, int* rows, int* terms) {
+  *rows = 0;
+  if (terms) *terms = 0;
+  if (!s.matrix_core_conv() || check_conv_args(s) != 0 || (s.Cout == 1 && s.stride == 1)) return 0;
+  const WgPlan p = wg_plan(ctx, s, false, gy, x, nullptr, nullptr);
+  if (p.route == WG_SMALLK || !wg_bias_served(p) || !p.in_range(4)) return 0;
+  *rows = p.ksplit;
+  if (terms) *terms = (int)vf_cdiv(p.nk, p.ksplit) * (32 * p.bm / 4 / 256);
+  return 0;
+}
+int vf_internal_conv2d_bwd_weight_bias(vf_ctx* ctx, const float* x, const float* gy, float* gw, const VfConvShape& s, float beta,
+                                       double* bias_part, int rows_cap) {
+  VF_REQUIRE(bias_part && rows_cap > 0, "vf_conv2d_bwd_weight_bias: no room for the partial rows");
+  VF_REQUIRE(s.matrix_core_conv(), "vf_conv2d_bwd_weight_bias: not a matrix-core geometry");
+  if (int rc = check_conv_args(s)) return rc;
+  return wgrad(ctx, gy, x, gw, s, false, beta, nullptr, nullptr, bias_part, rows_cap);
+}
+VF_API int vf_conv2d_bwd_weight_bias_rows(vf_ctx* ctx, const float* x, const float* gy, int B, int H, int W, int Cin, int Cout, int k,
+                                          int stride, int pad, int* rows, int* terms_per_thread) {
+  VF_REQUIRE(ctx && rows, "vf_conv2d_bwd_weight_bias_rows: NULL argument");
+  return vf_internal_conv2d_bwd_weight_bias_rows(ctx, x, gy, VfConvShape{B, H, W, Cin, Cout, k, stride, pad}, rows, terms_per_thread);
+}
+VF_API int vf_conv2d_bwd_weight_bias(vf_ctx* ctx, const float* x, const float* gy, float* gw, int B, int H, int W, int Cin, int Cout,
+                                     int k, int stride, int pad, float beta, double* bias_part, int rows_cap) {
+  return vf_internal_conv2d_bwd_weight_bias(ctx, x, gy, gw, VfConvShape{B, H, W, Cin, Cout, k, stride, pad}, beta, bias_part, rows_cap);
+}
 VF_API int vf_conv2d_bwd_weight(vf_ctx* ctx, const float* x, const float* gy, float* gw, float* gb, int B, int H, int W,
                                 int Cin, int Cout, int k, int stride, int pad, float beta) {
   return vf_conv2d_bwd_weight_planes(ctx, x, gy, nullptr, nullptr, gw, gb, B, H, W, Cin, Cout, k, stride, pad, beta);
diff --git a/video-filler_amd/csrc/vf_internal.h b/video-filler_amd/csrc/vf_internal.h
--- a/video-filler_amd/csrc/vf_internal.h
+++ b/video-filler_amd/csrc/vf_internal.h
@@ -25,6 +25,9 @@
                                     const VfConvShape& s, VfConvExtras* ex);
 int vf_internal_conv2d_bwd_weight(vf_ctx* ctx, const float* x, const float* gy, const void* x_planes, const void* gy_planes, float* gw,
                                   float* gb, const VfConvShape& s, float beta, const VfConvExtras* ex);
+int vf_internal_conv2d_bwd_weight_bias_rows(vf_ctx* ctx, const float* x, const float* gy, const VfConvShape& s, int* rows, int* terms);
+int vf_internal_conv2d_bwd_weight_bias(vf_ctx* ctx, const float* x, const float* gy, float* gw, const VfConvShape& s, float beta,
+                                       double* bias_part, int rows_cap);
 int vf_internal_deconv2d_fwd(vf_ctx* ctx, const float* x, const float* w, const float* bias, float* y, const VfConvShape& s, int act,
                              float slope, VfConvExtras* ex);
 int vf_internal_deconv2d_bwd_data(vf_ctx* ctx, const float* gy, const float* w, float* gx, const VfConvShape& s, VfConvExtras* ex);
diff --git a/video-filler_amd/csrc/vf_net.hip b/video-filler_amd/csrc/vf_net.hip
--- a/video-filler_amd/csrc/vf_net.hip
+++ b/video-filler_amd/csrc/vf_net.hip
@@ -28,6 +28,8 @@
   double* sums = nullptr;
   double* part = nullptr;
   int part_rows_cap = 0;
+  double* bpart = nullptr;
+  int bpart_rows_cap = 0;
   void* xp = nullptr;
   void* gp = nullptr;
   void* yp = nullptr;
@@ -318,17 +320,29 @@
   int64_t P;
   int C;
   float beta;
+  const double* part;
+  int64_t rows;
 };
-
-int conv_acc(vf_net* n, Layer& l, const float* x, const float* go, int Bn, std::vector<Deferred>* deferred, const VfConvExtras* ex) {
+static_assert(sizeof(Deferred) == 48, "Deferred is compared byte by byte");
+
+int conv_acc(vf_net* n, Layer& l, const float* x, const float* go, int Bn, std::vector<Deferred>* deferred, const VfConvExtras* ex,
+             const double* bpart = nullptr, int brows = 0) {
   vf_ctx* ctx = n->ctx;
   const bool full = is_full(l);
   float* gw = n->grads + l.w_off;
   float* gb = n->grads + l.b_off;
   const float beta = l.fresh ? 0.f : 1.f;
   l.fresh = false;
+  bool own_rows = false;
   if (deferred && l.Co % 4 == 0 && ((uintptr_t)go & 15) == 0) {
-    deferred->push_back(Deferred{go, gb, (int64_t)Bn * l.Ho * l.Wo, l.Co, beta});
+    if (!bpart && !full && l.C == 3 && l.bpart) {
+      if (int rc = vf_internal_conv2d_bwd_weight_bias_rows(ctx, x, go, l.shape(Bn), &brows, nullptr)) return rc;
+      if (brows > 0 && brows <= l.bpart_rows_cap) {
+        bpart = l.bpart;
+        own_rows = true;
+      }
+    }
+    deferred->push_back(Deferred{go, gb, (int64_t)Bn * l.Ho * l.Wo, l.Co, beta, bpart, bpart ? brows : 0});
     gb = nullptr;
   }
   VF_REQUIRE(!(n->fused_adam && l.fa && l.fa_k > 0 && beta != 0.f),
@@ -348,12 +362,13 @@
   l.g_seen = nullptr;
   l.gp_seen = nullptr;
   if (!planes) xp = gp = nullptr;
+  if (own_rows) return vf_internal_conv2d_bwd_weight_bias(ctx, x, go, gw, l.shape(Bn), beta, l.bpart, l.bpart_rows_cap);
   return full ? vf_internal_deconv2d_bwd_weight(ctx, x, go, xp, gp, gw, gb, l.shape(Bn), beta)
               : vf_internal_conv2d_bwd_weight(ctx, x, go, xp, gp, gw, gb, l.shape(Bn), beta, ex);
 }
 
 int bn_backward(vf_net* n, Layer& l, const float* x, const float* gy, int Bn, bool want_gx, bool want_gp, int act, float slope,
-                const float* y_act, int gsel, int pre_rows, bool want_planes) {
+                const float* y_act, int gsel, int pre_rows, bool want_planes, double* bias_part = nullptr) {
   vf_ctx* ctx = n->ctx;
   VF_REQUIRE(n->train, "vf_net_backward: BatchNorm backward in evaluate mode is not part of the path");
   const float* gamma = n->params + l.w_off;
@@ -377,17 +392,22 @@
     gp = l.bgp;
   }
   if (pre_rows > 0) {
-    int rc = vf_bn_bwd_pre(ctx, l.part, pre_rows, x, gy, gx, gg, gbt, gamma, sm, si, su, npix_g, l.C, G, pbeta, gp);
+    VF_REQUIRE(!bias_part || (gx && !sync_on(n)), "vf_net: bias partials need the BatchNorm's own gradInput pass");
+    int rc = bias_part ? vf_bn_bwd_pre_bias(ctx, l.part, pre_rows, x, gy, gx, gg, gbt, gamma, sm, si, su, npix_g, l.C, G, pbeta, gp, bias_part)
+                       : vf_bn_bwd_pre(ctx, l.part, pre_rows, x, gy, gx, gg, gbt, gamma, sm, si, su, npix_g, l.C, G, pbeta, gp);
     l.grad_planes = gp;
     return rc;
   }
   if (!sync_on(n)) {
-    int rc = gp ? vf_bn_bwd_planes(ctx, x, y_act, gy, gx, gg, gbt, gamma, sm, si, su, npix_g, l.C, G, act, slope, pbeta, gp)
-                : vf_bn_bwd_groups(ctx, x, y_act, gy, gx, gg, gbt, gamma, sm, si, su, npix_g, l.C, G, act, slope, pbeta);
+    VF_REQUIRE(!bias_part || gx, "vf_net: bias partials need the BatchNorm's own gradInput pass");
+    int rc = bias_part ? vf_bn_bwd_bias(ctx, x, y_act, gy, gx, gg, gbt, gamma, sm, si, su, npix_g, l.C, G, act, slope, pbeta, gp, bias_part)
+             : gp      ? vf_bn_bwd_planes(ctx, x, y_act, gy, gx, gg, gbt, gamma, sm, si, su, npix_g, l.C, G, act, slope, pbeta, gp)
+                       : vf_bn_bwd_groups(ctx, x, y_act, gy, gx, gg, gbt, gamma, sm, si, su, npix_g, l.C, G, act, slope, pbeta);
     l.grad_planes = gp;
     return rc;
   }
   VF_REQUIRE(G == 1 && gsel < 0, "SyncBN with batch groups is not part of the path");
+  VF_REQUIRE(!bias_part, "vf_net: bias partials under SyncBN are not part of the path");
   const int64_t npix = (int64_t)Bn * l.H * l.W, n_total = npix * n->sync_world;
   if (int rc = vf_bn_bwd_stats(ctx, x, y_act, gy, sm, su, npix, l.C, act, slope)) return rc;
   if (want_gp)
@@ -412,9 +432,13 @@
       const Deferred& d = items[i];
       int cq, rpb, gx, gy;
       if (int rc = vf_bias_grad_plan(d.P, d.C, &cq, &rpb, &gx, &gy)) return rc;
-      desc[i] = VfColsumDesc{d.g, d.gb, (double*)(ws + off), d.P, d.C, cq, rpb, gx, gy, b1, b2, d.beta};
-      off += ((size_t)gx * d.C * 8 + 255) / 256 * 256;
-      b1 += gx * gy;
+      if (d.part) {
+        desc[i] = VfColsumDesc{d.g, d.gb, const_cast<double*>(d.part), d.P, d.C, cq, rpb, (int)d.rows, gy, b1, b2, d.beta};
+      } else {
+        desc[i] = VfColsumDesc{d.g, d.gb, (double*)(ws + off), d.P, d.C, cq, rpb, gx, gy, b1, b2, d.beta};
+        off += ((size_t)gx * d.C * 8 + 255) / 256 * 256;
+        b1 += gx * gy;
+      }
       b2 += (d.C + 3) / 4;
     }
     VF_REQUIRE(off <= ws_avail, "vf_net: workspace too small for the bias-gradient partials");
@@ -429,7 +453,7 @@
     it = n->colsum_plans.find(key);
   }
   const vf_net::ColsumPlan& p = it->second;
-  return vf_bias_grad_multi(n->ctx, p.dev, p.n, p.b1, p.b2);
+  return p.b1 ? vf_bias_grad_multi(n->ctx, p.dev, p.n, p.b1, p.b2) : vf_bias_grad_finish(n->ctx, p.dev, p.n, p.b2);
 }
 
 int net_walk_back(vf_net* n, const float* x_in, const float* gy, const float** gx_out, bool want_gp, bool need_input_grad, int hi,
@@ -446,6 +470,8 @@
   const float* g = gy;
   const void* g_pl = nullptr;
   std::vector<Deferred> deferred;
+  const double* bias_rows_of = nullptr;
+  int bias_nrows = 0;
   bool act_done = hi < np ? (n->act_done_at == hi) : false;
   int bn_pre = 0, pre = 0;
   if (!n->wp_managed)
@@ -475,13 +501,26 @@
         want_pl = is_conv(below) && pconv_layer(below) && (idx - 1 > 0 || need_input_grad) &&
                   pconv_ok(n, below, below.grad_shape(Bn), !is_full(below));
       }
+      double* bias_part = nullptr;
+      if (want_gp && want_gx && idx > lo && !sync_on(n)) {
+        Layer& below = n->L[n->plan[idx - 1].main];
+        const int64_t npix = (int64_t)Bn * l.H * l.W;
+        if (is_conv(below) && below.Co == l.C && below.Co % 4 == 0 && below.fused_act == VF_ACT_NONE && below.bpart &&
+            npix % n->groups == 0) {
+          if ((rc = vf_bn_bwd_bias_rows(npix / n->groups, l.C, n->groups, &bias_nrows, nullptr))) break;
+          if (bias_nrows <= below.bpart_rows_cap) bias_part = below.bpart;
+        }
+      }
       rc = bn_backward(n, l, x, g, Bn, want_gx, want_gp, l.fused_act, l.fused_slope, l.fused_act != VF_ACT_NONE ? mout : nullptr,
-                       gi, rows, want_pl);
+                       gi, rows, want_pl, bias_part);
+      bias_rows_of = bias_part;
       g = l.gx;
       g_pl = l.grad_planes;
       act_done = false;
       continue;
     }
+    const double* bpart = bias_rows_of;
+    bias_rows_of = nullptr;
     if (is_conv(l)) {
       const float* go = g;
       VfConvExtras ex;
@@ -536,7 +575,7 @@
         if (rc) break;
       }
       if (want_gp) {
-        rc = conv_acc(n, l, x, go, Bn, &deferred, &ex);
+        rc = conv_acc(n, l, x, go, Bn, &deferred, &ex, go == g ? bpart : nullptr, bias_nrows);
         if (rc) break;
       }
       g = want_gx ? l.gx : nullptr;
@@ -618,6 +657,8 @@
     l.x_seen = l.g_seen = nullptr;
     l.xp_seen = l.gp_seen = nullptr;
     l.part = nullptr;
+    l.bpart = nullptr;
+    l.bpart_rows_cap = 0;
     l.sm = l.si = nullptr;
     l.sums = nullptr;
   }
@@ -632,6 +673,18 @@
     }
     if (is_conv(l) || l.d.kind == VF_L_BN || (l.d.kind == VF_L_ACT && !l.absorbed))
       if (int rc = net_alloc(n->act_owned, (void**)&l.gx, sizeof(float) * in_e)) return rc;
+    if (is_conv(l) && l.Co % 4 == 0) {
+      if (i + 1 < n->L.size() && n->L[i + 1].d.kind == VF_L_BN) {
+        const int64_t npix = (int64_t)B * l.Ho * l.Wo;
+        for (int g = 1; g <= n->gcap; ++g) {
+          int rows = 0;
+          if (npix % g == 0 && vf_bn_bwd_bias_rows(npix / g, l.Co, g, &rows, nullptr) == 0) l.bpart_rows_cap = std::max(l.bpart_rows_cap, rows);
+        }
+      }
+      if (!is_full(l) && l.C == 3) l.bpart_rows_cap = std::max(l.bpart_rows_cap, 512);
+      if (l.bpart_rows_cap)
+        if (int rc = net_alloc(n->act_owned, (void**)&l.bpart, sizeof(double) * (size_t)l.bpart_rows_cap * l.Co)) return rc;
+    }
     if (l.d.kind == VF_L_BN) {
       const size_t gc = (size_t)n->gcap * l.C;
       if (int rc = net_alloc(n->act_owned, (void**)&l.sm, 4 * gc)) return rc;
diff --git a/video-filler_amd/nn.py b/video-filler_amd/nn.py
--- a/video-filler_amd/nn.py
+++ b/video-filler_amd/nn.py
@@ -192,17 +192,28 @@
         fn(to_nhwc(gradOutput), self.weight, gx, self.kH, self.dH, self.padH)
         return gx
 
-    def accGradParameters(self, input, gradOutput, scale=1, defer_bias=None, use_planes=True):
+    def accGradParameters(self, input, gradOutput, scale=1, defer_bias=None, use_planes=True, bias_part=None):
         assert scale == 1, "the reference always uses scale = 1"
         beta = 0.0 if self._fresh else 1.0
         self._fresh = False
         fn = get_backend().deconv2d_bwd_weight if self._is_full else get_backend().conv2d_bwd_weight
         go = to_nhwc(gradOutput)
         gb = self.gradBias
+        x = to_nhwc(input)
+        own_rows = None
         if defer_bias is not None and self.nOutputPlane % 4 == 0 and go.data_ptr() % 16 == 0:
-            defer_bias.append((go, self.gradBias, beta))
+            B = get_backend()
+            if bias_part is None and not self._is_full and self.nInputPlane == 3 and hasattr(B, "conv2d_bwd_weight_bias_rows"):
+                rows = B.conv2d_bwd_weight_bias_rows(x, go, self.kH, self.dH, self.padH)[0]
+                if 0 < rows <= self.OWN_BIAS_ROWS:
+                    own_rows = self._rows_buffer(B, self.OWN_BIAS_ROWS)
+                    bias_part = (own_rows, rows)
+            defer_bias.append((go, self.gradBias, beta) + (tuple(bias_part) if bias_part is not None else ()))
             gb = None
-        x = to_nhwc(input)
+        if own_rows is not None:
+            self._g_planes = None
+            B.conv2d_bwd_weight_bias(x, go, self.gradWeight, self.kH, self.dH, self.padH, beta, own_rows, self.OWN_BIAS_ROWS)
+            return
         xs, gs = getattr(self, "_x_planes", None), getattr(self, "_g_planes", None)
         self._g_planes = None
         if (use_planes and _PWGRAD and not _NO_PCONV and xs is not None and gs is not None and xs[0] == x.data_ptr()
@@ -210,6 +221,18 @@
             fn(x, go, self.gradWeight, gb, self.kH, self.dH, self.padH, beta, xs[2], gs[2])
         else:
             fn(x, go, self.gradWeight, gb, self.kH, self.dH, self.padH, beta)
+
+    def bias_part_buffer(self, B, npix, groups):
+        rows = B.bn_bwd_bias_rows(npix // groups, self.nOutputPlane, groups)[0]
+        return self._rows_buffer(B, rows), rows
+
+    OWN_BIAS_ROWS = 512
+
+    def _rows_buffer(self, B, rows):
+        t = getattr(self, "_bias_part", None)
+        if t is None or t.numel() < rows * self.nOutputPlane:
+            t = self._bias_part = B.zeros(rows * self.nOutputPlane, dtype=torch.float64)
+        return t
 
     def parameters(self):
         return [self.weight, self.bias], [self.gradWeight, self.gradBias]
@@ -335,7 +358,7 @@
         return self._gsave
 
     def _bwd(self, input, gradOutput, want_gx, want_gp, act="none", slope=0.0, y_act=None, group=None, buf="gradInput",
-             pre_rows=0, want_planes=False):
+             pre_rows=0, want_planes=False, bias_part=None):
         assert self.train, "the reference never back-propagates through BN in evaluate mode"
         B = get_backend()
         input, gradOutput = to_nhwc(input), to_nhwc(gradOutput)
@@ -359,7 +382,20 @@
                     gp = torch.empty((3, gx.numel()), dtype=torch.bfloat16, device=gx.device)
                     setattr(self, "_gp_" + buf, gp)
             B.bn_bwd_pre(self._part, pre_rows, input, gradOutput, gx, self.gradWeight if want_gp else None,
-                         self.gradBias if want_gp else None, self.weight, sm, ss, su, G, pbeta, gp)
+                         self.gradBias if want_gp else None, self.weight, sm, ss, su, G, pbeta, gp, bias_part=bias_part)
+            self.grad_planes = gp
+            return gx
+        if bias_part is not None:
+            assert gx is not None and group is None and not self._sync()
+            sm, ss, su = self._stat_bufs()
+            gp = None
+            if want_planes:
+                gp = getattr(self, "_gp_" + buf, None)
+                if gp is None or gp.shape[1] != gx.numel():
+                    gp = torch.empty((3, gx.numel()), dtype=torch.bfloat16, device=gx.device)
+                    setattr(self, "_gp_" + buf, gp)
+            B.bn_bwd_groups(input, y_act, gradOutput, gx, self.gradWeight if want_gp else None, self.gradBias if want_gp else None,
+                            self.weight, sm, ss, su, self.groups, act, slope, pbeta, gx_planes=gp, bias_part=bias_part)
             self.grad_planes = gp
             return gx
         if want_planes and gx is not None and not self._sync() and hasattr(B, "bn_bwd_groups"):
@@ -772,6 +808,8 @@
         act_done = self._act_done_at == hi if hi < len(plan) else False
         bn_pre, pre = 0, [0]
         g_pl = None
+        g_bias = None
+        side_rows = False
         managed = self._wp_managed
         if not managed or self._wp_stale():
             self.refresh_weight_planes()
@@ -801,7 +839,7 @@
                 if isinstance(m, ParallelTable):
                     assert group is None, "group passes are built for plain chains"
                     g = m.walk(x, g, want_gx, want_gp)
-                    g_pl = None
+                    g_pl = g_bias = None
                     act_done = False
                     continue
                 if isinstance(m, SpatialBatchNormalization):
@@ -812,14 +850,22 @@
                                and (idx - 1 > 0 or need_input_grad) and not _NO_PCONV
                                and below._pconv_ok(x.shape[0], x.shape[2], x.shape[3], below.nOutputPlane, below.nInputPlane,
                                                    not below._is_full))
+                    g_bias = None
+                    if (deferred is not None and want_gx and idx > lo and group is None and not m._sync()
+                            and isinstance(below, SpatialConvolution) and plan[idx - 1][1] is None and hasattr(B, "bn_bwd_bias_rows")
+                            and below.nOutputPlane == m.nOutputPlane and m.nOutputPlane % 4 == 0
+                            and (x.shape[0] * x.shape[2] * x.shape[3]) % m.groups == 0):
+                        g_bias = below.bias_part_buffer(B, x.shape[0] * x.shape[2] * x.shape[3], m.groups)
+                    bp = None if g_bias is None else g_bias[0]
                     if a is None:
-                        g = m._bwd(x, g, want_gx, want_gp, group=gsel, buf=gbuf, pre_rows=rows, want_planes=want_pl)
+                        g = m._bwd(x, g, want_gx, want_gp, group=gsel, buf=gbuf, pre_rows=rows, want_planes=want_pl, bias_part=bp)
                     else:
                         a.gradInput = g
                         g = m._bwd(x, g, want_gx, want_gp, a.act, a.slope, mout, group=gsel, buf=gbuf, pre_rows=rows,
-                                   want_planes=want_pl)
+                                   want_planes=want_pl, bias_part=bp)
                     g_pl = m.grad_planes
                 else:
+                    g_bias, gb_here = None, g_bias
                     if a is not None:
                         if not act_done:
                             if a.inplace:
@@ -870,13 +916,14 @@
                         upd = lambda: m.updateGradInput(x, g)
                     if want_gp and self.side is not None and m.parameters():
                         with self.side.on():
-                            self._acc(m, x, g, deferred, use_planes=False)
+                            self._acc(m, x, g, deferred, use_planes=False, bias_part=gb_here)
                         used_side = True
+                        side_rows = side_rows or (gb_here is None and bool(deferred) and len(deferred[-1]) > 3)
                         gin = upd() if want_gx else None
                     else:
                         gin = upd() if want_gx else None
                         if want_gp:
-                            self._acc(m, x, g, deferred)
+                            self._acc(m, x, g, deferred, bias_part=gb_here)
                     g = gin
                     g_pl = None
                     act_done = in_act is not None
@@ -888,6 +935,8 @@
                 Sequential._group_open = False
                 B.wgrad_group_abort()
             raise
+        if side_rows:
+            self.side.join()
         if cut_wg is not None:
             if grouped:
                 B.wgrad_group_end_partial(cut_wg)
@@ -910,9 +959,9 @@
         return g
 
     @staticmethod
-    def _acc(m, x, g, deferred, use_planes=True):
+    def _acc(m, x, g, deferred, use_planes=True, bias_part=None):
         if isinstance(m, SpatialConvolution):
-            m.accGradParameters(x, g, 1, deferred, use_planes)
+            m.accGradParameters(x, g, 1, deferred, use_planes, bias_part)
         else:
             m.accGradParameters(x, g, 1)
 
```

After: 23560 (median of 6 runs). Within noise of the previous version (+0.7%).
